# olofson/audiality2

Measured on AMD Instinct MI355X. Metric: voice-samples/sec + max realtime voices @48kHz, higher is better.
Workload: dtype int32; 1 GPU; 65536 voices 2xwtosc->panmix, 256 per group voice inline->fbdelay->fbdelay (benchmark/fmtest4.a2s delay settings; 256 groups, 512 fbdelays), 48 kHz, fragment=64, stereo (BASELINE configs[3]); voices_per_gpu=65536, chain=osc2-pan, groups=256

## Files before the change

### audiality2_amd/build.py

```python
import hashlib
import os
import shutil
import subprocess

HERE = os.path.dirname(os.path.abspath(__file__))
ROOT = os.path.dirname(HERE)
HIPCC = shutil.which("hipcc") or "/opt/rocm/bin/hipcc"


MARK = b"A2AMD_SRCHASH:"


def source_hash(sources, cmd=()):
    h = hashlib.sha256()
    for s in sources:
        h.update(os.path.basename(s).encode() + b"\0")
        with open(s, "rb") as f:
            h.update(f.read())
        h.update(b"\0")
    h.update(" ".join(cmd).encode())
    return h.hexdigest()[:32]


def stamped_hash(lib, mark=MARK):
    if not os.path.exists(lib):
        return None
    with open(lib, "rb") as f:
        blob = f.read()
    i = blob.find(mark)
    if i < 0:
        return None
    return blob[i + len(mark):i + len(mark) + 32].decode("ascii", "replace")


ENGMARK = b"A2AMD_ENGHASH:"


def engine_hash(engine):
    files = []
    for d in ("include", "src", os.path.join("src", "units"), os.path.join("src", "drivers")):
        p = os.path.join(engine, d)
        if os.path.isdir(p):
            files += [os.path.join(p, f) for f in sorted(os.listdir(p)) if f.endswith((".h", ".h.cmake", ".h.in"))]
    return source_hash(files, (stamped_hash(os.path.join(HERE, "liba2amd_units.so")) or "",))


def _stale(target, want):
    return stamped_hash(target) != want


def _define(h):
    return '-DA2AMD_SRCHASH="%s"' % h


def build_lib(force=False):
    csrc = os.path.join(HERE, "csrc")
    srcs = [os.path.join(csrc, f) for f in ("a2amd_host.cpp", "a2amd_sched.cpp", "a2amd_render.cpp", "a2amd_dist.cpp",
                                            "a2amd_vm.cpp", "a2amd_kernels.hip", "a2amd_fast.hip", "a2amd_vm.hip", "a2amd_wavecap.hip", "a2amd_wavepost.hip", "a2amd_win.hip", "a2amd_vmwin.hip", "a2amd_noise.hip", "a2amd_noisepan.hip", "a2amd_noisefiltpan.hip", "a2amd_cutsweep.hip", "a2amd_oscbare.hip", "a2amd_osc3filtpan.hip")]
    deps = srcs + [os.path.join(csrc, "a2amd_host.h"), os.path.join(csrc, "a2amd_switches.h"), os.path.join(csrc, "a2amd_device.h"), os.path.join(csrc, "a2amd_dsp.h"),
                   os.path.join(csrc, "a2amd_fm.h"), os.path.join(csrc, "a2amd_vmcore.h"), os.path.join(csrc, "a2amd_taps.h"), os.path.join(csrc, "a2amd_winctl.h"), os.path.join(csrc, "a2amd_vmdev.h"), os.path.join(csrc, "a2amd_noisemap.h"), os.path.join(csrc, "a2amd_noisevoice.h"), os.path.join(csrc, "a2amd_settled.h"), os.path.join(csrc, "a2amd_quiet.h"), os.path.join(csrc, "a2amd_cutsweep.h"), os.path.join(csrc, "a2amd_filt.h"), os.path.join(csrc, "a2amd_wavepads.h"), os.path.join(csrc, "a2amd_wavetame.h"), os.path.join(ROOT, "include", "a2amd.h"),
                   os.path.join(ROOT, "include", "a2amd_noise.h"), os.path.join(ROOT, "include", "a2amd_noisepan.h"), os.path.join(ROOT, "include", "a2amd_noisefilt.h"), os.path.join(ROOT, "include", "a2amd_sweep.h"), os.path.join(ROOT, "include", "a2amd_wavepost.h"),
                   os.path.join(ROOT, "include", "a2amd_bus.h"), os.path.join(ROOT, "include", "a2amd_oscbare.h"), os.path.join(ROOT, "include", "a2amd_osc3filt.h"), os.path.join(ROOT, "include", "a2amd_fbdpan.h"), os.path.join(ROOT, "include", "a2amd_buswin.h"), os.path.join(ROOT, "include", "a2amd_vmbatch.h"), os.path.join(ROOT, "include", "a2amd_osc2.h"), os.path.join(ROOT, "include", "a2amd_osc2lds.h"), os.path.join(ROOT, "include", "a2amd_osc2tame.h"), os.path.join(ROOT, "include", "a2amd_wavepool.h"), os.path.join(ROOT, "include", "a2amd_vm.h")]
    out = os.path.join(HERE, "liba2amd.so")
    flags = ["--offload-arch=gfx950", "-O3", "-std=c++17", "-fPIC", "-shared", "-Wno-unused-value"]
    want = source_hash(deps, flags)
    if force or _stale(out, want):
        subprocess.run([HIPCC] + flags + [_define(want), "-o", out] + srcs, check=True)
    return out


def build_units(force=False):
    src = os.path.join(HERE, "csrc", "a2amd_units.c")
    deps = [src, os.path.join(ROOT, "include", "a2amd.h"), os.path.join(ROOT, "include", "a2amd_noise.h"), os.path.join(ROOT, "include", "a2amd_noisepan.h"),
            os.path.join(ROOT, "include", "a2amd_noisefilt.h"), os.path.join(ROOT, "include", "a2amd_sweep.h"), os.path.join(ROOT, "include", "a2amd_bus.h"),
            os.path.join(ROOT, "include", "a2amd_wavepost.h"), os.path.join(ROOT, "include", "a2amd_oscbare.h"), os.path.join(ROOT, "include", "a2amd_osc3filt.h"), os.path.join(ROOT, "include", "a2amd_fbdpan.h"), os.path.join(ROOT, "include", "a2amd_buswin.h"), os.path.join(ROOT, "include", "a2amd_vmbatch.h"), os.path.join(ROOT, "include", "a2amd_osc2.h"), os.path.join(ROOT, "include", "a2amd_osc2lds.h"), os.path.join(ROOT, "include", "a2amd_osc2tame.h"), os.path.join(ROOT, "include", "a2amd_wavepool.h"), os.path.join(ROOT, "include", "a2amd_plugin.h"),
            os.path.join(ROOT, "include", "a2amd_walk.h"), os.path.join(ROOT, "include", "a2amd_vm.h")]
    out = os.path.join(HERE, "liba2amd_units.so")
    flags = ["-O2", "-Wall", "-fPIC", "-shared"]
    want = source_hash(deps, flags)
    if force or _stale(out, want):
        subprocess.run(["gcc"] + flags + [_define(want), "-o", out, src,
                        "-L" + HERE, "-la2amd", "-ldl", "-lpthread", "-lm", "-Wl,-rpath,$ORIGIN"], check=True)
    return out


def build_walk(force=False, engine=None):
    engine = engine or os.environ.get("A2_ENGINE_SRC", "/root/reference")
    out = os.path.join(HERE, "liba2amd_walk.so")
    src = os.path.join(HERE, "csrc", "a2amd_walk.c")
    own = [src, os.path.join(ROOT, "include", "a2amd_walk.h"), os.path.join(ROOT, "include", "a2amd_vm.h"),
           os.path.join(ROOT, "include", "a2amd_plugin.h")]
    flags = ["-O2", "-Wall", "-fPIC", "-shared"]
    want = source_hash(own, flags)
    kept = os.path.join(ROOT, "oracle", "_ref", "liba2amd_walk.so")
    if not (os.path.exists(os.path.join(engine, "src", "internals.h")) and shutil.which("cmake")):
        if (not os.path.exists(out) or _stale(out, want)) and not _stale(kept, want):
            shutil.copyfile(kept, out)
        if os.path.exists(out) and _stale(out, want):
            raise RuntimeError(f"{out} was not built from this tree's a2amd_walk.c (stamp {stamped_hash(out)}, "
                               f"sources {want}) and the engine's source tree ({engine}) is not here to rebuild it")
        return out if os.path.exists(out) else None
    inc = os.path.join(HERE, "_engine_include")
    weng = engine_hash(engine)
    if force or _stale(out, want) or stamped_hash(out, ENGMARK) != weng:
        subprocess.run(["cmake", f"-DENGINE={engine}", f"-DOUT={inc}", "-P", os.path.join(HERE, "csrc", "engine_header.cmake")],
                       check=True, stdout=subprocess.DEVNULL)
        subprocess.run(["gcc"] + flags + [_define(want), '-DA2AMD_ENGHASH="%s"' % weng, "-I" + inc] +
                       ["-I" + os.path.join(engine, d) for d in ("include", "src", "src/units", "src/drivers")] +
                       ["-o", out, src, "-L" + HERE, "-la2amd_units", "-la2amd", "-ldl", "-lpthread", "-Wl,-rpath,$ORIGIN"],
                       check=True)
    if stamped_hash(kept) != want or stamped_hash(kept, ENGMARK) != weng:
        os.makedirs(os.path.dirname(kept), exist_ok=True)
        shutil.copyfile(out, kept)
    return out


def build_oracle(force=False):
    odir = os.path.join(ROOT, "oracle")
    targets = ["restate"]
    if os.path.exists("/root/reference/src/core.c") and shutil.which("cmake"):
        targets += ["ref", "tools", "optionb"]
    subprocess.run(["make", "-s", "-C", odir] + (["-B"] if force else []) + targets, check=True)
    return os.path.join(odir, "liba2oracle.so")


def build_all(force=False):
    lib = build_lib(force)
    build_units(force)
    build_walk(force)
    return lib, build_oracle(force)
```

### audiality2_amd/csrc/a2amd_device.h

```cpp
#pragma once
#include <stdint.h>

#define A2D_MAXCHAIN   16
#define A2D_CHAIN_INLINE 8
#define A2D_MAXBATCH 256
#define FBW_MAXWIN (2 * A2D_MAXBATCH)
#define A2D_USTATE    24
#define A2D_MAXCH      8
#define A2D_FRAG      64
#define A2D_MIPS      10
#define A2D_FBD_BUFSIZE 131072
#define A2D_MAXPHINC  512
#define A2D_COEF_WORDS 3
#define A2D_WTOSC_MAXLENGTH (0x01000000 - 1 - 131)

enum { A2D_WTOSC = 0, A2D_PANMIX, A2D_FILTER12, A2D_FBDELAY, A2D_INLINE, A2D_XINSERT,
	A2D_FM1, A2D_FM2, A2D_FM3, A2D_FM4, A2D_FM3P, A2D_FM4P, A2D_FM2R, A2D_FM4R,
	A2D_DC, A2D_WAVESHAPER, A2D_DCBLOCK, A2D_LIMITER, A2D_XSINK, A2D_XSOURCE };
#define A2D_IS_FM(k) ((k) >= A2D_FM1 && (k) <= A2D_FM4R)

enum { A2D_OSC_OFF = 0, A2D_OSC_NOISE, A2D_OSC_WAVE, A2D_OSC_MIPWAVE };

#define A2D_DESC(kind, add, nin, nout, wired) \
	(((uint32_t)(kind) << 24) | ((uint32_t)(add) << 4) | ((uint32_t)(nin) << 8) | \
// ... 120 lines not shown
	A2DRun         *runs;
	A2DRun         *vmrun;
	A2DRec         *recs;
	uint32_t        rec_base, rec_cap;
	uint32_t       *total;
	uint32_t        now;
	uint32_t        msdur;
	int32_t         samplerate, basepitch;
	int32_t         nfrags;
	uint8_t         fragframes[A2D_MAXBATCH];
	uint8_t         fragbase[A2D_MAXBATCH];
};

enum { XW_SLOT = 0, XW_MODE = 1 };
#define A2D_XIO_HALF ((size_t)A2D_MAXBATCH * 8 * A2D_FRAG)
#define A2D_XIO_SLOT (2 * A2D_XIO_HALF)

#define A2D_FAST_FCH 8
#define A2D_OSC2_FCH 4
#define A2D_OSC2_SCH 16
#define A2D_OSC2_LDS_ENT 128
#define A2D_MAXVPW   32

struct A2DParams {
	const A2DVoice *voices;
	const A2DVoiceExt *vext;
	const uint32_t *udesc;
	int32_t        *ustate;
	int32_t        *vactive;
	const A2DRun   *runs;
	const A2DRec   *recs;
	const A2DWave  *waves;
	const int16_t  *wavepool;
	const int32_t  *wavecoef;
	int32_t        *busmem;
	int32_t        *fbdmem;
	const uint32_t *ptab;
	int32_t        *fmstate;
	const uint32_t *fmsine;
	int32_t *xio;
	const uint32_t *nseed;
	const int32_t  *nslot;
	int32_t         nnoise;
	const int32_t  *cutf;
	const int32_t  *cslot;
	int32_t         ncut;
	int32_t         nfrags;
	int32_t         samplerate;
	int32_t         debug;
	uint8_t         fragframes[A2D_MAXBATCH];
	uint16_t        fragstart[A2D_MAXBATCH];
	const int32_t  *wavecoef4;
};

#ifdef __HIPCC__
#define A2D_HD static inline __host__ __device__
#else
#define A2D_HD static inline
#endif
A2D_HD bool a2d_osc2_slice(int nfrags, int ysplit, int slice, int *c_lo, int *c_hi, int *nslices)
{
	const int nchunks = (nfrags + A2D_OSC2_FCH - 1) / A2D_OSC2_FCH;
	const int per = (nchunks + ysplit - 1) / ysplit;
	*c_lo = slice * per;
	*c_hi = *c_lo + per < nchunks ? *c_lo + per : nchunks;
	*nslices = (nchunks + per - 1) / per;
	return *c_lo < nchunks;
}
A2D_HD bool a2d_osc2_whole(unsigned start_first, unsigned start_last, unsigned frames_last, int n)
{
	return start_last + frames_last - start_first == (unsigned)n * A2D_FRAG;
}

A2D_HD unsigned a2d_osc2_stage(unsigned size0, unsigned periodic0, unsigned size1, unsigned periodic1)
{
	const bool c0 = periodic0 && size0 && !(size0 & (size0 - 1)) && size0 <= A2D_OSC2_LDS_ENT;
	const bool c1 = periodic1 && size1 && !(size1 & (size1 - 1)) && size1 <= A2D_OSC2_LDS_ENT;
	return (c0 ? 1u : 0u) | (c1 && (c0 ? size0 : 0u) + size1 <= A2D_OSC2_LDS_ENT ? 2u : 0u);
}

A2D_HD unsigned a2d_osc2_tame(unsigned tame0, unsigned tame1)
{
	return tame0 && tame1 ? 1u : 0u;
}

#ifdef __HIPCC__
static inline __host__ __device__ bool a2d_noise_seed(const A2DParams &p, int f, int ui, unsigned *seed)
{
	if(!p.nseed)
		return false;
	const int k = p.nslot[ui];
	if(k <= 0 || k > p.nnoise)
		return false;
	*seed = p.nseed[(size_t)f * (size_t)p.nnoise + (size_t)(k - 1)];
	return true;
}
#endif

#ifdef __HIPCC__
static inline __host__ __device__ bool a2d_cut_coeff(const A2DParams &p, int f, int ui, int *f1)
{
	if(p.ncut <= 0)
		return false;
#if defined(__HIP_DEVICE_COMPILE__)
	typedef const __attribute__((address_space(4))) A2DParams *CP;
	typedef const __attribute__((address_space(4))) int32_t *CI;
	uintptr_t qa = (uintptr_t)&p;
	asm volatile("" : "+s"(qa));
	const CP q = (CP)qa;
	const int ncut = q->ncut;
	const int k = *((CI)(uintptr_t)q->cslot + ui);
	if(k <= 0 || k > ncut)
		return false;
	const int v = *((CI)(uintptr_t)q->cutf + ((size_t)f * (size_t)ncut + (size_t)(k - 1)));
#else
	const int k = p.cslot[ui];
	if(k <= 0 || k > p.ncut)
		return false;
	const int v = p.cutf[(size_t)f * (size_t)p.ncut + (size_t)(k - 1)];
#endif
	if(v < 0)
		return false;
	*f1 = v;
	return true;
}
#endif

struct A2DCutSweep { int32_t ramper[4]; int32_t unit, slot, pad[2]; };
int a2d_launch_cut_sweep(const A2DCutSweep *list, int n, int f0, int count, unsigned frames, int32_t *cutf, int stride,
		size_t words, int32_t *cslot, int nunits, void *stream);
int a2d_launch_cut_resolve(int32_t *cutf, size_t words, const int32_t *f1tab, void *stream);

struct A2DNoiseOsc { uint32_t ph_lo, ph_hi, dphase; int32_t unit, slot, pad[3]; };
int a2d_launch_noise_seeds(const A2DNoiseOsc *osc, int n, uint32_t start, int f0, int count, unsigned frames,
		uint32_t *seed, int stride, size_t seed_words, int32_t *nslot, int nunits, void *stream);

int a2d_launch_leaf_noisepan(const A2DParams *dparams, const A2DParams &hp, const int *dlist, int nlist, int vpw, void *stream);
int a2d_launch_leaf_noisefiltpan(const A2DParams *dparams, const A2DParams &hp, const int *dlist, int nlist, int vpg, void *stream);
int a2d_launch_leaf_oscbare(const A2DParams *dparams, const A2DParams &hp, const int *dlist, int nlist, int vpw, void *stream);
int a2d_launch_leaf_osc3filtpan(const A2DParams *dparams, const A2DParams &hp, const int *dlist, int nlist, int vpg, void *stream);

int a2d_launch_vm(const A2DVmParams &vp, int emit, void *stream);
int a2d_launch_vm_pool(const A2DVmParams &vp, unsigned *out, void *stream);
#define A2D_WIN_STAGED 2
struct A2DVmwOut {
	A2DVmVoice *vmv;
	int        *ustate;
	int        *vactive;
	A2DRun     *runs;
	uint32_t   *total;
	uint32_t   *idle;
};
int a2d_launch_vm_commit(const A2DVmParams &vp, const A2DParams &hp, int nosc, int filt, const A2DVmwOut &from, void *stream);
int a2d_launch_vm_win(const A2DVmParams &vp, const A2DParams &hp, int nosc, int filt, int fa, int fb, uint32_t now_fa,
		uint32_t batch_end, int *wslot, int *wext, int *wscr, unsigned *widx, unsigned *wtop, unsigned wcap, void *stream,
		const A2DVmwOut *out = nullptr);
#define A2D_VMW_ROW (64 - 1 - 1)

int a2d_launch_voices(const A2DParams *dparams, const int *dlist, int nlist, int vpw, void *stream);
enum { A2D_STAGED_NONE = 0, A2D_STAGED_PHASES, A2D_STAGED_FULL };
struct A2DCommit { const int *list; int nlist, nosc; const int *ustage; const unsigned char *staged; };
struct A2DCommitSet { A2DCommit c[2]; int n; };
int a2d_launch_leaf_oscpan(const A2DParams *dparams, const A2DParams &hp, const int *dlist, int nlist,
		int vpw, int ysplit, int *ustage, unsigned char *staged, void *stream, void *event_after_main, A2DCommit *defer);
int a2d_launch_bus_driver(const A2DParams *dparams, const int *dlist, int nlist, int nfrags, int consume,
		const A2DCommitSet *commits, void *stream, int *master_host = nullptr, int ramping = 0);
int a2d_launch_commit(const A2DParams &hp, const A2DCommit &cm, void *stream);
int a2d_launch_bus_fbdchain(const A2DParams *dparams, const int *dlist, int nlist, int consume, void *stream);
int a2d_launch_bus_fbdpan(const A2DParams *dparams, const int *dlist, int nlist, int consume, void *stream, int windows = 0);
int a2d_launch_park(int32_t *stage, int32_t *bus, unsigned words, void *stream);
int a2d_launch_add_bus(int32_t *dst, int32_t *src, unsigned words, void *stream);
int a2d_launch_add_inject(const int32_t *inj, int32_t *bus, int nch, int n, int nfrags, void *stream);
int a2d_launch_build_coef(const int16_t *pool, int *coef, int *coef4, unsigned lo, unsigned hi, void *stream);
int a2d_launch_capture(const int32_t *bus, int32_t *dst, const uint32_t *fragpos, int nfrags, int nch, void *stream);
int a2d_launch_wave_from_pcm(const int32_t *pcm, int16_t *pool, const uint32_t *off, const uint32_t *size, int levels, int looped,
		int pre, int post, void *stream);
int a2d_launch_wave_level0(const int32_t *pcm, int16_t *d, unsigned size, void *stream);
int a2d_launch_wave_finish(int16_t *pool, const uint32_t *off, const uint32_t *size, int levels, int looped, int pre, int post,
		void *stream);
unsigned a2d_wavepost_scratch_words(unsigned size, unsigned flags, unsigned chunk);
int a2d_launch_wave_level0_post(const int32_t *pcm, int16_t *d, unsigned size, unsigned flags, unsigned chunk, uint32_t *scratch,
		void *stream);
int a2d_osc2filtpan_max_vpg(void);
int a2d_launch_leaf_osc2filtpan(const A2DParams *dparams, const A2DParams &hp, const int *dlist, int nlist,
		int vpg, void *stream);
int a2d_launch_leaf_oscfiltpan(const A2DParams *dparams, const A2DParams &hp, const int *dlist, int nlist,
		int vpw, void *stream);
int a2d_launch_scatter_runs(const int *didx, const A2DRun *dval, int n, A2DRun *druns, void *stream);
int a2d_launch_leaf_osc2pan(const A2DParams *dparams, const A2DParams &hp, const int *dlist, int nlist,
		int vpw, int ysplit, int *ustage, unsigned char *staged, void *stream, A2DCommit *defer, int voice_major, int lds_taps,
		int tame, unsigned long long *tame_count, int *ysplit_used);
struct A2Switches;
int a2d_launch_leaf_recs(const A2Switches &sw, const A2DParams *dparams, const A2DParams &hp, int nosc, int filt, const int *dlist,
		int nlist, int vpw, void *stream, int skip_empty = 0);
#define A2D_WIN_WORDS 24
#define A2D_WIN_SLOTWORDS(nosc, filt) ((filt) ? ((nosc) == 1 ? 20 : 24) : ((nosc) == 1 ? 12 : 20))
int a2d_launch_win_ctl(const A2DParams *dparams, const A2DParams &hp, int nosc, int filt, const int *dlist, int nlist,
		int skip_empty, int fa, int fb, int *wslot, int *wext, unsigned *widx, unsigned *wtop, unsigned wcap, int *wrc,
		void *stream);
int a2d_launch_win_render(const A2Switches &sw, const A2DParams &hp, int nosc, int filt, const int *dlist, int nlist, int fa, int fb,
		const int *wslot, const int *wext, const unsigned *widx, void *stream);
int a2d_launch_leaf_recs_all(const A2Switches &sw, const A2DParams *dparams, const A2DParams &hp, const int *const *lists, const int *counts,
		int vpw, void *stream, int skip_mask = 0);
int a2d_launch_leaf_fmpan(const A2DParams *dparams, const A2DParams &hp, int kind, const int *dlist, int nlist,
		int vpw, void *stream);
int a2d_launch_leaf_fmpan_all(const A2DParams *dparams, const A2DParams &hp, const int *dlist,
		const int *count8, int vpw, void *stream);
```

### audiality2_amd/csrc/a2amd_fast.hip

```cpp
#include <hip/hip_runtime.h>
#include <type_traits>
#include <algorithm>
#include <stdlib.h>
#include "a2amd_device.h"
#include "a2amd_switches.h"
#include "a2amd_dsp.h"
#include "a2amd_fm.h"
#include "a2amd_filt.h"

#include "a2amd_taps.h"

__global__ void k_build_coef(const int16_t *__restrict__ pool, int *__restrict__ coef, int *__restrict__ coef4, unsigned lo,
		unsigned hi)
{
	const unsigned j = lo + blockIdx.x * blockDim.x + threadIdx.x;
	if(j >= hi)
		return;
	const int dm = pool[j - 1], d0 = pool[j], d1 = pool[j + 1], d2 = pool[j + 2];
	const int c = (d1 - dm) >> 1;
	const int a = (3 * (d0 - d1) + d2 - dm) >> 1;
	const int b = dm - d0 + c - a;
	int *e = coef + A2D_COEF_WORDS * (size_t)j;
	e[0] = a;
	e[1] = b;
// ... 148 lines not shown
		ramp_prepare_s(o.a, nframes);
		const uint64_t phk = o.phase + (uint64_t)(unsigned)(in ? lane : 0) * o.dphase;
		const uint64_t nph = phk + o.dphase;
		const bool draw = in && ((o.dphase >= (1u << 23)) || ((nph ^ phk) >> 23));
		const unsigned long long m = __ballot(draw);
		const int me = (int)(threadIdx.x & 63);
		const unsigned long long below = (me >= 63) ? ~0ull : ((2ull << me) - 1ull);
		const int mine = __popcll(m & below), total = __popcll(m);
		int held = o.noise, myval = o.noise;
		unsigned st = o.seed;
		for(int j = 1; j <= total; ++j) {
			held = noise_next(st) - 32767;
			if(j == mine)
				myval = held;
		}
		o.seed = st;
		o.noise = held;
		if(in) {
			int ak = wadd(o.a.value, wmul(o.a.delta, lane));
			x = wmul(myval, ak >> 10) >> 6;
		}
		o.phase += (uint64_t)(unsigned)nframes * o.dphase;
		ramp_run(o.a, nframes);
	} else {
		ramp_prepare_s(o.p, nframes);
		ramp_prepare_s(o.a, nframes);
		ramp_run(o.p, nframes);
		ramp_run(o.a, nframes);
	}
	pd.x = x;
	return pd;
}

DEV int osc_fragment_s(const FastPtrs &g, OscS &o, int nframes, int lane)
{
	const OscPend pd = osc_fragment_begin(g, o, nframes, lane);
	return osc_fragment_end(pd);
}

DEV void pan_fragment_s(Ramp &vol, Ramp &pan, int x, int nframes, int lane, int &acc0, int &acc1)
{
	const bool clamp = a2s_pan_over(pan.target) || a2s_pan_over(pan.value);
	ramp_prepare_s(vol, nframes);
	ramp_prepare_s(pan, nframes);
	if((unsigned)lane < (unsigned)nframes) {
		int vk = wadd(vol.value, wmul(vol.delta, lane));
		int pk = wadd(pan.value, wmul(pan.delta, lane));
		int vp = mul64s(pk, vk, 24);
		int v0 = wsub(vk, vp), v1 = wadd(vk, vp);
		if(clamp) {
			int lim = wshl(vk, 1);
			if(v0 > lim) v0 = lim;
			if(v1 > lim) v1 = lim;
		}
		acc0 = wadd(acc0, mul64s(x, v0, 24));
		acc1 = wadd(acc1, mul64s(x, v1, 24));
	}
	ramp_run(vol, nframes);
	ramp_run(pan, nframes);
}

DEV void oscpan_fragment(const FastPtrs &g, OscS &o, Ramp &vol, Ramp &pan,
		int nframes, int lane, int &acc0, int &acc1)
{
	int x = osc_fragment_s(g, o, nframes, lane);
	pan_fragment_s(vol, pan, x, nframes, lane, acc0, acc1);
}

DEV int frames_of(const int (&ffr)[A2D_MAXBATCH / 64], int f)
{
	int r = 0;
#pragma unroll
	for(int k = 0; k < A2D_MAXBATCH / 64; ++k)
		if((f >> 6) == k)
			r = rdl(ffr[k], f & 63);
	return r;
}

enum { SV_MODE = 0, SV_WAVE, SV_DPHASE, SV_PHLO, SV_PHHI, SV_PRAMP, SV_P = 6, SV_A = 10,
	SV_VOL = 14, SV_PAN = 18, SV_NWORDS = 22 };

enum { DV_SETTLED = 0, DV_MM, DV_DPH, DV_SIZEM, DV_DOFF, DV_V0, DV_V1, DV_NWORDS };

DEV bool settled_wave(const A2DWave *w, unsigned dphase, int *d, bool settled = true, unsigned *periodic = nullptr,
		unsigned *tame = nullptr)
{
	unsigned dph;
	const unsigned mm = a2s_mip(dphase, w->period, &dph);
	d[0] = (int)mm;
	d[1] = (int)dph;
	d[2] = (int)w->size[mm];
	d[3] = (int)w->off[mm];
	if(periodic)
		*periodic = (w->periodic >> mm) & 1u;
	if(tame)
		*tame = (w->tame >> mm) & 1u;
	return settled && a2s_wave_ok(w->size[0], w->flags, dph);
}

DEV void osc_from_mem(OscS &o, const volatile int *w)
{
	o.mode = rfl(w[OW_MODE]);
	o.wave = rfl(w[OW_WAVE]);
	o.dphase = (unsigned)rfl(w[OW_DPHASE]);
	o.phase = (uint64_t)(unsigned)rfl(w[OW_PHASE_LO]) | ((uint64_t)(unsigned)rfl(w[OW_PHASE_HI]) << 32);
	o.p_ramping = rfl(w[OW_PRAMPING]);
	o.p.value = rfl(w[OW_P]); o.p.target = rfl(w[OW_P + 1]);
	o.p.delta = rfl(w[OW_P + 2]); o.p.timer = rfl(w[OW_P + 3]);
	o.a.value = rfl(w[OW_A]); o.a.target = rfl(w[OW_A + 1]);
	o.a.delta = rfl(w[OW_A + 2]); o.a.timer = rfl(w[OW_A + 3]);
	o.noise = 0;
	o.seed = 0;
}

DEV void osc_to_mem(int *w, const OscS &o)
{
	w[OW_MODE] = o.mode;
	w[OW_WAVE] = o.wave;
	w[OW_DPHASE] = (int)o.dphase;
	w[OW_PHASE_LO] = (int)(unsigned)o.phase;
	w[OW_PHASE_HI] = (int)(unsigned)(o.phase >> 32);
	w[OW_PRAMPING] = o.p_ramping;
	w[OW_P] = o.p.value; w[OW_P + 1] = o.p.target; w[OW_P + 2] = o.p.delta; w[OW_P + 3] = o.p.timer;
	w[OW_A] = o.a.value; w[OW_A + 1] = o.a.target; w[OW_A + 2] = o.a.delta; w[OW_A + 3] = o.a.timer;
}

DEV void stage_mark(unsigned char *m, bool mine, bool settled, bool last_slice, bool walker)
{
	if(mine && !settled) {
		if(walker)
			*m = A2D_STAGED_FULL;
	} else if(last_slice)
		*m = mine ? A2D_STAGED_PHASES : A2D_STAGED_NONE;
}

#define OSC1_WPE 4
__global__ __launch_bounds__(64 * FAST_WPB) __attribute__((amdgpu_waves_per_eu(OSC1_WPE, OSC1_WPE)))
void k_leaf_oscpan(const A2DParams *__restrict__ pp, const int *__restrict__ list, int nlist, int vpw,
		int ysplit, const A2DVoice *__restrict__ voices, const int *ustate,
		int *ustage, const int16_t *__restrict__ wavepool,
		const A2DWave *__restrict__ waves, const uint32_t *__restrict__ ptab, int *__restrict__ busmem,
		const int *__restrict__ wavecoef, unsigned char *__restrict__ staged)
{
	const A2DParams &p = *pp;
	const int wv = rfl((int)(threadIdx.x >> 6));
	const int lane = threadIdx.x & 63;
	const int first = (blockIdx.x * FAST_WPB + wv) * vpw;
	if(first >= nlist)
		return;
	const int nv = min(vpw, nlist - first);
	const int nfrags = p.nfrags;
	const int dbg = p.debug;
	FastPtrs g = { wavepool, waves, ptab, dbg };
	const CoefRsrc crs = coef_rsrc(wavecoef);

	const int nchunks = (nfrags + FAST_FCH - 1) / FAST_FCH;
	const int per = (nchunks + ysplit - 1) / ysplit;
	const int slice = blockIdx.y;
	const int c_lo = slice * per, c_hi = min(nchunks, c_lo + per);
	const bool last_slice = c_hi >= nchunks;
	if(c_lo >= nchunks)
		return;
	const int nslices = (nchunks + per - 1) / per;

	int ffr[A2D_MAXBATCH / 64], fst[A2D_MAXBATCH / 64];
#pragma unroll
	for(int k = 0; k < A2D_MAXBATCH / 64; ++k) {
		ffr[k] = (k * 64 + lane < nfrags) ? p.fragframes[k * 64 + lane] : 0;
		fst[k] = (k * 64 + lane < nfrags) ? p.fragstart[k * 64 + lane] : 0;
	}

	int dv[DV_NWORDS], amp_l = 0, phlo_l = 0, phhi_l = 0;
	int u0 = 0, u1 = 0, my_off = -1, my_nch = 2;
	bool mine = false;
#pragma unroll
	for(int k = 0; k < DV_NWORDS; ++k)
		dv[k] = 0;
	if(lane < nv)
		mine = p.runs[list[first + lane]].count == 0;
	if(mine) {
		const A2DVoice &vc = voices[list[first + lane]];
		u0 = vc.unit[0];
		u1 = vc.unit[1];
		my_off = vc.out_off;
		my_nch = vc.out_nch;
		const int *w0 = ustate + (size_t)u0 * A2D_USTATE;
		const int *w1 = ustate + (size_t)u1 * A2D_USTATE;
		int sv[SV_NWORDS];
		sv[SV_MODE] = w0[OW_MODE]; sv[SV_WAVE] = w0[OW_WAVE]; sv[SV_DPHASE] = w0[OW_DPHASE];
		sv[SV_PHLO] = w0[OW_PHASE_LO]; sv[SV_PHHI] = w0[OW_PHASE_HI]; sv[SV_PRAMP] = w0[OW_PRAMPING];
#pragma unroll
		for(int k = 0; k < 4; ++k) {
			sv[SV_P + k] = w0[OW_P + k];
			sv[SV_A + k] = w0[OW_A + k];
			sv[SV_VOL + k] = w1[PW_VOL + k];
			sv[SV_PAN + k] = w1[PW_PAN + k];
		}
		bool settled = a2s_osc_settled(sv[SV_MODE], (unsigned)sv[SV_DPHASE], sv[SV_PRAMP], sv + SV_P, sv + SV_A) &&
				a2s_arrived(sv + SV_VOL, sv + SV_PAN);
		if(settled) {
			settled = settled_wave(waves + sv[SV_WAVE], (unsigned)sv[SV_DPHASE], dv + DV_MM);
			a2s_pan_gains(sv[SV_VOL], sv[SV_PAN], a2s_pan_over(sv[SV_PAN]), &dv[DV_V0], &dv[DV_V1]);
		}
		dv[DV_SETTLED] = settled ? ((sv[SV_MODE] == A2D_OSC_MIPWAVE && (waves[sv[SV_WAVE]].flags & A2D_WF_RAWTAPS)) ? 3 : 1) : 0;
		amp_l = sv[SV_A];
		phlo_l = sv[SV_PHLO];
		phhi_l = sv[SV_PHHI];
	}
	const unsigned long long unsettled_mask = __ballot(mine && !dv[DV_SETTLED]);
	const unsigned long long settled_mask = __ballot(mine && dv[DV_SETTLED]);
	const unsigned long long raw_mask = __ballot(mine && dv[DV_SETTLED] == 3);

	for(int c = c_lo; c < c_hi; ++c) {
		const int f0 = c * FAST_FCH;
		const int nf = min((int)FAST_FCH, nfrags - f0);
		int acc0[FAST_FCH], acc1[FAST_FCH];
// ... 387 lines not shown
{
	CoefRsrc crs4 = crs;
	if(TAME)
		crs4 = coef4_rsrc(wavecoef4);
	int cur_off = rdl(my_off, 0), cur_nch = rdl(my_nch, 0);
	for(int v = 0; v < nv; ++v) {
		const int sl = rdl(settled_l, v);
		if(!sl)
			continue;
		const int voff = rdl(my_off, v);
		if(voff != cur_off) {
			flush_tile(busmem, cur_off, cur_nch, fa, nfs, nsc * OSC2_FCH, lane, dbg, tile);
			cur_off = voff;
			cur_nch = rdl(my_nch, v);
		}
		const int v0 = rdl(v0l, v), v1 = rdl(v1l, v);
		Osc2Voice s;
		unsigned ldph[2], mm[2];
		if(TAME && (sl & 8)) {
			osc2_voice_from_lanes(s, ldph, mm, od, amp_l, phlo_l, phhi_l, v, before, lane, true);
			Osc2Lds lv = { { level, level }, { 0, 0 } };
			const int st = (sl >> 1) & 3;
			if(st) {
				lds_wave_fence();
				if(st & 1) {
					lv.lg[0] = (s.sizem[0] - 1) << 4;
					stage_level4(level, wavecoef4, s.cb[0], s.sizem[0], lane);
				}
				if(st & 2) {
					LdsInt *const l1 = (st & 1) ? level + s.sizem[0] * 4 : level;
					lv.level[1] = l1;
					lv.lg[1] = (s.sizem[1] - 1) << 4;
					stage_level4(l1, wavecoef4, s.cb[1], s.sizem[1], lane);
				}
				lds_wave_fence();
			}
			switch(st) {
			case 0: osc2_voice_chunks<0, true>(crs4, s, ldph, mm, lv, nsc, nfs, last, v0, v1, v, lane, tile, phlo_l, phhi_l); break;
			case 1: osc2_voice_chunks<1, true>(crs4, s, ldph, mm, lv, nsc, nfs, last, v0, v1, v, lane, tile, phlo_l, phhi_l); break;
			case 2: osc2_voice_chunks<2, true>(crs4, s, ldph, mm, lv, nsc, nfs, last, v0, v1, v, lane, tile, phlo_l, phhi_l); break;
			default: osc2_voice_chunks<3, true>(crs4, s, ldph, mm, lv, nsc, nfs, last, v0, v1, v, lane, tile, phlo_l, phhi_l); break;
			}
			continue;
		}
		osc2_voice_from_lanes(s, ldph, mm, od, amp_l, phlo_l, phhi_l, v, before, lane);
		Osc2Lds lv = { { level, level }, { 0, 0 } };
		if(!STAGE) {
			osc2_voice_chunks<0>(crs, s, ldph, mm, lv, nsc, nfs, last, v0, v1, v, lane, tile, phlo_l, phhi_l);
			continue;
		}
		const int st = sl >> 1;
		if(st) {
			lds_wave_fence();
			if(st & 1) {
				lv.lg[0] = (unsigned)__builtin_ctz(s.sizem[0]);
				stage_level(level, wavecoef, s.cb[0], s.sizem[0], lane);
			}
			if(st & 2) {
				LdsInt *const l1 = (st & 1) ? level + s.sizem[0] * A2D_COEF_WORDS : level;
				lv.level[1] = l1;
				lv.lg[1] = (unsigned)__builtin_ctz(s.sizem[1]);
				stage_level(l1, wavecoef, s.cb[1], s.sizem[1], lane);
			}
			lds_wave_fence();
		}
		switch(st) {
		case 0: osc2_voice_chunks<0>(crs, s, ldph, mm, lv, nsc, nfs, last, v0, v1, v, lane, tile, phlo_l, phhi_l); break;
		case 1: osc2_voice_chunks<1>(crs, s, ldph, mm, lv, nsc, nfs, last, v0, v1, v, lane, tile, phlo_l, phhi_l); break;
		case 2: osc2_voice_chunks<2>(crs, s, ldph, mm, lv, nsc, nfs, last, v0, v1, v, lane, tile, phlo_l, phhi_l); break;
		default: osc2_voice_chunks<3>(crs, s, ldph, mm, lv, nsc, nfs, last, v0, v1, v, lane, tile, phlo_l, phhi_l); break;
		}
	}
	flush_tile(busmem, cur_off, cur_nch, fa, nfs, nsc * OSC2_FCH, lane, dbg, tile);
}

#define OSC2_WPE 4
template<bool TAME_K>
__global__ __launch_bounds__(64 * FAST_WPB) __attribute__((amdgpu_waves_per_eu(OSC2_WPE, OSC2_WPE)))
void k_leaf_osc2pan(const A2DParams *__restrict__ pp, const int *__restrict__ list, int nlist, int vpw,
		int ysplit, const A2DVoice *__restrict__ voices, const int *ustate, int *ustage,
		const int16_t *__restrict__ wavepool, const A2DWave *__restrict__ waves,
		const uint32_t *__restrict__ ptab, int *__restrict__ busmem, const int *__restrict__ wavecoef,
		unsigned char *__restrict__ staged, int vmajor, int lds_taps, const int *__restrict__ wavecoef4, int tame,
		unsigned long long *__restrict__ tame_count)
{
	const A2DParams &p = *pp;
	const int wv = rfl((int)(threadIdx.x >> 6));
	const int lane = threadIdx.x & 63;
	const int first = (blockIdx.x * FAST_WPB + wv) * vpw;
	if(first >= nlist)
		return;
	const int nv = min(vpw, nlist - first);
	const int nfrags = p.nfrags;
	const int dbg = p.debug;
	FastPtrs g = { wavepool, waves, ptab, dbg };
	const CoefRsrc crs = coef_rsrc(wavecoef);

	const int slice = blockIdx.y;
	int c_lo, c_hi, nslices;
	if(!a2d_osc2_slice(nfrags, ysplit, slice, &c_lo, &c_hi, &nslices))
		return;
	const bool last_slice = c_hi * OSC2_FCH >= nfrags;

	int ffr[A2D_MAXBATCH / 64], fst[A2D_MAXBATCH / 64];
#pragma unroll
	for(int k = 0; k < A2D_MAXBATCH / 64; ++k) {
		ffr[k] = (k * 64 + lane < nfrags) ? p.fragframes[k * 64 + lane] : 0;
		fst[k] = (k * 64 + lane < nfrags) ? p.fragstart[k * 64 + lane] : 0;
	}

	int od[2][OD_NWORDS], amp_l[2] = { 0, 0 }, phlo_l[2] = { 0, 0 }, phhi_l[2] = { 0, 0 };
	int v0l = 0, v1l = 0, settled_l = 0;
	int uu[3] = { 0, 0, 0 }, my_off = -1, my_nch = 2;
	bool mine = false;
#pragma unroll
	for(int o = 0; o < 2; ++o)
#pragma unroll
		for(int k = 0; k < OD_NWORDS; ++k)
			od[o][k] = 0;
	if(lane < nv)
		mine = p.runs[list[first + lane]].count == 0;
	if(mine) {
		const A2DVoice &vc = voices[list[first + lane]];
		my_off = vc.out_off;
		my_nch = vc.out_nch;
		bool settled = true;
		int wave_l[2], dphase_l[2];
		unsigned periodic[2] = { 0, 0 }, tame_lv[2] = { 0, 0 };
#pragma unroll
		for(int o = 0; o < 2; ++o) {
			uu[o] = vc.unit[o];
			const int *w = ustate + (size_t)uu[o] * A2D_USTATE;
			wave_l[o] = w[OW_WAVE];
			dphase_l[o] = w[OW_DPHASE];
			amp_l[o] = w[OW_A];
			phlo_l[o] = w[OW_PHASE_LO];
			phhi_l[o] = w[OW_PHASE_HI];
			settled = settled && a2s_osc_settled(w[OW_MODE], (unsigned)dphase_l[o], w[OW_PRAMPING], w + OW_P, w + OW_A);
		}
		uu[2] = vc.unit[2];
		const int *wp = ustate + (size_t)uu[2] * A2D_USTATE;
		int sp[8];
#pragma unroll
		for(int k = 0; k < 8; ++k)
			sp[k] = wp[k];
		settled = settled && a2s_arrived(sp + PW_VOL, sp + PW_PAN);
		if(settled) {
#pragma unroll
			for(int o = 0; o < 2; ++o)
				settled = settled_wave(waves + wave_l[o], (unsigned)dphase_l[o], od[o], settled, &periodic[o],
						TAME_K ? &tame_lv[o] : nullptr);
			a2s_pan_gains(sp[PW_VOL], sp[PW_PAN], a2s_pan_over(sp[PW_PAN]), &v0l, &v1l);
		}
		settled_l = settled ? 1 : 0;
		if(settled && lds_taps)
			settled_l |= (int)a2d_osc2_stage((unsigned)od[0][OD_SIZEM], periodic[0], (unsigned)od[1][OD_SIZEM], periodic[1]) << 1;
		if(TAME_K && settled && tame)
			settled_l |= (int)a2d_osc2_tame(tame_lv[0], tame_lv[1]) << 3;
	}
	const unsigned long long unsettled_mask = __ballot(mine && !settled_l);
	const bool any_staged = __ballot((settled_l & 6) != 0) != 0;
	const unsigned long long tame_mask = TAME_K ? __ballot((settled_l & 8) != 0) : 0ull;
	const bool any_tame = tame_mask != 0;
	if(TAME_K && any_tame && slice == 0 && lane == 0)
		atomicAdd(tame_count, (unsigned long long)__popcll(tame_mask));

	__shared__ int tiles[FAST_WPB][OSC2_SCH][2][A2D_FRAG];
	__shared__ __attribute__((aligned(16))) int levels[FAST_WPB][A2D_OSC2_LDS_ENT * (TAME_K ? 4 : A2D_COEF_WORDS)];
	int (*const tile)[2][A2D_FRAG] = tiles[wv];
	LdsInt *const level = (LdsInt *)levels[wv];
	if(vmajor)
#pragma unroll
		for(int r = 0; r < OSC2_SCH; ++r)
// ... 1932 lines not shown
						++r;
					wk = lane - ((fr[r][4] >> 8) & 0xff);
				}
				const int vk = wadd(fr[r][0], wmul(fr[r][1], wk));
				const int pk = wadd(fr[r][2], wmul(fr[r][3], wk));
				const int vp = mul64s(pk, vk, 24);
				v0 = wsub(vk, vp); v1 = wadd(vk, vp);
				if(WIN ? fr[r][4] & 1 : fr[r][4]) {
					const int lim = wshl(vk, 1);
					if(v0 > lim) v0 = lim;
					if(v1 > lim) v1 = lim;
				}
			}
			const int o0 = mul64s(x0, v0, 24), o1 = mul64s(x1, v1, 24);
			int *dst = out + (size_t)f * out_nch * A2D_FRAG;
			if(o0)
				atomicAdd(&dst[lane], o0);
			if(o1)
				atomicAdd(&dst[A2D_FRAG + lane], o1);
		}
		if(fend < nfrags)
			__syncthreads();
	}
	if(threadIdx.x == 0) {
		int total = 0;
		for(int f = 0; f < nfrags; ++f)
			total += p.fragframes[f];
#pragma unroll
		for(int k = 0; k < FBC_MAXD; ++k)
			if(k < nd)
				p.ustate[(size_t)vc.unit[k + 1] * A2D_USTATE + DW_BUFPOS] = wadd(d[k].pos, total);
	}
}

__global__ __launch_bounds__(FBC_THREADS)
void k_bus_fbdpan(const A2DParams *__restrict__ pp, const int *__restrict__ list, int nlist, int consume)
{
	bus_fbdpan<false>(pp, list, consume);
}

__global__ __launch_bounds__(FBC_THREADS)
void k_bus_fbdpan_win(const A2DParams *__restrict__ pp, const int *__restrict__ list, int nlist, int consume)
{
	bus_fbdpan<true>(pp, list, consume);
}

int a2d_launch_bus_fbdpan(const A2DParams *dparams, const int *dlist, int nlist, int consume, void *stream, int windows)
{
	if(nlist <= 0)
		return 0;
	hipLaunchKernelGGL(windows ? k_bus_fbdpan_win : k_bus_fbdpan, dim3(nlist), dim3(FBC_THREADS), 0, (hipStream_t)stream,
			dparams, dlist, nlist, consume);
	return (int)hipGetLastError();
}

int a2d_launch_leaf_oscpan(const A2DParams *dparams, const A2DParams &hp, const int *dlist, int nlist,
		int vpw, int ysplit, int *ustage, unsigned char *staged, void *stream, void *event_after_main, A2DCommit *defer)
{
	if(nlist <= 0)
		return 0;
	vpw = vpw < 1 ? 1 : (vpw > 64 ? 64 : vpw);
	if(ysplit < 1 || !ustage || !staged)
		ysplit = 1;
	int nwaves = (nlist + vpw - 1) / vpw;
	int nblocks = (nwaves + FAST_WPB - 1) / FAST_WPB;
	hipLaunchKernelGGL(k_leaf_oscpan, dim3(nblocks, ysplit), dim3(64 * FAST_WPB), 0, (hipStream_t)stream,
			dparams, dlist, nlist, vpw, ysplit, hp.voices, (const int *)hp.ustate,
			ysplit > 1 ? ustage : hp.ustate, hp.wavepool, hp.waves, hp.ptab, hp.busmem, hp.wavecoef, staged);
	if(event_after_main)
		hipEventRecord((hipEvent_t)event_after_main, (hipStream_t)stream);
	if(ysplit > 1) {
		A2DCommit cm = { dlist, nlist, 1, ustage, staged };
		if(defer)
			*defer = cm;
		else
			a2d_launch_commit(hp, cm, stream);
	} else if(defer)
		defer->nlist = 0;
	return (int)hipGetLastError();
}

int a2d_launch_leaf_osc2pan(const A2DParams *dparams, const A2DParams &hp, const int *dlist, int nlist,
		int vpw, int ysplit, int *ustage, unsigned char *staged, void *stream, A2DCommit *defer, int voice_major, int lds_taps,
		int tame, unsigned long long *tame_count, int *ysplit_used)
{
	if(nlist <= 0)
		return 0;
	vpw = vpw < 1 ? 1 : (vpw > 64 ? 64 : vpw);
	if(ysplit < 1 || !ustage || !staged)
		ysplit = 1;
	if(ysplit_used)
		*ysplit_used = ysplit;
	int nwaves = (nlist + vpw - 1) / vpw;
	int nblocks = (nwaves + FAST_WPB - 1) / FAST_WPB;
	if(tame && hp.wavecoef4 && tame_count)
		hipLaunchKernelGGL(k_leaf_osc2pan<true>, dim3(nblocks, ysplit), dim3(64 * FAST_WPB), 0, (hipStream_t)stream,
				dparams, dlist, nlist, vpw, ysplit, hp.voices, (const int *)hp.ustate,
				ysplit > 1 ? ustage : hp.ustate, hp.wavepool, hp.waves, hp.ptab, hp.busmem, hp.wavecoef, staged, voice_major, lds_taps,
				hp.wavecoef4, 1, tame_count);
	else
		hipLaunchKernelGGL(k_leaf_osc2pan<false>, dim3(nblocks, ysplit), dim3(64 * FAST_WPB), 0, (hipStream_t)stream,
				dparams, dlist, nlist, vpw, ysplit, hp.voices, (const int *)hp.ustate,
				ysplit > 1 ? ustage : hp.ustate, hp.wavepool, hp.waves, hp.ptab, hp.busmem, hp.wavecoef, staged, voice_major, lds_taps,
				(const int *)nullptr, 0, (unsigned long long *)nullptr);
	if(ysplit > 1) {
		A2DCommit cm = { dlist, nlist, 2, ustage, staged };
		if(defer)
			*defer = cm;
		else
			a2d_launch_commit(hp, cm, stream);
	} else if(defer)
		defer->nlist = 0;
	return (int)hipGetLastError();
}

__global__ void k_scatter_runs(const int *__restrict__ idx, const A2DRun *__restrict__ val, int n,
		A2DRun *__restrict__ runs)
{
	int i = blockIdx.x * blockDim.x + threadIdx.x;
	if(i < n)
		runs[idx[i]] = val[i];
}

int a2d_launch_scatter_runs(const int *didx, const A2DRun *dval, int n, A2DRun *druns, void *stream)
{
	if(n <= 0)
		return 0;
	hipLaunchKernelGGL(k_scatter_runs, dim3((n + 255) / 256), dim3(256), 0, (hipStream_t)stream,
			didx, dval, n, druns);
	return (int)hipGetLastError();
}

int a2d_launch_leaf_oscfiltpan(const A2DParams *dparams, const A2DParams &hp, const int *dlist, int nlist,
		int vpg, void *stream)
{
	if(nlist <= 0)
		return 0;
	vpg = vpg < 1 ? 1 : (vpg > FILT_MAXV ? FILT_MAXV : vpg);
	int nblocks = (nlist + vpg - 1) / vpg;
	size_t lds = (size_t)3 * vpg * FILT_PITCH * sizeof(int);
	hipLaunchKernelGGL(k_leaf_oscfiltpan, dim3(nblocks), dim3(64 * FILT_WAVES), lds, (hipStream_t)stream,
			dparams, dlist, nlist, vpg, hp.voices, hp.ustate, hp.wavepool, hp.waves, hp.ptab, hp.busmem, hp.wavecoef);
	return (int)hipGetLastError();
}

int a2d_osc2filtpan_max_vpg(void)
{
	const int nfull = FILT_WAVES - 1 - (FILT_WAVES / 4 - 1);
	const int v = nfull * (FILT2_LAUNCHV < FILT2_FASTV ? FILT2_LAUNCHV : FILT2_FASTV);
	return v > FILT_MAXV ? FILT_MAXV : v;
}

int a2d_launch_leaf_osc2filtpan(const A2DParams *dparams, const A2DParams &hp, const int *dlist, int nlist,
		int vpg, void *stream)
{
	if(nlist <= 0)
		return 0;
	vpg = vpg < 1 ? 1 : (vpg > FILT_MAXV ? FILT_MAXV : vpg);
	int nblocks = (nlist + vpg - 1) / vpg;
	size_t lds = (size_t)3 * vpg * FILT_PITCH * sizeof(int);
	hipLaunchKernelGGL(k_leaf_osc2filtpan, dim3(nblocks), dim3(64 * FILT_WAVES), lds, (hipStream_t)stream,
			dparams, dlist, nlist, vpg, hp.voices, hp.ustate, hp.wavepool, hp.waves, hp.ptab, hp.busmem, hp.wavecoef);
	return (int)hipGetLastError();
}

enum { PV_VOL = 0, PV_PAN = 4, PV_NWORDS = 8 };

DEV void pan_window_s(Ramp &vol, Ramp &pan, int x, int off, int len, int lane, int &acc0, int &acc1)
{
	const bool clamp = a2s_pan_over(pan.target) || a2s_pan_over(pan.value);
	ramp_prepare_s(vol, len);
	ramp_prepare_s(pan, len);
	const int k = lane - off;
	if(k >= 0 && k < len) {
		int vk = wadd(vol.value, wmul(vol.delta, k));
		int pk = wadd(pan.value, wmul(pan.delta, k));
		int vp = mul64s(pk, vk, 24);
		int v0 = wsub(vk, vp), v1 = wadd(vk, vp);
		if(clamp) {
			int lim = wshl(vk, 1);
			if(v0 > lim) v0 = lim;
			if(v1 > lim) v1 = lim;
		}
		acc0 = wadd(acc0, mul64s(x, v0, 24));
		acc1 = wadd(acc1, mul64s(x, v1, 24));
	}
	ramp_run(vol, len);
// ... 459 lines not shown
```

### audiality2_amd/csrc/a2amd_host.cpp

```cpp
#include "a2amd_host.h"
#include "a2amd_noisemap.h"
#include "a2amd_cutsweep.h"
#include "a2amd_settled.h"
#include "a2amd_wavepads.h"
#include "a2amd_wavetame.h"

namespace a2h { thread_local char g_err[256] = ""; }

extern "C" {

const char *a2amd_version(void) { return "a2amd 0.1 (gfx950)"; }
#ifndef A2AMD_SRCHASH
#define A2AMD_SRCHASH "unstamped"
#endif
const char *a2amd_source_stamp(void) { return "A2AMD_SRCHASH:" A2AMD_SRCHASH; }

const char *a2amd_last_error(const a2amd_ctx *c) { return c ? c->err : g_err; }

int a2amd_device_count(void)
{
	int n = 0;
	return hipGetDeviceCount(&n) == hipSuccess ? n : 0;
}


int a2amd_open(const a2amd_config *cfg, a2amd_ctx **out)
{
	if(!cfg || !out || cfg->channels < 1 || cfg->channels > A2D_MAXCH || cfg->samplerate <= 0) {
		snprintf(g_err, sizeof(g_err), "a2amd_open: bad configuration");
		return A2AMD_EINVAL;
	}
	int ndev = 0;
	hipError_t e = hipGetDeviceCount(&ndev);
	if(e != hipSuccess || ndev <= 0 || cfg->device >= ndev) {
		snprintf(g_err, sizeof(g_err), "a2amd_open: no usable HIP device (%s, %d devices, want #%d); "
				"this library has no CPU fallback", hipGetErrorString(e), ndev, cfg->device);
		return A2AMD_ENODEVICE;
	}
	a2amd_ctx *c = new a2amd_ctx();
	c->cfg = *cfg;
	c->err[0] = 0;
	if(!c->cfg.max_batch)
		c->cfg.max_batch = 1;
	if(c->cfg.max_batch > A2D_MAXBATCH)
		c->cfg.max_batch = A2D_MAXBATCH;
	memset(&c->stats, 0, sizeof(c->stats));
	build_pitch_table(c->ptab);
	a2amd_read_switches(&c->sw);
	c->bus_stride_frames = (size_t)c->cfg.max_batch * A2D_FRAG;
	c->bus_used = c->bus_stride_frames * (size_t)c->cfg.channels;
#define OPENCHK(call) do { hipError_t e_ = (call); if(e_ != hipSuccess) { \
	snprintf(g_err, sizeof(g_err), "a2amd_open: %s: %s", #call, hipGetErrorString(e_)); \
	delete c; return A2AMD_EHIP; } } while(0)
	OPENCHK(hipSetDevice(cfg->device));
	if(cfg->stream)
		c->stream = (hipStream_t)cfg->stream;
	else {
		OPENCHK(hipStreamCreateWithFlags(&c->stream, hipStreamNonBlocking));
		c->own_stream = true;
	}
	OPENCHK(hipEventCreate(&c->ev0));
	OPENCHK(hipEventCreate(&c->ev1));
	OPENCHK(hipEventCreate(&c->ev2));
	c->ev_pool.push_back(c->ev0);
	c->ev_pool.push_back(c->ev1);
	c->ev_pool.push_back(c->ev2);
	OPENCHK(hipMalloc((void **)&c->d_ptab, sizeof(c->ptab)));
	OPENCHK(hipMalloc((void **)&c->d_wavepool.d, (size_t)(8u << 20) * sizeof(int16_t)));
	c->d_wavepool.cap = 8u << 20;
	OPENCHK(hipMalloc((void **)&c->d_wavecoef.d, (size_t)(8u << 20) * A2D_COEF_WORDS * sizeof(int32_t)));
	c->d_wavecoef.cap = 8u << 20;
	if(coef4_wanted(c, 0)) {
		OPENCHK(hipMalloc((void **)&c->d_wavecoef4.d, (size_t)(8u << 20) * 4 * sizeof(int32_t)));
		c->d_wavecoef4.cap = 8u << 20;
	}
	OPENCHK(hipMalloc((void **)&c->d_tame_count, sizeof(unsigned long long)));
	OPENCHK(hipMemset(c->d_tame_count, 0, sizeof(unsigned long long)));
#undef OPENCHK
	*out = c;
	return A2AMD_OK;
}

void a2amd_close(a2amd_ctx *c)
{
	if(!c)
		return;
	use_device(c);
	hipStreamSynchronize(c->stream);
	if(c->vm.pred_stream)
		hipStreamSynchronize(c->vm.pred_stream);
	drop_graphs(c);
	if(c->comm && g_rccl.CommDestroy)
		g_rccl.CommDestroy(c->comm);
	if(c->grp_ev)
		hipEventDestroy(c->grp_ev);
	hipFree(c->d_voices.d); hipFree(c->d_vext.d); hipFree(c->d_udesc.d); hipFree(c->d_ustate.d); hipFree(c->d_ustage.d);
	hipFree(c->d_vactive.d); hipFree(c->d_runs.d); hipFree(c->d_recs.d);
	hipFree(c->d_nseed.d); hipFree(c->d_nslot.d);
	hipFree(c->d_cutf.d); hipFree(c->d_cslot.d);
	hipFree(c->d_win.d); hipFree(c->d_wext.d); hipFree(c->d_wscr.d); hipFree(c->d_wrc.d); hipFree(c->d_widx.d); hipFree(c->d_wtop);
	if(c->h_wtop)
		hipHostFree(c->h_wtop);
	if(c->wtop_ev)
		hipEventDestroy(c->wtop_ev);
	if(c->win_stream)
		hipStreamDestroy(c->win_stream);
	for(int k = 0; k < 7; ++k)
		if(c->win_fork[k])
			hipStreamDestroy(c->win_fork[k]);
	for(int k = 0; k < 8; ++k)
		if(c->win_fev[k])
			hipEventDestroy(c->win_fev[k]);
	for(int k = 0; k < 5; ++k)
		if(c->win_ev[k])
			hipEventDestroy(c->win_ev[k]);
	hipFree(c->d_waves.d); hipFree(c->d_wavepool.d); hipFree(c->d_wavecoef.d); hipFree(c->d_wavecoef4.d); hipFree(c->d_tame_count); hipFree(c->d_busmem.d);
	vm_close(c);
	hipFree(c->capture.d); hipFree(c->capture.d_fragpos); hipFree(c->d_wavepost.d);
	hipFree(c->d_fbdmem.d); hipFree(c->d_fmstate.d); hipFree(c->d_xio.d); hipFree(c->d_fmsine); hipFree(c->d_list.d); hipFree(c->d_staged.d); hipFree(c->d_scatter.d); hipFree(c->d_ptab); hipFree(c->d_blob.d);
	for(int k = 0; k < 2; ++k) { if(c->h_blob[k]) hipHostFree(c->h_blob[k]); if(c->blob_ev[k]) hipEventDestroy(c->blob_ev[k]); }
	if(c->h_master)
		hipHostFree(c->h_master);
	for(int k = 0; k < 2; ++k) { if(c->rb[k].h) hipHostFree(c->rb[k].h); if(c->rb[k].ev) hipEventDestroy(c->rb[k].ev); }
	for(hipEvent_t e : c->ev_pool)
		hipEventDestroy(e);
	if(c->own_stream)
		hipStreamDestroy(c->stream);
	delete c;
}

int a2amd_set_pitch_table(a2amd_ctx *c, const uint32_t *t)
{
	memcpy(c->ptab, t, sizeof(c->ptab));
	c->ptab_dirty = true;
	return A2AMD_OK;
}

int a2amd_get_pitch_table(const a2amd_ctx *c, uint32_t *t)
{
	memcpy(t, c->ptab, sizeof(c->ptab));
	return A2AMD_OK;
}

}
namespace a2h {
bool coef4_wanted(const a2amd_ctx *c, size_t pool_samples)
{
	return c->sw.raw <= 0 && pool_samples * (4 * A2D_COEF_WORDS) <= ((size_t)c->sw.coef_cache_mb << 20);
}

void coef4_drop(a2amd_ctx *c)
{
	if(!c->d_wavecoef4.d)
		return;
	hipStreamSynchronize(c->stream);
	if(c->vm.pred_stream)
		hipStreamSynchronize(c->vm.pred_stream);
	hipFree(c->d_wavecoef4.d);
	c->d_wavecoef4.d = nullptr;
	c->d_wavecoef4.cap = 0;
	c->waves_dirty = true;
	drop_graphs(c);
	c->blob_quiet = false;
}

void wave_tap_policy(a2amd_ctx *c)
{
	const int force = c->sw.raw;
	const size_t budget = (size_t)c->sw.coef_cache_mb << 20;
	const bool big = c->wavepool_used * (4 * A2D_COEF_WORDS) > budget;
	if(!coef4_wanted(c, c->wavepool_used))
		coef4_drop(c);
	for(size_t i = 0; i < c->waves.size(); ++i) {
		HWave &w = c->waves[i];
		if(!w.live || w.dw.type != A2AMD_WMIPWAVE)
			continue;
		const bool raw = force >= 0 ? force != 0 : (big && w.dw.size[0] >= 4096);
		const uint32_t f = (w.dw.flags & ~A2D_WF_RAWTAPS) | (raw ? A2D_WF_RAWTAPS : 0u);
		if(f != w.dw.flags) {
			w.dw.flags = f;
			c->mwaves[i].flags = f;
			c->waves_dirty = true;
		}
	}
}
}
extern "C" {
}

struct a2amd_capture {
	int32_t *d;
	size_t n;
	int device;
};

namespace a2h {
int capture_append(a2amd_ctx *c)
{
	a2amd_ctx::Capture &cp = c->capture;
// ... 1507 lines not shown
```

### audiality2_amd/csrc/a2amd_host.h

```cpp
#ifndef A2AMD_HOST_H
#define A2AMD_HOST_H
#include <hip/hip_runtime.h>
#include <rccl/rccl.h>
#include <dlfcn.h>
#include <math.h>
#include <stdarg.h>
#include <stdio.h>
#include <stdlib.h>
#include <string.h>
#include <algorithm>
#include <map>
#include <vector>
#include <future>

#include "../../include/a2amd.h"
#include "../../include/a2amd_vm.h"
#include "a2amd_device.h"
#include "a2amd_switches.h"

#ifndef M_PI
#define M_PI 3.14159265358979323846
#endif

namespace a2h {
// ... 304 lines not shown
	size_t ev_used = 0;
	uint32_t ptab[128];

	std::vector<HUnit> units;
	std::vector<int> free_units, deferred_free_units;
	std::vector<HVoice> voices;
	std::vector<int> free_voices, deferred_free_voices;
	std::vector<HWave> waves;
	int building = -1;
	std::vector<int> stack;
	std::vector<A2DRec> up_recs;
	std::vector<int> up_idx, up_now;
	std::vector<A2DRun> up_val;
	std::vector<int> with_recs, prev_with_recs;
	std::vector<int> dirty_voices;
	long long serial_base = 0;
	bool o2f_quiet = true;
	int n_started_live = 0;
	int walked_started = 0;
	int n_noise = 0, n_cutoff_ramps = 0;
	std::vector<int> noise_order;
	long long noise_order_serial = -1, walk_serial = -2;
	struct NoiseStretch { int f0, count; unsigned frames; uint32_t start; size_t first, n; };
	std::vector<NoiseStretch> noise_st;
	std::vector<A2DNoiseOsc> noise_osc;
	int noise_slots = 0;
	DevBuf<uint32_t> d_nseed;
	DevBuf<int32_t> d_nslot;
	std::vector<int> sweeping;
	struct CutStretch { int f0, count; unsigned frames; size_t first, n; };
	std::vector<CutStretch> cut_st;
	std::vector<A2DCutSweep> cut_list;
	int cut_slots = 0;
	DevBuf<int32_t> d_cutf;
	DevBuf<int32_t> d_cslot;
	a2amd_sweep_batch_info last_sweeps = {};
	uint32_t n_cut_standin = 0;
	uint32_t n_cut_windows = 0;
	bool owners_all_driver = false;
	bool consume_ok = false;
	bool others_clean = false;
	bool root_clean = false;
	bool capturing = false;
	int n_clients = 0;
	int sub_resume = -1;
	int paused_at = 0;
	std::vector<int32_t> snap_ustate, snap_vactive;
	bool snap_valid = false;
	std::vector<uint8_t> defmap;
	bool defmap_used = false;
	bool defmap_dirty = false;
	std::vector<uint8_t> held;
	size_t n_held = 0;
	uint64_t walk_time = 0;
	unsigned prev_frames = 0;

	bool frag_open = false;
	int cur_frag = 0, nfrags = 0;
	unsigned fragframes[A2D_MAXBATCH];
	uint8_t fragbase[A2D_MAXBATCH];
	bool uploaded = false;

	std::vector<A2DVoice> mvoices;
	std::vector<A2DVoiceExt> mvext;
	bool long_chains = false;
	std::vector<uint32_t> mudesc;
	std::vector<A2DWave> mwaves;
	bool voices_dirty = true, udesc_dirty = true, waves_dirty = true, lists_dirty = true, ptab_dirty = true;
	std::vector<int> list_all;
	ListRange leaf[LEAF_N];
	int fm_kind_count[8] = { 0 };
	std::vector<DepthRange> depth_ranges;
	ListRange dyn[DYN_N];
	A2Switches sw;
	a2amd_batch_info last_batch = {};
	a2amd_noise_batch_info last_noise = {};
	uint32_t n_noise_standin = 0, n_noise_quiet = 0;
	uint32_t n_noise_filt_quiet = 0;
	a2amd_noise_filter_batch_info last_noise_filter = {};
	uint32_t n_bare_quiet = 0, n_bare_gliding = 0, n_bare_records = 0, n_mono_drivers = 0;
	a2amd_bare_batch_info last_bare = {};
	uint32_t n_o3f_quiet = 0, n_o3f_gliding = 0, n_o3f_records = 0;
	a2amd_osc3filt_batch_info last_osc3filt = {};
	a2amd_osc2_batch_info last_osc2 = {};
	a2amd_fbdpan_batch_info last_fbdpan = {};
	a2amd_bus_windows_info last_buswin = {};
	a2amd_bus_info last_bus = {};
	uint32_t n_bus_windows_dropped = 0;

	size_t bus_stride_frames;
	size_t bus_used = 0;
	std::map<int, std::vector<int>> bus_free;
	std::vector<std::pair<int,int>> deferred_bus_free;

	int fbd_count = 0;
	std::vector<int> fbd_free, fbd_deferred_free, fbd_to_zero;
	int fm_count = 0;
	std::vector<int> fm_free, fm_deferred_free;

	std::vector<XioSlot> xio;
	std::vector<int> xio_free, xio_deferred_free;

	size_t wavepool_used = 0;
	std::vector<std::pair<size_t, size_t>> wavepool_free;
	std::vector<std::pair<size_t, size_t>> deferred_wavepool_free;
	std::vector<int> free_wave_slots, deferred_wave_slots;
	uint32_t wavepool_reallocs = 0, wavepool_reused = 0;

	DevBuf<A2DVoice> d_voices;
	DevBuf<A2DVoiceExt> d_vext;
	DevBuf<uint32_t> d_udesc;
	DevBuf<int32_t> d_ustate;
	DevBuf<int32_t> d_ustage;
	DevBuf<int32_t> d_vactive;
	DevBuf<A2DRun> d_runs;
	DevBuf<A2DRec> d_recs;
	DevBuf<A2DWave> d_waves;
	DevBuf<int16_t> d_wavepool;
	DevBuf<int32_t> d_wavecoef;
	DevBuf<int32_t> d_wavecoef4;
	unsigned long long *d_tame_count = nullptr;
	DevBuf<int32_t> d_busmem;
	DevBuf<int32_t> d_fbdmem;
	DevBuf<int32_t> d_fmstate;
	DevBuf<int32_t> d_xio;
	uint32_t *d_fmsine = nullptr;
	DevBuf<int> d_list;
	DevBuf<unsigned char> d_staged;
	DevBuf<int> d_scatter;
	uint32_t *d_ptab = nullptr;
	A2DParams *d_params = nullptr;
	DevBuf<char> d_blob;
	char *h_blob[2] = { nullptr, nullptr };
	size_t h_blob_cap[2] = { 0, 0 };
	hipEvent_t blob_ev[2] = { nullptr, nullptr };
	bool blob_busy[2] = { false, false };
	int blob_i = 0;
	const int *d_dyn = nullptr;
	A2DParams hparams;
	hipGraph_t graph[12] = {};
	hipGraphExec_t gexec[12] = {};
	const int32_t *gdst[12] = {};
	bool gdirect[12] = {};
	uint32_t gconsume[12] = {};
	struct Capture { int32_t *d = nullptr; size_t cap = 0, n = 0; bool on = false; uint32_t *d_fragpos = nullptr; } capture;
	DevBuf<uint32_t> d_wavepost;
	uint64_t wave_h2d_bytes = 0;
	uint32_t waves_uploaded = 0, waves_resident = 0;
	int32_t *master_dst = nullptr;
	bool master_direct = false;
	int32_t *h_master = nullptr;
	size_t h_master_cap = 0;
	bool blob_quiet = false;
	int blob_nfrags = 0;
	unsigned blob_frames[A2D_MAXBATCH];
	int quiet_streak = 0;
	struct Readback {
		int32_t *h = nullptr;
		size_t cap = 0;
		hipEvent_t ev = nullptr;
		int nfrags = 0;
		unsigned total = 0;
		uint8_t frames[A2D_MAXBATCH];
	} rb[2];
	int rb_head = 0, rb_count = 0;

	ncclComm_t comm = nullptr;
	int dist_rank = 0, dist_ranks = 1;
	bool dist_local = false;
	hipEvent_t grp_ev = nullptr;

	std::vector<int> moving;
	size_t n_moving_listed = 0;
	DevBuf<int> d_win, d_wext, d_wrc, d_wscr;
	DevBuf<unsigned> d_widx;
	unsigned *d_wtop = nullptr;
	unsigned *h_wtop = nullptr;
	hipEvent_t wtop_ev = nullptr;
	bool wtop_pending = false;
	hipStream_t win_fork[7] = { nullptr, nullptr, nullptr, nullptr, nullptr, nullptr, nullptr };
	hipEvent_t win_fev[8] = { nullptr, nullptr, nullptr, nullptr, nullptr, nullptr, nullptr, nullptr };
	hipStream_t win_stream = nullptr;
	hipEvent_t win_ev[5] = { nullptr, nullptr, nullptr, nullptr, nullptr };

	a2amd_stats stats;
	VmHost vm;

	int fail(int code, const char *fmt, ...)
	{
		va_list ap;
		va_start(ap, fmt);
		vsnprintf(err, sizeof(err), fmt, ap);
		va_end(ap);
		snprintf(g_err, sizeof(g_err), "%s", err);
		return code;
	}
};

static inline void use_device(const a2amd_ctx *c) { (void)hipSetDevice(c->cfg.device); }

namespace a2h {
template<class T>
int grow(a2amd_ctx *c, DevBuf<T> &b, size_t need, size_t elem_mult, bool keep)
{
	if(need <= b.cap)
		return 0;
	size_t ncap = std::max(need, b.cap ? b.cap * 2 : (elem_mult >= 65536 ? (size_t)2 : (size_t)1024));
	T *nd = nullptr;
	HIPCHK(c, hipMalloc((void **)&nd, ncap * elem_mult * sizeof(T)));
	if(keep && b.d && b.cap) {
// ... 97 lines not shown
```

### audiality2_amd/csrc/a2amd_render.cpp

```cpp
#include "a2amd_host.h"
#include "a2amd_wavepads.h"
#include "a2amd_wavetame.h"

extern "C" {
static double now_us()
{
	timespec ts;
	clock_gettime(CLOCK_MONOTONIC, &ts);
	return ts.tv_sec * 1e6 + ts.tv_nsec * 1e-3;
}
static double g_t[4], g_n;
static double g_why[13];
static double g_cnt[6];
struct TimingDump { ~TimingDump() {
	A2Switches sw; a2amd_read_switches(&sw); if(sw.hosttiming && g_n) fprintf(stderr,
	"a2amd host timing per render: upload %.1f us, issue %.1f us, readback %.1f us (%g renders; %g quiet uploads, "
	"%g graph launches, %g records, %g voices with records, %g walk scans, %g R_NOPs)\n",
	g_t[0] / g_n, g_t[1] / g_n, g_t[2] / g_n, g_n, g_cnt[0], g_cnt[5], g_cnt[1], g_cnt[4], g_cnt[2], g_cnt[3]);
	if(sw.hosttiming && g_n) { fprintf(stderr, "a2amd uploads by first reason against the quiet path "
	"(blob, recs, prev recs, voices, udesc, waves, lists, ptab, dirty voices, fbd, nfrags, bus, none):");
	for(int k = 0; k < 13; ++k) fprintf(stderr, " %g", g_why[k]); fprintf(stderr, "\n"); } } } g_timing_dump;

}
namespace a2h { double *dbg_counters() { return g_cnt; } double *dbg_why() { return g_why; } }
// ... 432 lines not shown
	return A2AMD_OK;
}

int a2amd_last_batch_bare(const a2amd_ctx *c, a2amd_bare_batch_info *out)
{
	if(!c || !out)
		return A2AMD_EINVAL;
	*out = c->last_bare;
	return A2AMD_OK;
}

int a2amd_last_batch_osc3filt(const a2amd_ctx *c, a2amd_osc3filt_batch_info *out)
{
	if(!c || !out)
		return A2AMD_EINVAL;
	*out = c->last_osc3filt;
	return A2AMD_OK;
}

int a2amd_last_batch_osc2(const a2amd_ctx *c, a2amd_osc2_batch_info *out)
{
	if(!c || !out)
		return A2AMD_EINVAL;
	*out = c->last_osc2;
	if(!out->launched || c->blob_nfrags < 1 || c->blob_nfrags > A2D_MAXBATCH)
		return A2AMD_OK;
	unsigned start[A2D_MAXBATCH];
	for(int f = 0, acc = 0; f < c->blob_nfrags; ++f) {
		start[f] = (unsigned)acc;
		acc += (int)c->blob_frames[f];
	}
	unsigned n = 0;
	for(int slice = 0; slice < (int)out->ysplit; ++slice) {
		int c_lo, c_hi, nslices;
		if(!a2d_osc2_slice(c->blob_nfrags, (int)out->ysplit, slice, &c_lo, &c_hi, &nslices))
			break;
		for(int s_lo = c_lo; s_lo < c_hi; s_lo += A2D_OSC2_SCH / A2D_OSC2_FCH, ++n) {
			const int s_hi = std::min(c_hi, s_lo + A2D_OSC2_SCH / A2D_OSC2_FCH);
			const int fa = s_lo * A2D_OSC2_FCH, fb = std::min(c->blob_nfrags, s_hi * A2D_OSC2_FCH);
			if(out->voice_major && a2d_osc2_whole(start[fa], start[fb - 1], c->blob_frames[fb - 1], fb - fa))
				++out->superchunks_voice_major;
			else {
				++out->superchunks_chunk_major;
				if(n < 64)
					out->chunk_major_mask |= 1ull << n;
			}
		}
	}
	return A2AMD_OK;
}

unsigned a2amd_osc2_stage_rule(unsigned size0, int periodic0, unsigned size1, int periodic1)
{
	return a2d_osc2_stage(size0, periodic0 != 0, size1, periodic1 != 0);
}

int a2amd_wave_level_periodic(const int16_t *level, unsigned size)
{
	return a2w_pads_periodic(level, size, A2AMD_WAVEPRE, A2AMD_WAVEPOST);
}

int a2amd_wave_level_tame(const int16_t *level, unsigned size)
{
	return a2w_level_tame(level, size, A2AMD_WAVEPRE, A2AMD_WAVEPOST);
}

unsigned a2amd_osc2_tame_rule(int tame0, int tame1)
{
	return a2d_osc2_tame(tame0 != 0, tame1 != 0);
}

int a2amd_osc2_tame_voices(a2amd_ctx *c, uint64_t *out)
{
	if(!c || !out)
		return A2AMD_EINVAL;
	use_device(c);
	unsigned long long n = 0;
	HIPCHK(c, hipStreamSynchronize(c->stream));
	HIPCHK(c, hipMemcpy(&n, c->d_tame_count, sizeof(n), hipMemcpyDeviceToHost));
	*out = n;
	return A2AMD_OK;
}

int a2amd_last_batch_fbdpan(const a2amd_ctx *c, a2amd_fbdpan_batch_info *out)
{
	if(!c || !out)
		return A2AMD_EINVAL;
	*out = c->last_fbdpan;
	return A2AMD_OK;
}

int a2amd_last_batch_bus_windows(const a2amd_ctx *c, a2amd_bus_windows_info *out)
{
	if(!c || !out)
		return A2AMD_EINVAL;
	*out = c->last_buswin;
	out->window_cap = FBW_MAXWIN;
	return A2AMD_OK;
}

int a2amd_set_profiling(a2amd_ctx *c, int on)
{
	if(int r = drain_events(c))
		return r;
	if(on) {
		c->stats.timed_leaf_ms = c->stats.timed_all_ms = 0;
		c->stats.timed_batches = 0;
	}
	c->profiling = on != 0;
	return A2AMD_OK;
}

}
```

### audiality2_amd/csrc/a2amd_sched.cpp

```cpp
#include "a2amd_host.h"
#include "a2amd_cutsweep.h"
#include <functional>

namespace a2h {




void touch(a2amd_ctx *c, int vi)
{
	HVoice &v = c->voices[vi];
	const long long serial = c->serial_base + rec_tag(c);
	if(v.touched != serial) {
		v.touched = serial;
		v.frag_mark = v.recs.size();
	}
}



void spell_out_pending(a2amd_ctx *c, int vi)
{
	HVoice &dv = c->voices[vi];
	const bool marked = c->frag_open && c->defmap_used && (size_t)vi < c->defmap.size() && c->defmap[vi];
// ... 258 lines not shown
			!xi.xio_mode;
}


static bool fbd_units_ok(const a2amd_ctx *c, const HVoice &v, int nd)
{
	if(nd < 1 || nd > 4 || v.own_nch != 2 || v.out_nch < 2 || v.own_off < 0 || v.inline_pos != 0)
		return false;
	const HUnit &il = c->units[v.unit[0]];
	if(il.kind != A2AMD_INLINE || (il.flags & A2AMD_PROCADD) || il.wired || il.nout != 2)
		return false;
	for(int k = 1; k <= nd; ++k) {
		const HUnit &d = c->units[v.unit[k]];
		if(d.kind != A2AMD_FBDELAY || d.nin != 2 || d.nout != 2)
			return false;
		for(int t = 0; t < 3; ++t)
			if(!fbd_tap_ok(d.fbd_taps[t]))
				return false;
	}
	return true;
}

bool is_fbdchain(const a2amd_ctx *c, const HVoice &v)
{
	const int nd = v.nunits - 1;
	if(!fbd_units_ok(c, v, nd))
		return false;
	for(int k = 1; k <= nd; ++k) {
		const HUnit &d = c->units[v.unit[k]];
		const bool last = k == nd;
		if((d.wired != 0) != last || (last && !(d.flags & A2AMD_PROCADD)))
			return false;
	}
	return true;
}

int seg_rows(const A2DRec *recs, size_t nrecs, const unsigned *fragframes, int nfrags)
{
	if(!nrecs)
		return 0;
	for(size_t i = 0; i < nrecs; ++i)
		if(A2D_ROP(recs[i].head) != R_SEG)
			return 0;
	int rows = nfrags, prev = -1;
	unsigned at = 0;
	for(size_t i = 0; i < nrecs; ++i) {
		const int f = (int)A2D_RFRAG(recs[i].head);
		const unsigned off = recs[i].dur & 0xffff, n = recs[i].dur >> 16;
		if(f >= nfrags || f < prev)
			return -1;
		if(f != prev) {
			if(prev >= 0 && at != fragframes[prev])
				return -1;
			prev = f;
			at = 0;
		} else
			++rows;
		if(off != at || !n || n > fragframes[f] - at)
			return -1;
		at += n;
	}
	return at == fragframes[prev] ? rows : -1;
}

bool is_fbdpan_chain(const a2amd_ctx *c, const HVoice &v)
{
	const int nd = v.nunits - 2;
	if(!fbd_units_ok(c, v, nd))
		return false;
	for(int k = 1; k <= nd; ++k)
		if(c->units[v.unit[k]].wired)
			return false;
	const HUnit &pm = c->units[v.unit[nd + 1]];
	return pm.kind == A2AMD_PANMIX && pm.nin == 2 && pm.nout == 2 && pm.wired && (pm.flags & A2AMD_PROCADD);
}

static ListRange append_range(std::vector<int> &to, const std::vector<int> &l)
{
	const ListRange r = { (int)to.size(), (int)l.size() };
	to.insert(to.end(), l.begin(), l.end());
	return r;
}

int upload(a2amd_ctx *c)
{
	if(!c->cut_st.empty())
		vm_build_f1tab(c);
	if(int r = vm_prepare_batch(c))
		return r;
	c->last_sweeps = a2amd_sweep_batch_info{};
	c->n_cut_standin = 0;
	c->n_noise_standin = c->n_noise_quiet = c->n_noise_filt_quiet = 0;
	c->n_bus_windows_dropped = 0;
	c->last_bus.driver_ramping = c->last_bus.driver_windows_dropped = 0;
	c->last_fbdpan.gliding_voices = 0;
	c->last_buswin = a2amd_bus_windows_info{};
	c->last_buswin.window_cap = FBW_MAXWIN;
	if(c->sw.hosttiming) {
		const int why = !c->blob_quiet ? 0 : !c->with_recs.empty() ? 1 : !c->prev_with_recs.empty() ? 2 :
				c->voices_dirty ? 3 : c->udesc_dirty ? 4 : c->waves_dirty ? 5 : c->lists_dirty ? 6 : c->ptab_dirty ? 7 :
				!c->dirty_voices.empty() ? 8 : !c->fbd_to_zero.empty() ? 9 : c->nfrags != c->blob_nfrags ? 10 :
				c->bus_used > c->d_busmem.cap ? 11 :
				memcmp(c->fragframes, c->blob_frames, (size_t)c->nfrags * sizeof(unsigned)) ? 10 : 12;
		dbg_why()[why] += 1;
	}
	if(c->blob_quiet && c->with_recs.empty() && c->prev_with_recs.empty() && c->moving.empty() && c->noise_st.empty() && c->cut_st.empty() && !c->voices_dirty &&
			!c->udesc_dirty && !c->waves_dirty && !c->lists_dirty && !c->ptab_dirty && !c->vm.list_dirty &&
			c->dirty_voices.empty() && c->fbd_to_zero.empty() && c->bus_used <= c->d_busmem.cap) {
		bool inject = false;
		for(const XioSlot &x : c->xio)
			if(x.unit >= 0 && (x.inj_used || (c->units[x.unit].xio_mode & A2AMD_XIO_INJECT)))
				inject = true;
		const bool same = c->nfrags == c->blob_nfrags &&
				!memcmp(c->fragframes, c->blob_frames, (size_t)c->nfrags * sizeof(unsigned));
		if(!inject && same) {
			if(c->sw.hosttiming)
				dbg_counters()[0] += 1;
			++c->quiet_streak;
			c->uploaded = true;
			return 0;
		}
		if(!inject && c->d_params && c->stream) {
			A2DParams p = c->hparams;
			p.nfrags = c->nfrags;
			p.nseed = nullptr;
			p.nnoise = 0;
			p.cutf = nullptr;
			p.ncut = 0;
			memset(p.fragframes, 0, sizeof(p.fragframes));
			memset(p.fragstart, 0, sizeof(p.fragstart));
			for(int f = 0, acc = 0; f < c->nfrags; ++f) {
				p.fragframes[f] = (uint8_t)c->fragframes[f];
				p.fragstart[f] = (uint16_t)acc;
				acc += (int)c->fragframes[f];
			}
			const int bi = c->blob_i;
			c->blob_i ^= 1;
			if(c->blob_busy[bi]) {
				HIPCHK(c, hipEventSynchronize(c->blob_ev[bi]));
				c->blob_busy[bi] = false;
			}
			if(c->h_blob[bi] && c->h_blob_cap[bi] >= sizeof(A2DParams) && c->blob_ev[bi]) {
				memcpy(c->h_blob[bi], &p, sizeof(p));
				HIPCHK(c, hipMemcpyAsync(c->d_blob.d, c->h_blob[bi], sizeof(p), hipMemcpyHostToDevice, c->stream));
				HIPCHK(c, hipEventRecord(c->blob_ev[bi], c->stream));
				c->blob_busy[bi] = true;
				c->hparams = p;
				if(c->nfrags != c->blob_nfrags) {
					drop_graphs(c);
					c->quiet_streak = 0;
				} else
					++c->quiet_streak;
				c->blob_nfrags = c->nfrags;
				memcpy(c->blob_frames, c->fragframes, (size_t)c->nfrags * sizeof(unsigned));
				if(c->sw.hosttiming)
					dbg_counters()[0] += 1;
				c->uploaded = true;
				return 0;
			}
		}
	}
	c->blob_quiet = false;
	c->quiet_streak = 0;
	drop_graphs(c);
	const size_t nv = c->voices.size(), nu = c->units.size();
	if(int r = grow(c, c->d_voices, nv, 1, true)) return r;
	if(int r = grow(c, c->d_udesc, nu, 1, false)) return r;
	if(int r = grow(c, c->d_ustate, nu, A2D_USTATE, true)) return r;
	if(int r = grow(c, c->d_ustage, c->d_ustate.cap, A2D_USTATE, false)) return r;
	if(int r = grow(c, c->d_vactive, nv, 1, true)) return r;
	if(int r = grow(c, c->d_runs, nv, 1, true)) return r;
	if(!c->noise_st.empty()) {
		if(int r = grow(c, c->d_nseed, (size_t)c->nfrags * (size_t)c->noise_slots, 1, false)) return r;
		if(int r = grow(c, c->d_nslot, c->d_ustate.cap, 1, false)) return r;
	}
	if(!c->cut_st.empty()) {
		if(int r = grow(c, c->d_cutf, (size_t)c->nfrags * (size_t)c->cut_slots, 1, false)) return r;
		if(int r = grow(c, c->d_cslot, c->d_ustate.cap, 1, false)) return r;
	}
	{
		const int32_t *before = c->d_busmem.d;
		if(int r = grow(c, c->d_busmem, c->bus_used, 1, false)) return r;
		if(c->d_busmem.d != before)
			c->others_clean = c->root_clean = false;
	}
	if(c->fbd_count)
		if(int r = grow(c, c->d_fbdmem, c->fbd_count, 2 * (size_t)A2D_FBD_BUFSIZE, true)) return r;
	if(!c->xio.empty()) {
		if(int r = grow(c, c->d_xio, c->xio.size(), A2D_XIO_SLOT, true)) return r;
		const size_t n = (size_t)c->nfrags * A2AMD_MAXCHANNELS * A2D_FRAG;
		for(size_t k = 0; k < c->xio.size(); ++k) {
			XioSlot &x = c->xio[k];
			if(x.unit < 0 || !(x.inj_used || (c->units[x.unit].xio_mode & A2AMD_XIO_INJECT)))
				continue;
			HIPCHK(c, hipMemcpyAsync(c->d_xio.d + k * A2D_XIO_SLOT + A2D_XIO_HALF, x.inj.data(),
					n * sizeof(int32_t), hipMemcpyHostToDevice, c->stream));
			HIPCHK(c, hipStreamSynchronize(c->stream));
			if(x.inj_used)
				std::fill(x.inj.begin(), x.inj.begin() + n, 0);
			x.inj_used = false;
		}
	}
	if(c->fm_count) {
		if(int r = grow(c, c->d_fmstate, c->fm_count, A2D_FMSTATE, true)) return r;
		if(!c->d_fmsine) {
			int16_t sine[2049];
			uint32_t pairs[2048];
			for(int k = 0; k < 2049; ++k)
				sine[k] = (int16_t)(sin(k * 2.0f * M_PI / 2048) * 32767.0f);
			for(int k = 0; k < 2048; ++k)
				pairs[k] = (uint32_t)(uint16_t)sine[k] | ((uint32_t)(sine[k + 1] - sine[k]) << 16);
			HIPCHK(c, hipMalloc((void **)&c->d_fmsine, sizeof(pairs)));
			HIPCHK(c, hipMemcpy(c->d_fmsine, pairs, sizeof(pairs), hipMemcpyHostToDevice));
		}
	}

	if(c->voices_dirty && nv) {
		if(c->mvoices.size() < nv)
			c->mvoices.resize(nv);
		int lo = (int)nv, hi = -1;
		for(int vi : c->dirty_voices)
			if(vi < (int)nv) {
				sync_voice_mirror(c, vi);
				lo = std::min(lo, vi);
				hi = std::max(hi, vi);
			}
		c->dirty_voices.clear();
		if(hi >= lo)
			HIPCHK(c, hipMemcpyAsync(c->d_voices.d + lo, c->mvoices.data() + lo,
					(size_t)(hi - lo + 1) * sizeof(A2DVoice), hipMemcpyHostToDevice, c->stream));
		if(c->long_chains) {
// ... 179 lines not shown
	sc_idx.resize(nsc_used);
	sc_val.resize(nsc_used);
	c->prev_with_recs.clear();
	c->stats.records += recs.size();
	if(c->sw.hosttiming) {
		dbg_counters()[1] += (double)recs.size();
		dbg_counters()[4] += (double)c->with_recs.size();
	}

	if(c->lists_dirty) {
		const bool cls_check = c->sw.cls_check;
		bool owners_ok = !c->sw.no_selfclean, root_driver = false;
		std::vector<int> leaf[LEAF_N];
		std::map<int, std::pair<std::vector<int>, std::vector<int>>> bydepth;
		std::map<int, std::vector<int>> fbd_bydepth, fbdpan_bydepth;
		int maxdepth = -1;
		for(size_t vi = 0; vi < nv; ++vi) {
			HVoice &v = c->voices[vi];
			if(!(v.live || v.dying) || !v.resolved) {
				v.cls = -1;
				continue;
			}
			const bool classify = v.cls_stale || v.cls < 0 || cls_check;
			const int was_cls = v.cls;
			if(v.inline_pos >= 0) {
				auto &d = bydepth[v.depth];
				if(classify)
					v.cls = !(c->sw.no_fast & 4) && is_driver_chain(c, v) ? CLS_BUSDRIVER :
							!(c->sw.no_fast & 32) && v.depth > 0 && is_fbdchain(c, v) ? CLS_FBDCHAIN :
							!(c->sw.no_fast & 512) && v.depth > 0 && is_fbdpan_chain(c, v) ? CLS_FBDPAN : CLS_BUSGENERIC;
				if(v.cls == CLS_BUSGENERIC || (v.out_off == 0) != (v.depth == 0))
					owners_ok = false;
				else if(v.depth == 0)
					root_driver = true;
				(v.cls == CLS_BUSDRIVER ? d.first : v.cls == CLS_FBDCHAIN ? fbd_bydepth[v.depth] :
						v.cls == CLS_FBDPAN ? fbdpan_bydepth[v.depth] : d.second).push_back((int)vi);
				maxdepth = std::max(maxdepth, v.depth);
			} else {
				if(classify)
					v.cls = !(c->sw.no_fast & 1) && is_oscpan_chain(c, v) ?
								(c->sw.noise_quiet && c->units[v.unit[0]].mode == A2D_OSC_NOISE ? CLS_NOISEPAN : CLS_OSCPAN) :
							!(c->sw.no_fast & 8) && is_osc2pan_chain(c, v) ? CLS_OSC2PAN :
							!(c->sw.no_fast & 2) && is_oscfiltpan_chain(c, v) ?
								(c->sw.noise_quiet && c->units[v.unit[0]].mode == A2D_OSC_NOISE ? CLS_NOISEFILTPAN : CLS_OSCFILTPAN) :
							!(c->sw.no_fast & 128) && !v.mode_mix && is_osc2filtpan_chain(c, v) ? CLS_OSC2FILTPAN :
							!(c->sw.no_fast & 16) && is_fmpan_chain(c, v) ? CLS_FMPAN :
							!(c->sw.no_fast & 256) && v.vm < 0 && is_oscbare_chain(c, v) ? CLS_OSCBARE :
							!(c->sw.no_fast & 1024) && v.vm < 0 && !v.mode_mix && is_osc3filtpan_chain(c, v) ? CLS_OSC3FILTPAN :
							CLS_GENERIC;
				if(v.out_off == 0)
					owners_ok = false;
				leaf[cls_lists[v.cls].leaf].push_back((int)vi);
			}
			if(cls_check && !v.cls_stale && was_cls >= 0 && was_cls != v.cls)
				return c->fail(A2AMD_ESTATE, "voice %zu: remembered launch class %d, classified %d (a change nobody reported)",
						vi, was_cls, v.cls);
			v.cls_stale = false;
		}
		auto by_bus = [&](int a, int b) { return c->voices[a].out_off < c->voices[b].out_off; };
		for(int k = 0; k < LEAF_N; ++k)
			if(k != LEAF_FMPAN && !std::is_sorted(leaf[k].begin(), leaf[k].end(), by_bus))
				std::stable_sort(leaf[k].begin(), leaf[k].end(), by_bus);
		std::stable_sort(leaf[LEAF_FMPAN].begin(), leaf[LEAF_FMPAN].end(), [&](int a, int b) {
			const int ka = c->units[c->voices[a].unit[0]].kind, kb = c->units[c->voices[b].unit[0]].kind;
			return ka != kb ? ka < kb : c->voices[a].out_off < c->voices[b].out_off;
		});
		for(int k = 0; k < 8; ++k)
			c->fm_kind_count[k] = 0;
		for(int vi : leaf[LEAF_FMPAN])
			++c->fm_kind_count[c->units[c->voices[vi].unit[0]].kind - A2AMD_FM1];
		c->list_all.clear();
		for(int k = 0; k < LEAF_N; ++k)
			c->leaf[k] = append_range(c->list_all, leaf[k]);
		c->depth_ranges.assign(maxdepth + 1, DepthRange());
		for(int d = 0; d <= maxdepth; ++d) {
			DepthRange &r = c->depth_ranges[d];
			r.driver = append_range(c->list_all, bydepth[d].first);
			r.fbd = append_range(c->list_all, fbd_bydepth[d]);
			r.fbdpan = append_range(c->list_all, fbdpan_bydepth[d]);
			r.generic = append_range(c->list_all, bydepth[d].second);
		}
		if(int r = grow(c, c->d_list, c->list_all.size() + 64, 1, false)) return r;
		if(int r = grow(c, c->d_staged, c->d_list.cap, 1, false)) return r;
		if(!c->list_all.empty())
			HIPCHK(c, hipMemcpyAsync(c->d_list.d, c->list_all.data(), c->list_all.size() * sizeof(int),
					hipMemcpyHostToDevice, c->stream));
		c->lists_dirty = false;
		c->owners_all_driver = owners_ok && root_driver;
		if(!c->vm.list.empty() || c->vm.stats.live)
			c->vm.list_dirty = true;
	}
	if(int r = vm_build_lists(c))
		return r;
	std::vector<int> dyn_all;
	{
		std::vector<int> dyn[DYN_N];
		std::vector<std::vector<int>> dyn_bus(c->depth_ranges.size()), fbdpan_win(c->depth_ranges.size());
		const bool no_recs_kernel = (c->sw.no_fast & 64) != 0;
		for(int vi : c->with_recs) {
			HVoice &v = c->voices[vi];
			if(c->sw.vm_dump)
				for(const A2DRec &r : v.recs)
					fprintf(stderr, "REC %lld v%d f%u op%u u%u r%u val %d dur %u start %u\n", c->serial_base, vi,
							A2D_RFRAG(r.head), A2D_ROP(r.head), A2D_RUNIT(r.head), A2D_RREG(r.head), r.value, r.dur, r.start);
			if(v.cls == CLS_OSCPAN || v.cls == CLS_NOISEPAN || v.cls == CLS_OSCFILTPAN || v.cls == CLS_NOISEFILTPAN || v.cls == CLS_OSC2PAN ||
					v.cls == CLS_OSC2FILTPAN) {
				const bool ok = !no_recs_kernel && !v.mode_mix && !v.fancy_recs;
				if(v.cls == CLS_OSC2FILTPAN)
					v.dynf2_run = c->serial_base;
				dyn[ok ? cls_lists[v.cls].dyn : DYN_REST].push_back(vi);
			} else if(v.cls == CLS_OSCBARE || v.cls == CLS_OSC3FILTPAN) {
				dyn[DYN_REST].push_back(vi);
			} else if((v.cls == CLS_BUSDRIVER || v.cls == CLS_FBDCHAIN || v.cls == CLS_FBDPAN) && v.depth < (int)dyn_bus.size()) {
				if(v.cls == CLS_FBDPAN && !c->sw.bus_windows && !(c->sw.no_fast & 512) && v.depth > 0 && v.vm < 0 && v.resolved) {
					const int rows = seg_rows(v.recs.data(), v.recs.size(), c->fragframes, c->nfrags);
					a2amd_bus_windows_info &bw = c->last_buswin;
					if(rows > 0 && rows <= FBW_MAXWIN) {
						fbdpan_win[v.depth].push_back(vi);
						++bw.fbdpan_voices;
						bw.fbdpan_gliding += v.moving_until > c->vm.batch_time;
						bw.fbdpan_windows += (uint32_t)rows;
						continue;
					}
					bw.refused_tiling += rows < 0;
					bw.refused_cap += rows > FBW_MAXWIN;
				}
				dyn_bus[v.depth].push_back(vi);
				if(c->sw.hosttiming_level >= 3 && !v.recs.empty())
					fprintf(stderr, "a2amd: bus voice %d (depth %d, class %d) carries %zu records, first: frag %u op %u unit %u reg %u value %d\n",
							vi, v.depth, v.cls, v.recs.size(), A2D_RFRAG(v.recs[0].head), A2D_ROP(v.recs[0].head),
							A2D_RUNIT(v.recs[0].head), A2D_RREG(v.recs[0].head), v.recs[0].value);
			}
		}
		for(int vi : c->vm.o2f_voices) {
			HVoice &v = c->voices[vi];
			if(v.dynf2_run == c->serial_base || v.cls != CLS_OSC2FILTPAN || !(v.live || v.dying) || v.vm < 0)
				continue;
			v.dynf2_run = c->serial_base;
			dyn[DYN_FILT2].push_back(vi);
		}
		const ListRange o2f = c->leaf[LEAF_OSC2FILTPAN];
		c->o2f_quiet = o2f.count >= c->sw.o2f_min;
		if(!c->o2f_quiet)
			for(int k = 0; k < o2f.count; ++k) {
				const int vi = c->list_all[o2f.first + k];
				HVoice &v = c->voices[vi];
				if(v.dynf2_run == c->serial_base || v.mode_mix)
					continue;
				v.dynf2_run = c->serial_base;
				dyn[DYN_FILT2].push_back(vi);
			}
		auto by_bus_dyn = [&](int a, int b) { return c->voices[a].out_off < c->voices[b].out_off; };
		for(int k = 0; k < DYN_N; ++k) {
			if(!std::is_sorted(dyn[k].begin(), dyn[k].end(), by_bus_dyn))
				std::stable_sort(dyn[k].begin(), dyn[k].end(), by_bus_dyn);
			c->dyn[k] = append_range(dyn_all, dyn[k]);
		}
		c->consume_ok = c->owners_all_driver;
		for(size_t d = 0; d < dyn_bus.size(); ++d) {
			c->depth_ranges[d].dyn = append_range(dyn_all, dyn_bus[d]);
			if(!dyn_bus[d].empty())
				c->consume_ok = false;
			c->depth_ranges[d].fbdpan_win = append_range(dyn_all, fbdpan_win[d]);
		}
		a2amd_bus_info &bi = c->last_bus;
		bi = a2amd_bus_info{};
// ... 649 lines not shown
			return false;
	return c->dyn[DYN_REST].first + c->dyn[DYN_REST].count == 0;
}

struct LeafPass {
	A2DCommitSet *pend;
	hipEvent_t e1;
	bool use_win;
	bool solo;
	bool done;
};

static int launch_leaves(a2amd_ctx *c, LeafPass &lp)
{
	if(lp.done)
		return 0;
	lp.done = true;
	A2DCommitSet &pend = *lp.pend;
	const int *const list = c->d_list.d;
	auto none_quiet = [&](int k, int nleaf) {
		return (c->sw.vmskip & (k == 2 ? 2 : 1)) && c->vm.spec_use && !c->vm.list.empty() && c->vm.n_cls[k] == nleaf && c->vm.spec_idle[k] == 0;
	};
	const ListRange oscpan = c->leaf[LEAF_OSCPAN];
	if(oscpan.count && none_quiet(0, oscpan.count)) {
		if(lp.solo && lp.e1)
			HIPCHK(c, hipEventRecord(lp.e1, c->stream));
		++c->vm.quiet_skipped;
	} else if(oscpan.count) {
		int vpw, ysplit;
		pick_fast_shape(c->sw, oscpan.count, c->nfrags, &vpw, &ysplit);
		if(a2d_launch_leaf_oscpan(c->d_params, c->hparams, list + oscpan.first, oscpan.count,
				vpw, ysplit, c->d_ustage.d, c->d_staged.d + oscpan.first, c->stream, lp.solo ? (void *)lp.e1 : nullptr,
				&pend.c[pend.n]))
			return c->fail(A2AMD_EHIP, "fast leaf launch failed: %s", hipGetErrorString(hipGetLastError()));
		if(pend.c[pend.n].nlist)
			++pend.n;
		++c->stats.launches;
		c->vm.last.quiet_launched[0] = 1;
	}
	const ListRange noisepan = c->leaf[LEAF_NOISEPAN];
	if(noisepan.count && !c->noise_st.empty() && c->n_noise_quiet) {
		const int vpw = c->sw.nzvpw_set ? c->sw.nzvpw : (noisepan.count + 1023) / 1024;
		if(a2d_launch_leaf_noisepan(c->d_params, c->hparams, list + noisepan.first, noisepan.count, vpw, c->stream))
			return c->fail(A2AMD_EHIP, "noise leaf launch failed: %s", hipGetErrorString(hipGetLastError()));
		++c->stats.launches;
		c->last_noise.quiet_launched = 1;
	}
	const ListRange noisefilt = c->leaf[LEAF_NOISEFILTPAN];
	if(noisefilt.count && !c->noise_st.empty() && c->n_noise_filt_quiet) {
		const int vpg = c->sw.nzfvpg_set ? c->sw.nzfvpg : (noisefilt.count + 255) / 256;
		if(a2d_launch_leaf_noisefiltpan(c->d_params, c->hparams, list + noisefilt.first, noisefilt.count, vpg, c->stream))
			return c->fail(A2AMD_EHIP, "noise filter leaf launch failed: %s", hipGetErrorString(hipGetLastError()));
		++c->stats.launches;
		c->last_noise_filter.quiet_launched = 1;
	}
	const ListRange bare = c->leaf[LEAF_OSCBARE];
	if(bare.count && c->n_bare_quiet) {
		const int vpw = std::min(std::max(c->sw.vpw_set ? c->sw.vpw : (bare.count + 1023) / 1024, 1), 64);
		if(a2d_launch_leaf_oscbare(c->d_params, c->hparams, list + bare.first, bare.count, vpw, c->stream))
			return c->fail(A2AMD_EHIP, "bare oscillator leaf launch failed: %s", hipGetErrorString(hipGetLastError()));
		++c->stats.launches;
		c->last_bare.launched = 1;
		c->last_bare.vpw = (uint32_t)vpw;
	}
	const ListRange o3f = c->leaf[LEAF_OSC3FILTPAN];
	if(o3f.count && c->n_o3f_quiet) {
		const int vpg = std::min(std::max(c->sw.f2vpw ? c->sw.f2vpw : (o3f.count + 255) / 256, 1), 64);
		if(a2d_launch_leaf_osc3filtpan(c->d_params, c->hparams, list + o3f.first, o3f.count, vpg, c->stream))
			return c->fail(A2AMD_EHIP, "3-osc filter leaf launch failed: %s", hipGetErrorString(hipGetLastError()));
		++c->stats.launches;
		c->last_osc3filt.launched = 1;
		c->last_osc3filt.vpg = (uint32_t)vpg;
		c->last_osc3filt.workgroups = (uint32_t)((o3f.count + vpg - 1) / vpg);
	}
	const ListRange osc2pan = c->leaf[LEAF_OSC2PAN];
	if(osc2pan.count && none_quiet(1, osc2pan.count))
		++c->vm.quiet_skipped;
	else if(osc2pan.count) {
		int vpw, ysplit;
		pick_fast_shape(c->sw, osc2pan.count, c->nfrags * A2D_FAST_FCH / A2D_OSC2_FCH, &vpw, &ysplit, 16);
		const int voice_major = !(c->sw.debug & 16);
		const int lds_taps = !(c->sw.debug & (1 << 17));
		const int tame = !(c->sw.debug & (1 << 18));
		if(a2d_launch_leaf_osc2pan(c->d_params, c->hparams, list + osc2pan.first, osc2pan.count,
				vpw, ysplit, c->d_ustage.d, c->d_staged.d + osc2pan.first, c->stream, &pend.c[pend.n], voice_major, lds_taps, tame, c->d_tame_count, &ysplit))
			return c->fail(A2AMD_EHIP, "2-osc leaf launch failed: %s", hipGetErrorString(hipGetLastError()));
		c->last_osc2.launched = 1;
		c->last_osc2.voices = (uint32_t)osc2pan.count;
		c->last_osc2.vpw = (uint32_t)std::min(std::max(vpw, 1), 64);
		c->last_osc2.ysplit = (uint32_t)ysplit;
		c->last_osc2.voice_major = (uint32_t)voice_major;
		if(pend.c[pend.n].nlist)
			++pend.n;
		++c->stats.launches;
		c->vm.last.quiet_launched[1] = 1;
	}
	const ListRange oscfilt = c->leaf[LEAF_OSCFILTPAN];
	if(oscfilt.count && none_quiet(2, oscfilt.count))
		++c->vm.quiet_skipped;
	else if(oscfilt.count) {
		const int nf = oscfilt.count;
		int vpw = c->sw.fvpw_set ? c->sw.fvpw : std::min(std::max((nf + 255) / 256, 1), 64);
		if(a2d_launch_leaf_oscfiltpan(c->d_params, c->hparams, list + oscfilt.first, nf, vpw, c->stream))
			return c->fail(A2AMD_EHIP, "filter leaf launch failed: %s", hipGetErrorString(hipGetLastError()));
		++c->stats.launches;
		c->vm.last.quiet_launched[2] = 1;
	}
	const ListRange o2f = c->leaf[LEAF_OSC2FILTPAN];
	if(o2f.count && c->o2f_quiet) {
		const int nf = o2f.count;
		const int maxv = a2d_osc2filtpan_max_vpg();
		const int rounds = std::max(1, (nf + 256 * maxv - 1) / (256 * maxv));
		const int vpg = c->sw.f2vpw ? c->sw.f2vpw : std::min(std::max((nf + 256 * rounds - 1) / (256 * rounds), 1), maxv);
		if(a2d_launch_leaf_osc2filtpan(c->d_params, c->hparams, list + o2f.first, nf, vpg, c->stream))
			return c->fail(A2AMD_EHIP, "2-osc filter leaf launch failed: %s", hipGetErrorString(hipGetLastError()));
		++c->stats.launches;
		c->last_batch.o2f_launched = 1;
		c->last_batch.o2f_voices = (uint32_t)nf;
		c->last_batch.o2f_max_vpg = (uint32_t)maxv;
		c->last_batch.o2f_vpg = (uint32_t)std::min(std::max(vpg, 1), 64);
	}
	const ListRange fm = c->leaf[LEAF_FMPAN];
	int fm_kinds = 0;
	for(int k = 0; k < 8; ++k)
		fm_kinds += c->fm_kind_count[k] != 0;
	if(fm_kinds > 1 && fm.count <= 16384 && !c->sw.fmvpw_set) {
		if(a2d_launch_leaf_fmpan_all(c->d_params, c->hparams, list + fm.first, c->fm_kind_count, (fm.count + 1023) / 1024, c->stream))
			return c->fail(A2AMD_EHIP, "fm leaf launch failed: %s", hipGetErrorString(hipGetLastError()));
		++c->stats.launches;
	} else {
		for(int k = 0, at = fm.first; k < 8; at += c->fm_kind_count[k++]) {
			const int n = c->fm_kind_count[k];
			if(!n)
				continue;
			int vpw = c->sw.fmvpw_set ? c->sw.fmvpw : (n + 1023) / 1024;
			vpw = std::min(std::max(vpw, 1), 64);
			if(a2d_launch_leaf_fmpan(c->d_params, c->hparams, A2AMD_FM1 + k, list + at, n, vpw, c->stream))
				return c->fail(A2AMD_EHIP, "fm leaf launch failed: %s", hipGetErrorString(hipGetLastError()));
			++c->stats.launches;
		}
	}
	const ListRange gen = c->leaf[LEAF_GENERIC];
	if(gen.count) {
		if(a2d_launch_voices(c->d_params, list + gen.first, gen.count, pick_vpw(gen.count), c->stream))
			return c->fail(A2AMD_EHIP, "leaf launch failed: %s", hipGetErrorString(hipGetLastError()));
		++c->stats.launches;
	}
	if(!lp.use_win) {
		static const int nosc[4] = { 1, 2, 1, 2 }, filt[4] = { 0, 0, 1, 1 };
		const int *lists[4];
		int counts[4], total = 0, kinds = 0;
		for(int k = 0; k < 4; ++k) {
			lists[k] = c->d_dyn + c->dyn[k].first;
			counts[k] = c->dyn[k].count;
			total += counts[k];
			kinds += counts[k] != 0;
		}
		c->last_batch.recs_voices = (uint32_t)total;
		if(!c->vm.list.empty())
			c->last_batch.recs_voices += (uint32_t)(c->vm.n_cls[0] + c->vm.n_cls[1] + c->vm.n_cls[2]);
		if(kinds > 1 && total <= 4096 && !c->sw.rvpw_set) {
			if(a2d_launch_leaf_recs_all(c->sw, c->d_params, c->hparams, lists, counts, 1, c->stream, c->o2f_quiet ? 8 : 0))
				return c->fail(A2AMD_EHIP, "leaf records launch failed: %s", hipGetErrorString(hipGetLastError()));
			++c->stats.launches;
		} else {
			for(int k = 0; k < 4; ++k)
				if(int r = launch_recs(c, nosc[k], filt[k], lists[k], counts[k], k == DYN_FILT2 && c->o2f_quiet))
					return r;
		}
		if(!c->vm.list.empty()) {
			const int *l = c->vm.d_list.d + c->vm.list.size();
			for(int k = 0; k < 3; l += c->vm.n_cls[k++])
				if(int r = launch_recs(c, nosc[k], filt[k], l, c->vm.n_cls[k], 1))
					return r;
		}
	}
	const ListRange rest = c->dyn[DYN_REST];
	if(rest.count > 0) {
		if(a2d_launch_voices(c->d_params, c->d_dyn + rest.first, rest.count, pick_vpw(rest.count), c->stream))
			return c->fail(A2AMD_EHIP, "leaf launch failed: %s", hipGetErrorString(hipGetLastError()));
		++c->stats.launches;
	}
	return 0;
}

static int issue_leaf_phase(a2amd_ctx *c, bool consume, bool consume_sub, hipEvent_t e0, hipEvent_t e1, A2DCommitSet *pend)
{
	const bool selfclean = consume || consume_sub;
	if(c->capturing ? !selfclean : !(selfclean && c->others_clean && c->root_clean))
		HIPCHK(c, hipMemsetAsync(c->d_busmem.d, 0, c->bus_used * sizeof(int32_t), c->stream));
	c->others_clean = selfclean;
	c->root_clean = consume;
	if(e0)
		HIPCHK(c, hipEventRecord(e0, c->stream));
	bool use_win;
	{
		int nwinv = 0;
		for(int k = DYN_OSC1; k <= DYN_FILT2; ++k)
			nwinv += c->dyn[k].count;
		for(int k = 0; k < 3; ++k)
			nwinv += c->vm.list.empty() ? 0 : c->vm.n_cls[k];
		use_win = c->sw.win >= 0 ? c->sw.win != 0 : nwinv >= c->sw.win_min;
	}
	const bool vmwin_ok = c->sw.vmwin;
	if(int r = vm_issue(c, use_win && vmwin_ok && !c->vm.fused_off))
		return r;
	c->last_batch = a2amd_batch_info{};
	c->last_batch.o2f_class = (uint32_t)c->leaf[LEAF_OSC2FILTPAN].count;
	c->last_batch.o2f_listed = (uint32_t)c->dyn[DYN_FILT2].count;
	c->last_batch.n_moving_listed = (uint32_t)c->n_moving_listed;
	c->last_batch.general_voices = (uint32_t)c->dyn[DYN_REST].count;
	c->last_noise = a2amd_noise_batch_info{};
	c->last_noise.class_voices = (uint32_t)c->leaf[LEAF_NOISEPAN].count;
	c->last_noise.standin_voices = c->n_noise_standin;
	c->last_noise.quiet_voices = c->n_noise_quiet;
	c->last_noise_filter = a2amd_noise_filter_batch_info{};
	c->last_noise_filter.class_voices = (uint32_t)c->leaf[LEAF_NOISEFILTPAN].count;
	c->last_noise_filter.quiet_voices = c->n_noise_filt_quiet;
	c->last_noise_filter.min_voices = (uint32_t)c->sw.nzf_min;
	c->last_bare = a2amd_bare_batch_info{};
	c->last_bare.class_voices = (uint32_t)c->leaf[LEAF_OSCBARE].count;
	c->last_bare.quiet_voices = c->n_bare_quiet;
	c->last_bare.gliding_voices = c->n_bare_gliding;
	c->last_bare.record_voices = c->n_bare_records;
	c->last_bare.mono_drivers = c->n_mono_drivers;
	c->last_osc3filt = a2amd_osc3filt_batch_info{};
	c->last_osc3filt.class_voices = (uint32_t)c->leaf[LEAF_OSC3FILTPAN].count;
	c->last_osc3filt.quiet_voices = c->n_o3f_quiet;
	c->last_osc3filt.gliding_voices = c->n_o3f_gliding;
	c->last_osc3filt.record_voices = c->n_o3f_records;
	c->last_osc2 = a2amd_osc2_batch_info{};
	LeafPass lp = { pend, e1, use_win, oscpan_alone(c), false };
	const std::function<int()> mid = [&]() -> int {
		if(!c->sw.vmspec_early || !vmwin_ok || !vm_spec_wanted(c))
			return 0;
		if(int r = launch_leaves(c, lp))
			return r;
		flush_commits(c, pend);
		return vm_speculate(c);
	};
	if(use_win) {
		if(int r = issue_windows(c, c->d_dyn, c->dyn, mid))
			return r;
		if(vmwin_ok)
			if(int r = vm_predict(c))
				return r;
	}
	if(int r = launch_leaves(c, lp))
		return r;
	if(e1 && !lp.solo)
		HIPCHK(c, hipEventRecord(e1, c->stream));
	if(use_win && vmwin_ok && !c->vm.spec_launched_now && vm_spec_wanted(c)) {
		flush_commits(c, pend);
		if(int r = vm_speculate(c))
			return r;
	}
	vm_note_batch(c, use_win && vmwin_ok);
	return 0;
}

int issue_kernels(a2amd_ctx *c, unsigned phases, hipEvent_t e0, hipEvent_t e1, hipEvent_t e2)
{
	const bool has_sub = (phases & A2AMD_RENDER_SUBTREES) != 0, has_root = (phases & A2AMD_RENDER_ROOT) != 0;
	const bool consume = c->consume_ok && has_sub && has_root;
	const bool consume_sub = c->consume_ok && has_sub && !has_root;
	A2DCommitSet pend;
	pend.n = 0;
	pend.c[0].nlist = pend.c[1].nlist = 0;
	if(phases & A2AMD_RENDER_SUBTREES) {
		if(c->sub_resume < 0)
			if(int r = issue_leaf_phase(c, consume, consume_sub, e0, e1, &pend))
				return r;
		const int dstart = c->sub_resume >= 0 ? c->sub_resume : (int)c->depth_ranges.size() - 1;
		c->sub_resume = -1;
		c->paused_at = 0;
		for(int d = dstart; d >= 1; --d) {
			if(int r = launch_depth(c, d, consume ? 3 : consume_sub ? 1 : 0, &pend))
				return r;
			if((phases & A2AMD_RENDER_TAPS) && depth_has_mutes(c, d)) {
				c->paused_at = d;
				c->sub_resume = d > 1 ? d - 1 : -1;
				break;
			}
		}
		if(!(phases & A2AMD_RENDER_ROOT))
			flush_commits(c, &pend);
	}
	if(phases & A2AMD_RENDER_ROOT) {
		const bool root_stores = consume || c->consume_ok;
		if(!has_sub && !root_stores)
			HIPCHK(c, hipMemsetAsync(c->d_busmem.d, 0,
					(size_t)c->nfrags * c->cfg.channels * A2D_FRAG * sizeof(int32_t), c->stream));
		if(!c->depth_ranges.empty())
			if(int r = launch_depth(c, 0, root_stores ? 3 : 0, &pend))
				return r;
		if(!has_sub && root_stores)
			c->root_clean = true;
		flush_commits(c, &pend);
		if(e2)
			HIPCHK(c, hipEventRecord(e2, c->stream));
		c->stats.fragments += c->nfrags;
		c->stats.voice_fragments += (uint64_t)c->nfrags * (uint64_t)c->list_all.size();
	}
	return 0;
}

void drop_graphs(a2amd_ctx *c)
{
	for(int i = 0; i < 12; ++i) {
		if(c->gexec[i]) {
			hipGraphExecDestroy(c->gexec[i]);
			c->gexec[i] = nullptr;
		}
		if(c->graph[i]) {
// ... 53 lines not shown
```

### audiality2_amd/csrc/a2amd_taps.h

```cpp
#pragma once
#include <hip/hip_runtime.h>
#include <stdint.h>
#include "a2amd_device.h"
#include "a2amd_dsp.h"
#include "a2amd_fm.h"

#define FAST_WPB   4
#define FAST_FCH   A2D_FAST_FCH

#define WRL(reg, val) reg = me ? (val) : reg

DEV int hermite_step(int v, unsigned ph)
{
	int p;
	asm("v_mul_i32_i24_sdwa %0, %1, %2 dst_sel:DWORD dst_unused:UNUSED_PAD src0_sel:DWORD src1_sel:BYTE_0"
			: "=v"(p) : "v"(v), "v"(ph));
	return __builtin_amdgcn_sbfe(p, 8, 17);
}

DEV int hermite4(int dm, int d0, int d1, int d2, unsigned ph)
{
	int c = (d1 - dm) >> 1;
	int a = (3 * (d0 - d1) + d2 - dm) >> 1;
	int b = dm - d0 + c - a;
	a = hermite_step(a, ph);
	a = hermite_step(a + b, ph);
	return d0 + hermite_step(a + c, ph);
}

struct __attribute__((packed, aligned(2))) Quad16 { uint32_t lo, hi; };

DEV int inter_quads(const Quad16 qa, const Quad16 qb, unsigned ph, unsigned ph2)
{
	int h0 = hermite4((int16_t)(qa.lo & 0xffff), (int)qa.lo >> 16, (int16_t)(qa.hi & 0xffff), (int)qa.hi >> 16, ph);
	int h1 = hermite4((int16_t)(qb.lo & 0xffff), (int)qb.lo >> 16, (int16_t)(qb.hi & 0xffff), (int)qb.hi >> 16, ph2);
	return h0 + h1;
}

DEV int inter_dwords(const int16_t *d, unsigned ph, unsigned dph16)
{
	const unsigned ph2 = ph + (dph16 >> 1);
	const Quad16 qa = *(const Quad16 *)(d + (int)(ph >> 8) - 1);
	const Quad16 qb = *(const Quad16 *)(d + (int)(ph2 >> 8) - 1);
	return inter_quads(qa, qb, ph, ph2);
}

typedef int Coef4 __attribute__((ext_vector_type(3)));
#define A2D_COEF_LOAD "llvm.amdgcn.struct.buffer.load.v3i32"
typedef int CoefRsrc __attribute__((ext_vector_type(4)));
extern "C" __device__ Coef4 a2d_coef_load(CoefRsrc rsrc, int vindex, int voffset, int soffset, int aux)
		__asm(A2D_COEF_LOAD);

DEV CoefRsrc coef_rsrc(const int *wavecoef)
{
	const uint64_t b = (uint64_t)wavecoef;
	CoefRsrc r;
	r.x = rfl((int)(unsigned)b);
	r.y = rfl((int)(((unsigned)(b >> 32) & 0xffffu) | ((4u * A2D_COEF_WORDS) << 16)));
	r.z = -1;
	r.w = 0x00020000;
	return r;
}

DEV int coef_base(unsigned doff) { return (int)(doff * (4u * A2D_COEF_WORDS)); }

DEV int hermite_ct(const Coef4 k, unsigned ph)
{
	int t = hermite_step(k.x, ph);
	t = hermite_step(wadd(t, k.y), ph);
	return hermite_step(wadd(t, k.z >> 16), ph);
}

DEV int inter_coefs(const Coef4 ka, unsigned pa, const Coef4 kb, unsigned pb)
{
	int d;
	asm("v_add_u32_sdwa %0, sext(%1), sext(%2) dst_sel:DWORD dst_unused:UNUSED_PAD src0_sel:WORD_0 src1_sel:WORD_0"
			: "=v"(d) : "v"(ka.z), "v"(kb.z));
	return wadd(wadd(d, hermite_ct(ka, pa)), hermite_ct(kb, pb));
}

DEV int frac_x(unsigned ph)
{
	int x;
	const int seven = 7;
	asm("v_lshlrev_b32_sdwa %0, %1, %2 dst_sel:DWORD dst_unused:UNUSED_PAD src0_sel:DWORD src1_sel:BYTE_0"
			: "=v"(x) : "v"(seven), "v"(ph));
	return x;
}
// ... 84 lines not shown

DEV void stage_level4(LdsInt *level, const int *wavecoef4, int cb, unsigned size, int lane)
{
	const Coef4x *src = (const Coef4x *)(wavecoef4 + ((unsigned)cb >> 2));
	LdsCoef4x *dst = (LdsCoef4x *)level;
#pragma unroll
	for(int r = 0; r < A2D_OSC2_LDS_ENT / 64; ++r) {
		const unsigned i = (unsigned)(r * 64 + lane);
		if(i < size)
			dst[i] = src[i];
	}
}

DEV void lds_wave_fence()
{
	__builtin_amdgcn_fence(__ATOMIC_ACQ_REL, "wavefront");
	__builtin_amdgcn_wave_barrier();
}

DEV unsigned tap_phase(uint64_t ph, unsigned ldph)
{
	const unsigned lo = (unsigned)ph & 0xffffu, hi = (unsigned)(ph >> 16);
	return hi + ((lo + ldph) >> 16);
}

DEV unsigned lane_dph(int lane, unsigned dph)
{
	unsigned t = (unsigned)lane * dph;
	asm("" : "+v"(t));
	return t;
}

DEV int64_t div_trunc_exact(int64_t n, int d)
{
	int64_t q = (int64_t)((double)n / (double)d);
	const int64_t r = n - q * d;
	if(n >= 0) {
		if(r < 0) --q; else if(r >= d) ++q;
	} else {
		if(r > 0) ++q; else if(r <= -(int64_t)d) --q;
	}
	return q;
}


template<int N>
DEV void flush_acc(int *busmem, int off, int nch, int f0, int nf, int lane, int dbg,
		int (&acc0)[N], int (&acc1)[N])
{
#pragma unroll
	for(int j = 0; j < N; ++j) {
		if(j < nf && off >= 0 && !(dbg & 1)) {
			int *dst = busmem + off + (size_t)(f0 + j) * nch * A2D_FRAG;
			if(acc0[j])
				atomicAdd(&dst[lane], acc0[j]);
			if(acc1[j])
				atomicAdd(&dst[A2D_FRAG + lane], acc1[j]);
		}
		acc0[j] = 0;
		acc1[j] = 0;
	}
}

DEV void tile_add(int *w, int x)
{
	(void)__hip_atomic_fetch_add(w, x, __ATOMIC_RELAXED, __HIP_MEMORY_SCOPE_WAVEFRONT);
}

DEV void flush_tile(int *busmem, int off, int nch, int f0, int nf, int nrows, int lane, int dbg, int (*tile)[2][A2D_FRAG])
{
	for(int r = 0; r < nrows; ++r) {
		const int a0 = tile[r][0][lane], a1 = tile[r][1][lane];
		tile[r][0][lane] = 0;
		tile[r][1][lane] = 0;
		if(r < nf && off >= 0 && !(dbg & 1)) {
			int *dst = busmem + off + (size_t)(f0 + r) * nch * A2D_FRAG;
			if(a0)
				atomicAdd(&dst[lane], a0);
			if(a1)
				atomicAdd(&dst[A2D_FRAG + lane], a1);
		}
	}
}
```

### audiality2_amd/replay.py

```python
import ctypes as C
import gzip
import lzma

import numpy as np

T_FRAGMENT, T_INIT, T_DEINIT, T_WRITE, T_PROCESS, T_INLINE_END, T_WAVE, T_CONFIG, T_WAVEDROP = range(1, 10)
MIPLEVELS = 10
WAVEPRE = 1
WAVEPOST = 131


class Trace:

    def __init__(self, path):
        opener = gzip.open if str(path).endswith(".gz") else lzma.open if str(path).endswith(".xz") else open
        with opener(path, "rb") as f:
            raw = f.read()
        words = np.frombuffer(raw[: len(raw) // 4 * 4], dtype="<i4")
        self.records = []
        self.waves = {}
        self.config = None
        i = 0
        n = len(words)
        while i + 8 <= n:
# ... 15 lines not shown
                                       sizes=[int(s) for s in sizes], data=data)
                self.records.append((T_WAVE, wid, 0, 0, 0, 0, 0, 0))
            elif op == T_CONFIG:
                self.config = dict(samplerate=r[1], basepitch=r[2], channels=r[3],
                                   buffer=r[4], noiseseed=r[5] & 0xFFFFFFFF)
            else:
                self.records.append(r)
        if self.config is None:
            raise ValueError("trace without CONFIG record")
        self.kinds = {r[1]: r[3] for r in self.records if r[0] == T_INIT}

    @property
    def total_frames(self):
        return sum(r[1] for r in self.records if r[0] == T_FRAGMENT)


class a2amd_config(C.Structure):
    _fields_ = [("struct_size", C.c_uint32), ("samplerate", C.c_int32),
                ("basepitch", C.c_int32), ("channels", C.c_int32),
                ("device", C.c_int32), ("max_batch", C.c_uint32),
                ("stream", C.c_void_p)]


class a2amd_wavedesc(C.Structure):
    _fields_ = [("type", C.c_int32), ("flags", C.c_uint32), ("period", C.c_uint32),
                ("size", C.c_uint32 * MIPLEVELS),
                ("data", C.POINTER(C.c_int16) * MIPLEVELS)]


class a2amd_noise_batch_info(C.Structure):
    _fields_ = [("quiet_launched", C.c_uint32), ("quiet_voices", C.c_uint32),
                ("class_voices", C.c_uint32), ("standin_voices", C.c_uint32)]

    def __repr__(self):
        return "noise_batch_info(" + ", ".join(f"{n}={getattr(self, n)}" for n, _ in self._fields_) + ")"


class a2amd_noise_filter_batch_info(C.Structure):
    _fields_ = [("quiet_launched", C.c_uint32), ("quiet_voices", C.c_uint32),
                ("class_voices", C.c_uint32), ("min_voices", C.c_uint32)]

    def __repr__(self):
        return "noise_filter_batch_info(" + ", ".join(f"{n}={getattr(self, n)}" for n, _ in self._fields_) + ")"


class a2amd_sweep_batch_info(C.Structure):
    _fields_ = [("pass_launched", C.c_uint32), ("filters", C.c_uint32),
                ("ramp_windows", C.c_uint32), ("standin_voices", C.c_uint32)]

    def __repr__(self):
        return "sweep_batch_info(" + ", ".join(f"{n}={getattr(self, n)}" for n, _ in self._fields_) + ")"


class a2amd_bus_info(C.Structure):
    _fields_ = [(n, C.c_uint32) for n in ("driver_voices", "driver_ramping", "driver_windows_dropped", "fbd_voices",
                                          "generic_voices", "consume", "master_direct")]

    def __repr__(self):
        return "bus_info(" + ", ".join(f"{n}={getattr(self, n)}" for n, _ in self._fields_) + ")"


class a2amd_bare_batch_info(C.Structure):
    _fields_ = [(n, C.c_uint32) for n in ("launched", "class_voices", "quiet_voices", "gliding_voices", "record_voices",
                                          "vpw", "mono_drivers", "reserved")]

    def __repr__(self):
        return "bare_batch_info(" + ", ".join(f"{n}={getattr(self, n)}" for n, _ in self._fields_) + ")"


class a2amd_osc3filt_batch_info(C.Structure):
    _fields_ = [(n, C.c_uint32) for n in ("launched", "class_voices", "quiet_voices", "gliding_voices", "record_voices",
                                          "vpg", "workgroups", "reserved")]

    def __repr__(self):
        return "osc3filt_batch_info(" + ", ".join(f"{n}={getattr(self, n)}" for n, _ in self._fields_) + ")"


class a2amd_osc2_batch_info(C.Structure):
    _fields_ = [(n, C.c_uint32) for n in ("launched", "voices", "vpw", "ysplit", "voice_major", "superchunks_voice_major",
                                          "superchunks_chunk_major", "reserved")] + [("chunk_major_mask", C.c_uint64)]

    def __repr__(self):
        return "osc2_batch_info(" + ", ".join(f"{n}={getattr(self, n)}" for n, _ in self._fields_) + ")"


class a2amd_fbdpan_batch_info(C.Structure):
    _fields_ = [(n, C.c_uint32) for n in ("launched", "class_voices", "quiet_voices", "gliding_voices", "record_voices",
                                          "max_delays")] + [("reserved", C.c_uint32 * 2)]

    def __repr__(self):
        return "fbdpan_batch_info(" + ", ".join(f"{n}={getattr(self, n)}" for n, _ in self._fields_[:-1]) + ")"


class a2amd_bus_windows_info(C.Structure):
    _fields_ = [(n, C.c_uint32) for n in ("fbd_dropped", "fbdpan_voices", "fbdpan_gliding", "fbdpan_windows", "refused_tiling",
                                          "refused_cap", "window_cap", "launched")]

    def __repr__(self):
        return "bus_windows_info(" + ", ".join(f"{n}={getattr(self, n)}" for n, _ in self._fields_) + ")"


class a2amd_vm_batch_info(C.Structure):
    _fields_ = [("listed", C.c_uint32), ("class_voices", C.c_uint32 * 3), ("other_voices", C.c_uint32),
                ("pending", C.c_uint32), ("fused", C.c_uint32), ("not_fused", C.c_uint32),
                ("spec_valid", C.c_uint32), ("spec_taken", C.c_uint32), ("spec_miss", C.c_uint32),
                ("spec_next", C.c_uint32), ("spec_why_not", C.c_uint32), ("records", C.c_uint32),
                ("idle_known", C.c_uint32), ("idle", C.c_uint32 * 3), ("quiet_launched", C.c_uint32 * 3)]

    def __repr__(self):
        return ("vm_batch_info(" + ", ".join(f"{n}={list(getattr(self, n)) if n in ('class_voices', 'idle', 'quiet_launched') else getattr(self, n)}"
                                             for n, _ in self._fields_) + ")")


class a2amd_wave_pool_info(C.Structure):
    _fields_ = [(n, C.c_uint64) for n in ("used", "capacity", "free_samples")] + \
               [(n, C.c_uint32) for n in ("coef4", "raw_waves", "reallocations", "regions_reused")]

    def __repr__(self):
        return "wave_pool_info(" + ", ".join(f"{n}={getattr(self, n)}" for n, _ in self._fields_) + ")"


class a2amd_vm_state(C.Structure):
    _fields_ = [("waketime", C.c_uint32), ("state", C.c_uint8), ("func", C.c_uint8), ("pc", C.c_uint16),
                ("r", C.c_int32 * 64)]


class Backend:

    def __init__(self, lib, prefix, samplerate, basepitch, channels=2, device=0,
                 max_batch=64, stream=None):
        self.lib, self.prefix, self.channels = lib, prefix, channels

        def fn(name, restype, *argtypes):
            f = getattr(lib, prefix + name)
            f.restype, f.argtypes = restype, list(argtypes)
            return f

        vp, i32, u32, u64 = C.c_void_p, C.c_int, C.c_uint, C.c_uint64
        self._open = fn("open", i32, C.POINTER(a2amd_config), C.POINTER(vp))
        self._close = fn("close", None, vp)
        self._err = fn("last_error", C.c_char_p, vp)
        self._wave_upload = fn("wave_upload", i32, vp, u64, C.POINTER(a2amd_wavedesc))
        self._wave_drop = fn("wave_drop", i32, vp, u64)
        self._fragment = fn("fragment", i32, vp, u32)
        self._unit_init = fn("unit_init", i32, vp, u64, i32, u32, i32, i32, i32, i32, u32)
        self._unit_deinit = fn("unit_deinit", i32, vp, i32)
        self._unit_write = fn("unit_write", i32, vp, i32, i32, i32, u32, u32, i32)
        self._unit_process = fn("unit_process", i32, vp, i32, u32, u32, C.POINTER(C.c_uint32))
        self._inline_end = fn("inline_end", i32, vp, i32)
        self._unit_clients = fn("unit_clients", i32, vp, i32, u32)
        self._unit_inject = fn("unit_inject", i32, vp, i32, u32, u32, C.POINTER(C.POINTER(C.c_int32)))
        self._unit_tapped = fn("unit_tapped", i32, vp, i32, u32, C.POINTER(C.POINTER(C.c_int32)))
        self._render = fn("render", i32, vp, u32, C.POINTER(C.POINTER(C.c_int32)), u32)
        self._set_pt = fn("set_pitch_table", i32, vp, C.POINTER(C.c_uint32))
        self._get_pt = fn("get_pitch_table", i32, vp, C.POINTER(C.c_uint32))
        self.has_walk = hasattr(lib, prefix + "voice_process")
        if self.has_walk:
            self._voice_process = fn("voice_process", i32, vp, i32, u32, u32, C.POINTER(C.c_uint32))
            self._voice_slot = fn("voice_slot", i32, vp, i32)
            self._default_map = fn("default_map", C.POINTER(C.c_uint8), vp, C.POINTER(u32))
        self._fragment_repeat_noise = None
        if hasattr(lib, prefix + "fragment_repeat_noise"):
            self._fragment_repeat_noise = fn("fragment_repeat_noise", i32, vp, u32, u32, C.POINTER(C.c_uint32))
        self._last_batch_noise = None
        if hasattr(lib, prefix + "last_batch_noise"):
            self._last_batch_noise = fn("last_batch_noise", i32, vp, C.POINTER(a2amd_noise_batch_info))
        self._last_batch_noise_filter = None
        if hasattr(lib, prefix + "last_batch_noise_filter"):
            self._last_batch_noise_filter = fn("last_batch_noise_filter", i32, vp, C.POINTER(a2amd_noise_filter_batch_info))
        self._fragment_repeat = None
        if hasattr(lib, prefix + "fragment_repeat"):
            self._fragment_repeat = fn("fragment_repeat", i32, vp, u32, u32)
        self._last_batch_sweeps = None
        if hasattr(lib, prefix + "last_batch_sweeps"):
            self._last_batch_sweeps = fn("last_batch_sweeps", i32, vp, C.POINTER(a2amd_sweep_batch_info))
        self._last_batch_buses = None
        if hasattr(lib, prefix + "last_batch_buses"):
            self._last_batch_buses = fn("last_batch_buses", i32, vp, C.POINTER(a2amd_bus_info))
        self._last_batch_bare = None
        if hasattr(lib, prefix + "last_batch_bare"):
            self._last_batch_bare = fn("last_batch_bare", i32, vp, C.POINTER(a2amd_bare_batch_info))
        self._last_batch_osc3filt = None
        if hasattr(lib, prefix + "last_batch_osc3filt"):
            self._last_batch_osc3filt = fn("last_batch_osc3filt", i32, vp, C.POINTER(a2amd_osc3filt_batch_info))
        self._last_batch_osc2 = None
        if hasattr(lib, prefix + "last_batch_osc2"):
            self._last_batch_osc2 = fn("last_batch_osc2", i32, vp, C.POINTER(a2amd_osc2_batch_info))
        self._osc2_stage_rule = self._wave_level_periodic = None
        if hasattr(lib, prefix + "osc2_stage_rule"):
            self._osc2_stage_rule = fn("osc2_stage_rule", u32, u32, i32, u32, i32)
            self._wave_level_periodic = fn("wave_level_periodic", i32, C.POINTER(C.c_int16), u32)
        self._osc2_tame_rule = self._wave_level_tame = None
        if hasattr(lib, prefix + "osc2_tame_rule"):
            self._osc2_tame_rule = fn("osc2_tame_rule", u32, i32, i32)
            self._wave_level_tame = fn("wave_level_tame", i32, C.POINTER(C.c_int16), u32)
            self._osc2_tame_voices = fn("osc2_tame_voices", i32, vp, C.POINTER(C.c_uint64))
        if hasattr(lib, prefix + "wave_pool_info"):
            self._wave_pool_info = fn("wave_pool_info", i32, vp, C.POINTER(a2amd_wave_pool_info))

            def wave_pool_info():
                pi = a2amd_wave_pool_info()
                self._chk(self._wave_pool_info(self.ctx, C.byref(pi)), "wave_pool_info")
                return pi
            self.wave_pool_info = wave_pool_info
        self._last_batch_fbdpan = None
        if hasattr(lib, prefix + "last_batch_fbdpan"):
            self._last_batch_fbdpan = fn("last_batch_fbdpan", i32, vp, C.POINTER(a2amd_fbdpan_batch_info))
        self._last_batch_bus_windows = None
        if hasattr(lib, prefix + "last_batch_bus_windows"):
            self._last_batch_bus_windows = fn("last_batch_bus_windows", i32, vp, C.POINTER(a2amd_bus_windows_info))
        self.has_vm = hasattr(lib, prefix + "vm_adopt")
        if self.has_vm:
            self._fragment_offset = fn("fragment_offset", i32, vp, u32)
            self._vm_program = fn("vm_program", i32, vp, u64, C.POINTER(C.c_uint32), u32)
            self._vm_adopt = fn("vm_adopt", i32, vp, i32, i32, C.POINTER(a2amd_vm_state), C.POINTER(C.c_int32),
                                C.POINTER(C.c_uint8), C.c_uint32, C.c_uint32, vp, i32)
            self._vm_expect_cuts = fn("vm_expect_cuts", i32, vp, C.POINTER(C.c_uint32), i32)
            self._vm_recall = fn("vm_recall", i32, vp, C.POINTER(C.c_int32), u32, C.POINTER(a2amd_vm_state), vp)
        self._last_batch_vm = None
        if hasattr(lib, prefix + "last_batch_vm"):
            self._last_batch_vm = fn("last_batch_vm", i32, vp, C.POINTER(a2amd_vm_batch_info))
        self.has_capture = hasattr(lib, prefix + "wave_upload_captured_post")
        if self.has_capture:
            self._capture_begin = fn("capture_begin", i32, vp)
            self._capture_end = fn("capture_end", i32, vp, C.POINTER(vp))
            self._capture_frames = fn("capture_frames", u32, vp)
            self._capture_free = fn("capture_free", None, vp)
            self._wave_upload_captured = fn("wave_upload_captured", i32, vp, u64, C.POINTER(a2amd_wavedesc), vp)
            self._wave_upload_captured_post = fn("wave_upload_captured_post", i32, vp, u64, C.POINTER(a2amd_wavedesc), vp, u32)
            self._wave_stats = fn("wave_stats", i32, vp, C.POINTER(u64), C.POINTER(u32), C.POINTER(u32))
        cfg = a2amd_config(C.sizeof(a2amd_config), samplerate, basepitch, channels,
                           device, max_batch, stream)
        self.ctx = vp()
        rc = self._open(C.byref(cfg), C.byref(self.ctx))
        if rc != 0:
            raise RuntimeError(f"{prefix}open failed: {rc} "
                               f"{self._err(None).decode(errors='replace')}")
        self.noise = C.c_uint32(0)
        self._keep = []

    def close(self):
        if self.ctx:
            self._close(self.ctx)
            self.ctx = None

    def _chk(self, rc, what):
        if rc < 0:
            msg = self._err(self.ctx)
            raise RuntimeError(f"{self.prefix}{what}: {rc} {msg.decode(errors='replace') if msg else ''}")
        return rc

    def wave_upload(self, key, wtype, flags, period, sizes, data):
        d = a2amd_wavedesc()
        d.type, d.flags, d.period = wtype, flags, period
        for lv, arr in enumerate(data):
            arr = np.ascontiguousarray(arr, dtype=np.int16)
            self._keep.append(arr)
            d.size[lv] = sizes[lv]
            d.data[lv] = arr.ctypes.data_as(C.POINTER(C.c_int16))
        return self._chk(self._wave_upload(self.ctx, key, C.byref(d)), "wave_upload")

    def capture_begin(self):
        return self._chk(self._capture_begin(self.ctx), "capture_begin")

    def capture_end(self):
        cap = C.c_void_p()
        self._chk(self._capture_end(self.ctx, C.byref(cap)), "capture_end")
        return cap if cap.value else None

    def capture_frames(self, cap):
# ... 3 lines not shown
        self._capture_free(cap)

    def wave_upload_captured(self, key, wtype, flags, period, sizes, cap, chunk=None, check=True):
        d = a2amd_wavedesc()
        d.type, d.flags, d.period = wtype, flags, period
        for lv, n in enumerate(sizes):
            d.size[lv] = n
        if chunk is None:
            rc = self._wave_upload_captured(self.ctx, key, C.byref(d), cap)
        else:
            rc = self._wave_upload_captured_post(self.ctx, key, C.byref(d), cap, chunk)
        return self._chk(rc, "wave_upload_captured") if check else rc

    def wave_stats(self):
        h2d, up, res = C.c_uint64(), C.c_uint32(), C.c_uint32()
        self._chk(self._wave_stats(self.ctx, C.byref(h2d), C.byref(up), C.byref(res)), "wave_stats")
        return h2d.value, up.value, res.value

    def wave_drop(self, key):
        return self._chk(self._wave_drop(self.ctx, key), "wave_drop")

    def fragment(self, frames):
        return self._chk(self._fragment(self.ctx, frames), "fragment")

    def fragment_repeat(self, frames, count):
        if self._fragment_repeat is None:
            raise RuntimeError(f"this library has no {self.prefix}fragment_repeat")
        return self._chk(self._fragment_repeat(self.ctx, frames, count), "fragment_repeat")

    def last_batch_sweeps(self):
        if self._last_batch_sweeps is None:
            raise RuntimeError(f"this library has no {self.prefix}last_batch_sweeps")
        bi = a2amd_sweep_batch_info()
        self._chk(self._last_batch_sweeps(self.ctx, C.byref(bi)), "last_batch_sweeps")
        return bi

    def fragment_repeat_noise(self, frames, count):
        if self._fragment_repeat_noise is None:
            raise RuntimeError(f"this library has no {self.prefix}fragment_repeat_noise")
        return self._chk(self._fragment_repeat_noise(self.ctx, frames, count, C.byref(self.noise)),
                         "fragment_repeat_noise")

    def last_batch_noise(self):
        if self._last_batch_noise is None:
            raise RuntimeError(f"this library has no {self.prefix}last_batch_noise")
        bi = a2amd_noise_batch_info()
        self._chk(self._last_batch_noise(self.ctx, C.byref(bi)), "last_batch_noise")
        return bi

    def last_batch_noise_filter(self):
        if self._last_batch_noise_filter is None:
            raise RuntimeError(f"this library has no {self.prefix}last_batch_noise_filter")
        bi = a2amd_noise_filter_batch_info()
        self._chk(self._last_batch_noise_filter(self.ctx, C.byref(bi)), "last_batch_noise_filter")
        return bi

    def last_batch_buses(self):
        if self._last_batch_buses is None:
            raise RuntimeError(f"this library has no {self.prefix}last_batch_buses")
        bi = a2amd_bus_info()
        self._chk(self._last_batch_buses(self.ctx, C.byref(bi)), "last_batch_buses")
        return bi

    def last_batch_bare(self):
        if self._last_batch_bare is None:
            raise RuntimeError(f"this library has no {self.prefix}last_batch_bare")
        bi = a2amd_bare_batch_info()
        self._chk(self._last_batch_bare(self.ctx, C.byref(bi)), "last_batch_bare")
        return bi

    def last_batch_osc3filt(self):
        if self._last_batch_osc3filt is None:
            raise RuntimeError(f"this library has no {self.prefix}last_batch_osc3filt")
        bi = a2amd_osc3filt_batch_info()
        self._chk(self._last_batch_osc3filt(self.ctx, C.byref(bi)), "last_batch_osc3filt")
        return bi

    def last_batch_osc2(self):
        if self._last_batch_osc2 is None:
            raise RuntimeError(f"this library has no {self.prefix}last_batch_osc2")
        bi = a2amd_osc2_batch_info()
        self._chk(self._last_batch_osc2(self.ctx, C.byref(bi)), "last_batch_osc2")
        return bi

    def osc2_stage_rule(self, size0, periodic0, size1, periodic1):
        if self._osc2_stage_rule is None:
            raise RuntimeError(f"this library has no {self.prefix}osc2_stage_rule")
        return int(self._osc2_stage_rule(size0, int(bool(periodic0)), size1, int(bool(periodic1))))

    def osc2_tame_rule(self, tame0, tame1):
        if self._osc2_tame_rule is None:
            raise RuntimeError(f"this library has no {self.prefix}osc2_tame_rule")
        return int(self._osc2_tame_rule(int(bool(tame0)), int(bool(tame1))))

    def osc2_tame_voices(self):
        if self._osc2_tame_rule is None:
            raise RuntimeError(f"this library has no {self.prefix}osc2_tame_voices")
        n = C.c_uint64(0)
        self._chk(self._osc2_tame_voices(self.ctx, C.byref(n)), "osc2_tame_voices")
        return int(n.value)

    def wave_level_tame(self, level, size=None):
        if self._wave_level_tame is None:
            raise RuntimeError(f"this library has no {self.prefix}wave_level_tame")
        arr = np.ascontiguousarray(level, dtype=np.int16)
        n = len(arr) - WAVEPRE - WAVEPOST if size is None else size
        return bool(self._wave_level_tame(arr.ctypes.data_as(C.POINTER(C.c_int16)), n))

    def wave_level_periodic(self, level):
        if self._wave_level_periodic is None:
            raise RuntimeError(f"this library has no {self.prefix}wave_level_periodic")
        arr = np.ascontiguousarray(level, dtype=np.int16)
        return bool(self._wave_level_periodic(arr.ctypes.data_as(C.POINTER(C.c_int16)), len(arr) - WAVEPRE - WAVEPOST))

    def last_batch_fbdpan(self):
        if self._last_batch_fbdpan is None:
            raise RuntimeError(f"this library has no {self.prefix}last_batch_fbdpan")
        bi = a2amd_fbdpan_batch_info()
        self._chk(self._last_batch_fbdpan(self.ctx, C.byref(bi)), "last_batch_fbdpan")
        return bi

    def last_batch_bus_windows(self):
        if self._last_batch_bus_windows is None:
            raise RuntimeError(f"this library has no {self.prefix}last_batch_bus_windows")
        bi = a2amd_bus_windows_info()
        self._chk(self._last_batch_bus_windows(self.ctx, C.byref(bi)), "last_batch_bus_windows")
        return bi

    def last_batch_vm(self):
        if self._last_batch_vm is None:
            raise RuntimeError(f"this library has no {self.prefix}last_batch_vm")
        bi = a2amd_vm_batch_info()
        self._chk(self._last_batch_vm(self.ctx, C.byref(bi)), "last_batch_vm")
        return bi

    def fragment_offset(self, offset):
        return self._chk(self._fragment_offset(self.ctx, offset), "fragment_offset")

    def vm_program(self, key, words):
        code = (C.c_uint32 * len(words))(*[w & 0xffffffff for w in words])
        return self._chk(self._vm_program(self.ctx, key, code, len(words)), "vm_program")

    def vm_adopt(self, head_unit, prog, state, wires, now, msdur, check=True):
        wu = (C.c_int32 * 64)(*([-1] * 64))
        wr = (C.c_uint8 * 64)()
        for r, (u, ureg) in wires.items():
            wu[r], wr[r] = u, ureg
        rc = self._vm_adopt(self.ctx, head_unit, prog, C.byref(state), wu, wr, now & 0xffffffff, msdur, None, 0)
        return self._chk(rc, "vm_adopt") if check else rc

    def vm_expect_cuts(self, when):
        arr = (C.c_uint32 * max(len(when), 1))(*[w & 0xffffffff for w in when])
        return self._chk(self._vm_expect_cuts(self.ctx, arr, len(when)), "vm_expect_cuts")

    def vm_recall(self, head_units):
        n = len(head_units)
        out = (a2amd_vm_state * n)()
        self._chk(self._vm_recall(self.ctx, (C.c_int32 * n)(*head_units), n, out, None), "vm_recall")
        return list(out)

    def last_error(self):
        msg = self._err(self.ctx)
        return msg.decode(errors="replace") if msg else ""

    def unit_init(self, voice_key, kind, flags, nin, nout, wired, transpose=0, wakefrac=0):
        return self._chk(self._unit_init(self.ctx, voice_key, kind, flags, nin, nout, wired,
# ... 130 lines not shown
```

### include/a2amd.h

```cpp
#ifndef A2AMD_H
#define A2AMD_H

#include <stdint.h>

#ifdef __cplusplus
extern "C" {
#endif

#define A2AMD_MAXFRAG      64
#define A2AMD_MAXCHANNELS   8
#define A2AMD_MIPLEVELS    10
#define A2AMD_WAVEPRE       1
#define A2AMD_WAVEPOST    131
#define A2AMD_MAXCHAIN     16

typedef struct a2amd_ctx a2amd_ctx;

typedef enum a2amd_errors {
	A2AMD_OK = 0,
	A2AMD_ENODEVICE   = -1,
	A2AMD_EINVAL      = -2,
	A2AMD_ENOMEM      = -3,
	A2AMD_EUNSUPPORTED= -4,
	A2AMD_ESTATE      = -5,
// ... 97 lines not shown
#define A2AMD_XIO_MUTE    4u
int  a2amd_unit_clients(a2amd_ctx *ctx, int unit, unsigned mode);
int  a2amd_unit_insertable(a2amd_ctx *ctx, int unit);
int  a2amd_render_paused(a2amd_ctx *ctx);
int  a2amd_unit_insert(a2amd_ctx *ctx, int unit, unsigned fragment, unsigned offset, unsigned frames,
		const int32_t *const *bufs);
int  a2amd_unit_inject(a2amd_ctx *ctx, int unit, unsigned offset, unsigned frames,
		const int32_t *const *bufs);
int  a2amd_unit_tapped(a2amd_ctx *ctx, int unit, unsigned fragment, const int32_t **bufs);

int  a2amd_inline_end(a2amd_ctx *ctx, int unit);

#define A2AMD_RENDER_SUBTREES 1u
#define A2AMD_RENDER_ROOT     2u
#define A2AMD_RENDER_UPLOAD   4u
#define A2AMD_RENDER_READBACK 8u
#define A2AMD_RENDER_TAPS     64u
#define A2AMD_RENDER_KEEP    16u
#define A2AMD_RENDER_ASYNC   32u
#define A2AMD_RENDER_EXCHANGE 128u
#define A2AMD_RENDER_ALL     15u
int  a2amd_render(a2amd_ctx *ctx, unsigned phases, int32_t *const *out,
		unsigned out_capacity_frames);
int  a2amd_collect(a2amd_ctx *ctx, int32_t *const *out, unsigned out_capacity_frames);
int  a2amd_replay(a2amd_ctx *ctx, unsigned steps);
int  a2amd_rootbus(a2amd_ctx *ctx, void **devptr, uint64_t *bytes);
int  a2amd_rootbus_copy(a2amd_ctx *ctx, void *stage, int to_stage);

int  a2amd_dist_unique_id(void *id128);
int  a2amd_dist_init(a2amd_ctx *ctx, const void *id128, int rank, int nranks);
int  a2amd_dist_init_local(a2amd_ctx *const *ctxs, int n);
int  a2amd_render_group(a2amd_ctx *const *ctxs, int n, unsigned phases, int32_t *const *out,
		unsigned out_capacity_frames);

int  a2amd_fragment_repeat(a2amd_ctx *ctx, unsigned frames, unsigned count);


typedef struct a2amd_stats {
	uint64_t fragments;
	uint64_t voice_fragments;
	uint64_t records;
	uint64_t launches;
	double   last_kernel_ms;
	double   last_leaf_ms;
	uint32_t live_units, live_voices, live_waves, reserved;
	double   timed_leaf_ms;
	double   timed_all_ms;
	uint64_t timed_batches;
} a2amd_stats;
int  a2amd_get_stats(a2amd_ctx *ctx, a2amd_stats *st);
int  a2amd_set_profiling(a2amd_ctx *ctx, int on);
typedef struct a2amd_batch_info {
	uint32_t o2f_launched;
	uint32_t o2f_voices;
	uint32_t o2f_vpg;
	uint32_t o2f_max_vpg;
	uint32_t o2f_class;
	uint32_t o2f_listed;
	uint32_t recs_voices;
	uint32_t win_voices;
	uint32_t win_slabs;
	uint32_t n_moving_listed;
	uint32_t general_voices;
} a2amd_batch_info;
int  a2amd_last_batch(const a2amd_ctx *ctx, a2amd_batch_info *bi);

#ifdef __cplusplus
}
#endif

#include "a2amd_noise.h"
#include "a2amd_noisepan.h"
#include "a2amd_noisefilt.h"
#include "a2amd_sweep.h"
#include "a2amd_bus.h"
#include "a2amd_wavepost.h"
#include "a2amd_oscbare.h"
#include "a2amd_fbdpan.h"
#include "a2amd_buswin.h"
#include "a2amd_vmbatch.h"
#include "a2amd_osc2.h"
#include "a2amd_osc2lds.h"
#include "a2amd_osc2tame.h"
#include "a2amd_osc3filt.h"
#include "a2amd_wavepool.h"

#endif
```

Before: 571.7 billion voice-samples/s.

## Add specialized tame 2-osc leaf kernel that claims simple wavefronts before general kernel

```diff
diff --git a/audiality2_amd/build.py b/audiality2_amd/build.py
--- a/audiality2_amd/build.py
+++ b/audiality2_amd/build.py
@@ -56,11 +56,11 @@
 def build_lib(force=False):
     csrc = os.path.join(HERE, "csrc")
     srcs = [os.path.join(csrc, f) for f in ("a2amd_host.cpp", "a2amd_sched.cpp", "a2amd_render.cpp", "a2amd_dist.cpp",
-                                            "a2amd_vm.cpp", "a2amd_kernels.hip", "a2amd_fast.hip", "a2amd_vm.hip", "a2amd_wavecap.hip", "a2amd_wavepost.hip", "a2amd_win.hip", "a2amd_vmwin.hip", "a2amd_noise.hip", "a2amd_noisepan.hip", "a2amd_noisefiltpan.hip", "a2amd_cutsweep.hip", "a2amd_oscbare.hip", "a2amd_osc3filtpan.hip")]
+                                            "a2amd_vm.cpp", "a2amd_kernels.hip", "a2amd_fast.hip", "a2amd_vm.hip", "a2amd_wavecap.hip", "a2amd_wavepost.hip", "a2amd_win.hip", "a2amd_vmwin.hip", "a2amd_noise.hip", "a2amd_noisepan.hip", "a2amd_noisefiltpan.hip", "a2amd_cutsweep.hip", "a2amd_oscbare.hip", "a2amd_osc3filtpan.hip", "a2amd_osc2tame.hip")]
     deps = srcs + [os.path.join(csrc, "a2amd_host.h"), os.path.join(csrc, "a2amd_switches.h"), os.path.join(csrc, "a2amd_device.h"), os.path.join(csrc, "a2amd_dsp.h"),
                    os.path.join(csrc, "a2amd_fm.h"), os.path.join(csrc, "a2amd_vmcore.h"), os.path.join(csrc, "a2amd_taps.h"), os.path.join(csrc, "a2amd_winctl.h"), os.path.join(csrc, "a2amd_vmdev.h"), os.path.join(csrc, "a2amd_noisemap.h"), os.path.join(csrc, "a2amd_noisevoice.h"), os.path.join(csrc, "a2amd_settled.h"), os.path.join(csrc, "a2amd_quiet.h"), os.path.join(csrc, "a2amd_cutsweep.h"), os.path.join(csrc, "a2amd_filt.h"), os.path.join(csrc, "a2amd_wavepads.h"), os.path.join(csrc, "a2amd_wavetame.h"), os.path.join(ROOT, "include", "a2amd.h"),
                    os.path.join(ROOT, "include", "a2amd_noise.h"), os.path.join(ROOT, "include", "a2amd_noisepan.h"), os.path.join(ROOT, "include", "a2amd_noisefilt.h"), os.path.join(ROOT, "include", "a2amd_sweep.h"), os.path.join(ROOT, "include", "a2amd_wavepost.h"),
-                   os.path.join(ROOT, "include", "a2amd_bus.h"), os.path.join(ROOT, "include", "a2amd_oscbare.h"), os.path.join(ROOT, "include", "a2amd_osc3filt.h"), os.path.join(ROOT, "include", "a2amd_fbdpan.h"), os.path.join(ROOT, "include", "a2amd_buswin.h"), os.path.join(ROOT, "include", "a2amd_vmbatch.h"), os.path.join(ROOT, "include", "a2amd_osc2.h"), os.path.join(ROOT, "include", "a2amd_osc2lds.h"), os.path.join(ROOT, "include", "a2amd_osc2tame.h"), os.path.join(ROOT, "include", "a2amd_wavepool.h"), os.path.join(ROOT, "include", "a2amd_vm.h")]
+                   os.path.join(ROOT, "include", "a2amd_bus.h"), os.path.join(ROOT, "include", "a2amd_oscbare.h"), os.path.join(ROOT, "include", "a2amd_osc3filt.h"), os.path.join(ROOT, "include", "a2amd_fbdpan.h"), os.path.join(ROOT, "include", "a2amd_buswin.h"), os.path.join(ROOT, "include", "a2amd_vmbatch.h"), os.path.join(ROOT, "include", "a2amd_osc2.h"), os.path.join(ROOT, "include", "a2amd_osc2lds.h"), os.path.join(ROOT, "include", "a2amd_osc2tame.h"), os.path.join(ROOT, "include", "a2amd_osc2tame_kernel.h"), os.path.join(ROOT, "include", "a2amd_wavepool.h"), os.path.join(ROOT, "include", "a2amd_vm.h")]
     out = os.path.join(HERE, "liba2amd.so")
     flags = ["--offload-arch=gfx950", "-O3", "-std=c++17", "-fPIC", "-shared", "-Wno-unused-value"]
     want = source_hash(deps, flags)
@@ -73,7 +73,7 @@
     src = os.path.join(HERE, "csrc", "a2amd_units.c")
     deps = [src, os.path.join(ROOT, "include", "a2amd.h"), os.path.join(ROOT, "include", "a2amd_noise.h"), os.path.join(ROOT, "include", "a2amd_noisepan.h"),
             os.path.join(ROOT, "include", "a2amd_noisefilt.h"), os.path.join(ROOT, "include", "a2amd_sweep.h"), os.path.join(ROOT, "include", "a2amd_bus.h"),
-            os.path.join(ROOT, "include", "a2amd_wavepost.h"), os.path.join(ROOT, "include", "a2amd_oscbare.h"), os.path.join(ROOT, "include", "a2amd_osc3filt.h"), os.path.join(ROOT, "include", "a2amd_fbdpan.h"), os.path.join(ROOT, "include", "a2amd_buswin.h"), os.path.join(ROOT, "include", "a2amd_vmbatch.h"), os.path.join(ROOT, "include", "a2amd_osc2.h"), os.path.join(ROOT, "include", "a2amd_osc2lds.h"), os.path.join(ROOT, "include", "a2amd_osc2tame.h"), os.path.join(ROOT, "include", "a2amd_wavepool.h"), os.path.join(ROOT, "include", "a2amd_plugin.h"),
+            os.path.join(ROOT, "include", "a2amd_wavepost.h"), os.path.join(ROOT, "include", "a2amd_oscbare.h"), os.path.join(ROOT, "include", "a2amd_osc3filt.h"), os.path.join(ROOT, "include", "a2amd_fbdpan.h"), os.path.join(ROOT, "include", "a2amd_buswin.h"), os.path.join(ROOT, "include", "a2amd_vmbatch.h"), os.path.join(ROOT, "include", "a2amd_osc2.h"), os.path.join(ROOT, "include", "a2amd_osc2lds.h"), os.path.join(ROOT, "include", "a2amd_osc2tame.h"), os.path.join(ROOT, "include", "a2amd_osc2tame_kernel.h"), os.path.join(ROOT, "include", "a2amd_wavepool.h"), os.path.join(ROOT, "include", "a2amd_plugin.h"),
             os.path.join(ROOT, "include", "a2amd_walk.h"), os.path.join(ROOT, "include", "a2amd_vm.h")]
     out = os.path.join(HERE, "liba2amd_units.so")
     flags = ["-O2", "-Wall", "-fPIC", "-shared"]
diff --git a/audiality2_amd/csrc/a2amd_device.h b/audiality2_amd/csrc/a2amd_device.h
--- a/audiality2_amd/csrc/a2amd_device.h
+++ b/audiality2_amd/csrc/a2amd_device.h
@@ -226,6 +226,52 @@
 A2D_HD unsigned a2d_osc2_tame(unsigned tame0, unsigned tame1)
 {
 	return tame0 && tame1 ? 1u : 0u;
+}
+
+A2D_HD void a2d_osc2_shape(int *vpw, int *ysplit, bool can_stage)
+{
+	*vpw = *vpw < 1 ? 1 : (*vpw > 64 ? 64 : *vpw);
+	if(*ysplit < 1 || !can_stage)
+		*ysplit = 1;
+}
+
+#define A2D_OSC2TAME_MIN 1024
+A2D_HD bool a2d_osc2_all_whole(const unsigned *frames, int nfrags, int ysplit)
+{
+	if(nfrags <= 0 || ysplit < 1)
+		return false;
+	for(int slice = 0; slice < ysplit; ++slice) {
+		int c_lo, c_hi, nslices;
+		if(!a2d_osc2_slice(nfrags, ysplit, slice, &c_lo, &c_hi, &nslices))
+			break;
+		for(int s_lo = c_lo; s_lo < c_hi; s_lo += A2D_OSC2_SCH / A2D_OSC2_FCH) {
+			const int s_hi = s_lo + A2D_OSC2_SCH / A2D_OSC2_FCH < c_hi ? s_lo + A2D_OSC2_SCH / A2D_OSC2_FCH : c_hi;
+			const int fa = s_lo * A2D_OSC2_FCH, fb = s_hi * A2D_OSC2_FCH < nfrags ? s_hi * A2D_OSC2_FCH : nfrags;
+			unsigned n = 0;
+			for(int f = fa; f < fb; ++f)
+				n += frames[f];
+			if(!a2d_osc2_whole(0, n - frames[fb - 1], frames[fb - 1], fb - fa))
+				return false;
+		}
+	}
+	return true;
+}
+A2D_HD bool a2d_osc2tame_voice(unsigned records, bool osc0, bool osc1, bool pan, bool waves, unsigned tame0, unsigned tame1,
+		unsigned size0, unsigned size1, unsigned dph0, unsigned dph1, uint64_t ph0, uint64_t ph1, unsigned frames)
+{
+	if(records || !(osc0 && osc1 && pan && waves) || !a2d_osc2_tame(tame0, tame1))
+		return false;
+	if(!size0 || (size0 & (size0 - 1)) || !size1 || (size1 & (size1 - 1)))
+		return false;
+	if((ph0 >> 48) || (ph1 >> 48))
+		return false;
+	if(((ph0 + (uint64_t)frames * dph0) >> 48) || ((ph1 + (uint64_t)frames * dph1) >> 48))
+		return false;
+	return !((((uint64_t)size0 << 24) + (uint64_t)A2D_FRAG * dph0) >> 48) && !((((uint64_t)size1 << 24) + (uint64_t)A2D_FRAG * dph1) >> 48);
+}
+A2D_HD bool a2d_osc2tame_wave(unsigned long long ok, int nv)
+{
+	return nv >= 1 && nv <= 64 && ok == (nv == 64 ? ~0ull : (1ull << nv) - 1);
 }
 
 #ifdef __HIPCC__
@@ -333,7 +379,10 @@
 int a2d_launch_scatter_runs(const int *didx, const A2DRun *dval, int n, A2DRun *druns, void *stream);
 int a2d_launch_leaf_osc2pan(const A2DParams *dparams, const A2DParams &hp, const int *dlist, int nlist,
 		int vpw, int ysplit, int *ustage, unsigned char *staged, void *stream, A2DCommit *defer, int voice_major, int lds_taps,
-		int tame, unsigned long long *tame_count, int *ysplit_used);
+		int tame, unsigned long long *tame_count, int *ysplit_used, const unsigned char *taken = nullptr);
+int a2d_launch_leaf_osc2tame(const A2DParams *dparams, const A2DParams &hp, const int *dlist, int nlist, int vpw, int ysplit,
+		int *ustage, unsigned char *staged, void *stream, int lds_taps, unsigned long long *tame_count, unsigned char *taken,
+		unsigned long long *taken_count);
 struct A2Switches;
 int a2d_launch_leaf_recs(const A2Switches &sw, const A2DParams *dparams, const A2DParams &hp, int nosc, int filt, const int *dlist,
 		int nlist, int vpw, void *stream, int skip_empty = 0);
diff --git a/audiality2_amd/csrc/a2amd_fast.hip b/audiality2_amd/csrc/a2amd_fast.hip
--- a/audiality2_amd/csrc/a2amd_fast.hip
+++ b/audiality2_amd/csrc/a2amd_fast.hip
@@ -254,22 +254,6 @@
 
 enum { DV_SETTLED = 0, DV_MM, DV_DPH, DV_SIZEM, DV_DOFF, DV_V0, DV_V1, DV_NWORDS };
 
-DEV bool settled_wave(const A2DWave *w, unsigned dphase, int *d, bool settled = true, unsigned *periodic = nullptr,
-		unsigned *tame = nullptr)
-{
-	unsigned dph;
-	const unsigned mm = a2s_mip(dphase, w->period, &dph);
-	d[0] = (int)mm;
-	d[1] = (int)dph;
-	d[2] = (int)w->size[mm];
-	d[3] = (int)w->off[mm];
-	if(periodic)
-		*periodic = (w->periodic >> mm) & 1u;
-	if(tame)
-		*tame = (w->tame >> mm) & 1u;
-	return settled && a2s_wave_ok(w->size[0], w->flags, dph);
-}
-
 DEV void osc_from_mem(OscS &o, const volatile int *w)
 {
 	o.mode = rfl(w[OW_MODE]);
@@ -295,15 +279,6 @@
 	w[OW_PRAMPING] = o.p_ramping;
 	w[OW_P] = o.p.value; w[OW_P + 1] = o.p.target; w[OW_P + 2] = o.p.delta; w[OW_P + 3] = o.p.timer;
 	w[OW_A] = o.a.value; w[OW_A + 1] = o.a.target; w[OW_A + 2] = o.a.delta; w[OW_A + 3] = o.a.timer;
-}
-
-DEV void stage_mark(unsigned char *m, bool mine, bool settled, bool last_slice, bool walker)
-{
-	if(mine && !settled) {
-		if(walker)
-			*m = A2D_STAGED_FULL;
-	} else if(last_slice)
-		*m = mine ? A2D_STAGED_PHASES : A2D_STAGED_NONE;
 }
 
 #define OSC1_WPE 4
@@ -857,13 +832,15 @@
 		const int16_t *__restrict__ wavepool, const A2DWave *__restrict__ waves,
 		const uint32_t *__restrict__ ptab, int *__restrict__ busmem, const int *__restrict__ wavecoef,
 		unsigned char *__restrict__ staged, int vmajor, int lds_taps, const int *__restrict__ wavecoef4, int tame,
-		unsigned long long *__restrict__ tame_count)
+		unsigned long long *__restrict__ tame_count, const unsigned char *__restrict__ taken)
 {
 	const A2DParams &p = *pp;
 	const int wv = rfl((int)(threadIdx.x >> 6));
 	const int lane = threadIdx.x & 63;
 	const int first = (blockIdx.x * FAST_WPB + wv) * vpw;
 	if(first >= nlist)
+		return;
+	if(taken && taken[blockIdx.x * FAST_WPB + wv])
 		return;
 	const int nv = min(vpw, nlist - first);
 	const int nfrags = p.nfrags;
@@ -2962,13 +2939,11 @@
 
 int a2d_launch_leaf_osc2pan(const A2DParams *dparams, const A2DParams &hp, const int *dlist, int nlist,
 		int vpw, int ysplit, int *ustage, unsigned char *staged, void *stream, A2DCommit *defer, int voice_major, int lds_taps,
-		int tame, unsigned long long *tame_count, int *ysplit_used)
+		int tame, unsigned long long *tame_count, int *ysplit_used, const unsigned char *taken)
 {
 	if(nlist <= 0)
 		return 0;
-	vpw = vpw < 1 ? 1 : (vpw > 64 ? 64 : vpw);
-	if(ysplit < 1 || !ustage || !staged)
-		ysplit = 1;
+	a2d_osc2_shape(&vpw, &ysplit, ustage && staged);
 	if(ysplit_used)
 		*ysplit_used = ysplit;
 	int nwaves = (nlist + vpw - 1) / vpw;
@@ -2977,12 +2952,12 @@
 		hipLaunchKernelGGL(k_leaf_osc2pan<true>, dim3(nblocks, ysplit), dim3(64 * FAST_WPB), 0, (hipStream_t)stream,
 				dparams, dlist, nlist, vpw, ysplit, hp.voices, (const int *)hp.ustate,
 				ysplit > 1 ? ustage : hp.ustate, hp.wavepool, hp.waves, hp.ptab, hp.busmem, hp.wavecoef, staged, voice_major, lds_taps,
-				hp.wavecoef4, 1, tame_count);
+				hp.wavecoef4, 1, tame_count, taken);
 	else
 		hipLaunchKernelGGL(k_leaf_osc2pan<false>, dim3(nblocks, ysplit), dim3(64 * FAST_WPB), 0, (hipStream_t)stream,
 				dparams, dlist, nlist, vpw, ysplit, hp.voices, (const int *)hp.ustate,
 				ysplit > 1 ? ustage : hp.ustate, hp.wavepool, hp.waves, hp.ptab, hp.busmem, hp.wavecoef, staged, voice_major, lds_taps,
-				(const int *)nullptr, 0, (unsigned long long *)nullptr);
+				(const int *)nullptr, 0, (unsigned long long *)nullptr, taken);
 	if(ysplit > 1) {
 		A2DCommit cm = { dlist, nlist, 2, ustage, staged };
 		if(defer)
diff --git a/audiality2_amd/csrc/a2amd_host.cpp b/audiality2_amd/csrc/a2amd_host.cpp
--- a/audiality2_amd/csrc/a2amd_host.cpp
+++ b/audiality2_amd/csrc/a2amd_host.cpp
@@ -76,6 +76,8 @@
 	}
 	OPENCHK(hipMalloc((void **)&c->d_tame_count, sizeof(unsigned long long)));
 	OPENCHK(hipMemset(c->d_tame_count, 0, sizeof(unsigned long long)));
+	OPENCHK(hipMalloc((void **)&c->d_taken_count, sizeof(unsigned long long)));
+	OPENCHK(hipMemset(c->d_taken_count, 0, sizeof(unsigned long long)));
 #undef OPENCHK
 	*out = c;
 	return A2AMD_OK;
@@ -114,7 +116,7 @@
 	for(int k = 0; k < 5; ++k)
 		if(c->win_ev[k])
 			hipEventDestroy(c->win_ev[k]);
-	hipFree(c->d_waves.d); hipFree(c->d_wavepool.d); hipFree(c->d_wavecoef.d); hipFree(c->d_wavecoef4.d); hipFree(c->d_tame_count); hipFree(c->d_busmem.d);
+	hipFree(c->d_waves.d); hipFree(c->d_wavepool.d); hipFree(c->d_wavecoef.d); hipFree(c->d_wavecoef4.d); hipFree(c->d_tame_count); hipFree(c->d_taken_count); hipFree(c->d_osc2_taken.d); hipFree(c->d_busmem.d);
 	vm_close(c);
 	hipFree(c->capture.d); hipFree(c->capture.d_fragpos); hipFree(c->d_wavepost.d);
 	hipFree(c->d_fbdmem.d); hipFree(c->d_fmstate.d); hipFree(c->d_xio.d); hipFree(c->d_fmsine); hipFree(c->d_list.d); hipFree(c->d_staged.d); hipFree(c->d_scatter.d); hipFree(c->d_ptab); hipFree(c->d_blob.d);
diff --git a/audiality2_amd/csrc/a2amd_host.h b/audiality2_amd/csrc/a2amd_host.h
--- a/audiality2_amd/csrc/a2amd_host.h
+++ b/audiality2_amd/csrc/a2amd_host.h
@@ -410,6 +410,8 @@
 	a2amd_bare_batch_info last_bare = {};
 	uint32_t n_o3f_quiet = 0, n_o3f_gliding = 0, n_o3f_records = 0;
 	a2amd_osc3filt_batch_info last_osc3filt = {};
+	bool osc2quiet_hold = false;
+	a2amd_osc2quiet_batch_info last_osc2quiet = {};
 	a2amd_osc2_batch_info last_osc2 = {};
 	a2amd_fbdpan_batch_info last_fbdpan = {};
 	a2amd_bus_windows_info last_buswin = {};
@@ -447,6 +449,7 @@
 	DevBuf<int16_t> d_wavepool;
 	DevBuf<int32_t> d_wavecoef;
 	DevBuf<int32_t> d_wavecoef4;
+	unsigned long long *d_taken_count = nullptr;
 	unsigned long long *d_tame_count = nullptr;
 	DevBuf<int32_t> d_busmem;
 	DevBuf<int32_t> d_fbdmem;
@@ -454,6 +457,7 @@
 	DevBuf<int32_t> d_xio;
 	uint32_t *d_fmsine = nullptr;
 	DevBuf<int> d_list;
+	DevBuf<unsigned char> d_osc2_taken;
 	DevBuf<unsigned char> d_staged;
 	DevBuf<int> d_scatter;
 	uint32_t *d_ptab = nullptr;
diff --git a/audiality2_amd/csrc/a2amd_osc2tame.hip b/audiality2_amd/csrc/a2amd_osc2tame.hip
--- /dev/null
+++ b/audiality2_amd/csrc/a2amd_osc2tame.hip
@@ -0,0 +1,278 @@
+#include <hip/hip_runtime.h>
+#include "a2amd_device.h"
+#include "a2amd_dsp.h"
+#include "a2amd_settled.h"
+#include "a2amd_taps.h"
+
+#define O2T_FCH A2D_OSC2_FCH
+#define O2T_SCH A2D_OSC2_SCH
+#define O2T_WPE 4
+
+struct O2tVoice {
+	unsigned dph[2];
+	uint64_t mask[2];
+	int cb[2], amp[2];
+	uint64_t ph[2];
+};
+struct O2tLds {
+	const LdsInt *level[2];
+	unsigned m16[2];
+};
+
+template<int ST>
+DEV void o2t_chunk(const CoefRsrc &crs, O2tVoice &s, const unsigned (&ldph)[2], const O2tLds &lv, int (&xs)[O2T_FCH])
+{
+	constexpr int H = O2T_FCH / 2;
+	Coef4x ka[2][H], kb[2][H];
+	unsigned pa[2][O2T_FCH], pb[2][O2T_FCH];
+#pragma unroll
+	for(int o = 0; o < 2; ++o) {
+		const unsigned dph = s.dph[o];
+		uint64_t phs[O2T_FCH];
+#pragma unroll
+		for(int j = 0; j < O2T_FCH; ++j)
+			phs[j] = (s.ph[o] + (uint64_t)dph * (unsigned)(j * A2D_FRAG)) & s.mask[o];
+		s.ph[o] = phs[O2T_FCH - 1] + (uint64_t)dph * (unsigned)A2D_FRAG;
+#pragma unroll
+		for(int j = 0; j < O2T_FCH; ++j) {
+			pa[o][j] = tap_phase(phs[j], ldph[o]);
+			asm("" : "+v"(pa[o][j]));
+			pb[o][j] = pa[o][j] + (dph >> 17);
+		}
+	}
+	auto fetch = [&](int o, int h, int slot) {
+#pragma unroll
+		for(int j = 0; j < H; ++j) {
+			if((ST >> o) & 1) {
+				ka[slot][j] = coef4_lds(lv.level[o], pa[o][h * H + j], lv.m16[o]);
+				kb[slot][j] = coef4_lds(lv.level[o], pb[o][h * H + j], lv.m16[o]);
+			} else {
+				ka[slot][j] = coef4_at(crs, s.cb[o], pa[o][h * H + j]);
+				kb[slot][j] = coef4_at(crs, s.cb[o], pb[o][h * H + j]);
+			}
+		}
+	};
+	auto use = [&](int o, int h, int slot) {
+#pragma unroll
+		for(int j = 0; j < H; ++j) {
+			const int x = wadd(hermite_fused(ka[slot][j], pa[o][h * H + j]), hermite_fused(kb[slot][j], pb[o][h * H + j]));
+			const int y = mul64s(x, s.amp[o], 17);
+			xs[h * H + j] = o ? wadd(xs[h * H + j], y) : y;
+		}
+	};
+	fetch(0, 0, 0);
+	fetch(0, 1, 1);
+	__builtin_amdgcn_sched_barrier(0);
+	use(0, 0, 0);
+	__builtin_amdgcn_sched_barrier(0);
+	fetch(1, 0, 0);
+	__builtin_amdgcn_sched_barrier(0);
+	use(0, 1, 1);
+	__builtin_amdgcn_sched_barrier(0);
+	fetch(1, 1, 1);
+	__builtin_amdgcn_sched_barrier(0);
+	use(1, 0, 0);
+	use(1, 1, 1);
+}
+
+template<int ST>
+DEV void o2t_voice_chunks(const CoefRsrc &crs, O2tVoice &s, const unsigned (&ldph)[2], const O2tLds &lv, int nsc, int v0, int v1,
+		int lane, int (*tile)[2][A2D_FRAG])
+{
+	for(int k = 0; k < nsc; ++k) {
+		int xs[O2T_FCH];
+		o2t_chunk<ST>(crs, s, ldph, lv, xs);
+#pragma unroll
+		for(int j = 0; j < O2T_FCH; ++j) {
+			tile_add(&tile[k * O2T_FCH + j][0][lane], mul64s(xs[j], v0, 24));
+			tile_add(&tile[k * O2T_FCH + j][1][lane], mul64s(xs[j], v1, 24));
+		}
+	}
+}
+
+__global__ __launch_bounds__(64 * FAST_WPB) __attribute__((amdgpu_waves_per_eu(O2T_WPE, O2T_WPE)))
+void k_leaf_osc2tame(const A2DParams *__restrict__ pp, const int *__restrict__ list, int nlist, int vpw, int per,
+		const A2DVoice *__restrict__ voices, const int *ustate, int *ustage, const A2DWave *__restrict__ waves,
+		int *__restrict__ busmem, unsigned char *__restrict__ staged, int lds_taps, const int *__restrict__ wavecoef4,
+		unsigned long long *__restrict__ tame_count, unsigned char *__restrict__ taken,
+		unsigned long long *__restrict__ taken_count)
+{
+	const A2DParams &p = *pp;
+	const int wv = rfl((int)(threadIdx.x >> 6));
+	const int lane = threadIdx.x & 63;
+	const int w = blockIdx.x * FAST_WPB + wv;
+	const int first = w * vpw;
+	if(first >= nlist)
+		return;
+	const int nv = min(vpw, nlist - first);
+	const int nfrags = p.nfrags;
+	const int slice = blockIdx.y;
+	const int nchunks = (nfrags + O2T_FCH - 1) / O2T_FCH;
+	const int c_lo = slice * per, c_hi = min(c_lo + per, nchunks);
+	if(c_lo >= nchunks)
+		return;
+	const bool last_slice = c_hi * O2T_FCH >= nfrags;
+
+	int mm_l[2] = { 0, 0 }, dph_l[2] = { 0, 0 }, size_l[2] = { 0, 0 }, cb_l[2] = { 0, 0 }, amp_l[2] = { 0, 0 };
+	int phlo_l[2] = { 0, 0 }, phhi_l[2] = { 0, 0 };
+	int v0l = 0, v1l = 0, stage_l = 0, my_off = -1, my_nch = 2, uu[2] = { 0, 0 };
+	bool ok = false;
+	if(lane < nv) {
+		const int slot = list[first + lane];
+		const A2DVoice &vc = voices[slot];
+		my_off = vc.out_off;
+		my_nch = vc.out_nch;
+		bool osc[2];
+		int wave_l[2];
+		unsigned periodic[2] = { 0, 0 }, tame_lv[2] = { 0, 0 };
+		uint64_t phl[2] = { 0, 0 };
+#pragma unroll
+		for(int o = 0; o < 2; ++o) {
+			uu[o] = vc.unit[o];
+			const int *ws = ustate + (size_t)uu[o] * A2D_USTATE;
+			wave_l[o] = ws[OW_WAVE];
+			dph_l[o] = ws[OW_DPHASE];
+			amp_l[o] = ws[OW_A];
+			phlo_l[o] = ws[OW_PHASE_LO];
+			phhi_l[o] = ws[OW_PHASE_HI];
+			osc[o] = a2s_osc_settled(ws[OW_MODE], (unsigned)dph_l[o], ws[OW_PRAMPING], ws + OW_P, ws + OW_A);
+		}
+		const int *wp = ustate + (size_t)vc.unit[2] * A2D_USTATE;
+		int sp[8];
+#pragma unroll
+		for(int k = 0; k < 8; ++k)
+			sp[k] = wp[k];
+		const bool pan = a2s_arrived(sp + PW_VOL, sp + PW_PAN);
+		bool wok = false;
+		if(osc[0] && osc[1] && pan) {
+			wok = true;
+#pragma unroll
+			for(int o = 0; o < 2; ++o) {
+				int od[4];
+				wok = settled_wave(waves + wave_l[o], (unsigned)dph_l[o], od, wok, &periodic[o], &tame_lv[o]);
+				mm_l[o] = od[0];
+				dph_l[o] = od[1];
+				size_l[o] = od[2];
+				cb_l[o] = coef4_base((unsigned)od[3]);
+				phl[o] = ((uint64_t)(unsigned)phlo_l[o] | ((uint64_t)(unsigned)phhi_l[o] << 32)) >> mm_l[o];
+			}
+			a2s_pan_gains(sp[PW_VOL], sp[PW_PAN], a2s_pan_over(sp[PW_PAN]), &v0l, &v1l);
+		}
+		ok = wok && a2d_osc2tame_voice((unsigned)p.runs[slot].count, osc[0], osc[1], pan, wok, tame_lv[0], tame_lv[1],
+				(unsigned)size_l[0], (unsigned)size_l[1], (unsigned)dph_l[0], (unsigned)dph_l[1], phl[0], phl[1],
+				(unsigned)nfrags * A2D_FRAG);
+		if(ok) {
+			if(lds_taps)
+				stage_l = (int)a2d_osc2_stage((unsigned)size_l[0], periodic[0], (unsigned)size_l[1], periodic[1]);
+#pragma unroll
+			for(int o = 0; o < 2; ++o) {
+				phlo_l[o] = (int)(unsigned)phl[o];
+				phhi_l[o] = (int)(unsigned)(phl[o] >> 32);
+			}
+		}
+	}
+	const bool eligible = a2d_osc2tame_wave(__ballot(ok), nv);
+	if(slice == 0 && lane == 0) {
+		taken[w] = eligible ? 1 : 0;
+		if(eligible) {
+			atomicAdd(tame_count, (unsigned long long)nv);
+			atomicAdd(taken_count, 1ull);
+		}
+	}
+	if(!eligible)
+		return;
+
+	__shared__ int tiles[FAST_WPB][O2T_SCH][2][A2D_FRAG];
+	__shared__ __attribute__((aligned(16))) int levels[FAST_WPB][A2D_OSC2_LDS_ENT * 4];
+	int (*const tile)[2][A2D_FRAG] = tiles[wv];
+	LdsInt *const level = (LdsInt *)levels[wv];
+#pragma unroll
+	for(int r = 0; r < O2T_SCH; ++r)
+		tile[r][0][lane] = tile[r][1][lane] = 0;
+	const CoefRsrc crs = coef4_rsrc(wavecoef4);
+	const int dbg = p.debug;
+	for(int s_lo = c_lo; s_lo < c_hi; s_lo += O2T_SCH / O2T_FCH) {
+		const int s_hi = min(c_hi, s_lo + O2T_SCH / O2T_FCH);
+		const int fa = s_lo * O2T_FCH, nfs = min(nfrags, s_hi * O2T_FCH) - fa, nsc = s_hi - s_lo;
+		const unsigned before = (unsigned)fa * A2D_FRAG;
+		int cur_off = rdl(my_off, 0), cur_nch = rdl(my_nch, 0);
+		for(int v = 0; v < nv; ++v) {
+			const int voff = rdl(my_off, v);
+			if(voff != cur_off) {
+				flush_tile(busmem, cur_off, cur_nch, fa, nfs, nsc * O2T_FCH, lane, dbg, tile);
+				cur_off = voff;
+				cur_nch = rdl(my_nch, v);
+			}
+			const int v0 = rdl(v0l, v), v1 = rdl(v1l, v);
+			O2tVoice s;
+			unsigned ldph[2], size[2];
+#pragma unroll
+			for(int o = 0; o < 2; ++o) {
+				s.dph[o] = (unsigned)rdl(dph_l[o], v);
+				size[o] = (unsigned)rdl(size_l[o], v);
+				s.mask[o] = ((uint64_t)size[o] << 24) - 1;
+				s.cb[o] = rdl(cb_l[o], v);
+				s.amp[o] = rdl(amp_l[o], v);
+				s.ph[o] = ((uint64_t)(unsigned)rdl(phlo_l[o], v) | ((uint64_t)(unsigned)rdl(phhi_l[o], v) << 32)) +
+						(uint64_t)before * s.dph[o];
+				ldph[o] = lane_dph(lane, s.dph[o]);
+			}
+			O2tLds lv = { { level, level }, { 0, 0 } };
+			const int st = rdl(stage_l, v);
+			if(st) {
+				lds_wave_fence();
+				if(st & 1) {
+					lv.m16[0] = (size[0] - 1) << 4;
+					stage_level4(level, wavecoef4, s.cb[0], size[0], lane);
+				}
+				if(st & 2) {
+					LdsInt *const l1 = (st & 1) ? level + size[0] * 4 : level;
+					lv.level[1] = l1;
+					lv.m16[1] = (size[1] - 1) << 4;
+					stage_level4(l1, wavecoef4, s.cb[1], size[1], lane);
+				}
+				lds_wave_fence();
+			}
+			switch(st) {
+			case 0: o2t_voice_chunks<0>(crs, s, ldph, lv, nsc, v0, v1, lane, tile); break;
+			case 1: o2t_voice_chunks<1>(crs, s, ldph, lv, nsc, v0, v1, lane, tile); break;
+			case 2: o2t_voice_chunks<2>(crs, s, ldph, lv, nsc, v0, v1, lane, tile); break;
+			default: o2t_voice_chunks<3>(crs, s, ldph, lv, nsc, v0, v1, lane, tile); break;
+			}
+		}
+		flush_tile(busmem, cur_off, cur_nch, fa, nfs, nsc * O2T_FCH, lane, dbg, tile);
+	}
+
+	if(lane < nv && last_slice) {
+#pragma unroll
+		for(int o = 0; o < 2; ++o) {
+			const uint64_t dph = (unsigned)dph_l[o];
+			const uint64_t mask = ((uint64_t)(unsigned)size_l[o] << 24) - 1;
+			const uint64_t phl = (uint64_t)(unsigned)phlo_l[o] | ((uint64_t)(unsigned)phhi_l[o] << 32);
+			const uint64_t start = (phl + dph * ((uint64_t)(unsigned)(nfrags - 1) * A2D_FRAG)) & mask;
+			const uint64_t endph = (start + dph * A2D_FRAG) << mm_l[o];
+			int *ws = ustage + (size_t)uu[o] * A2D_USTATE;
+			ws[OW_PHASE_LO] = (int)(unsigned)endph;
+			ws[OW_PHASE_HI] = (int)(unsigned)(endph >> 32);
+		}
+	}
+	if(ustage != ustate && lane < nv)
+		stage_mark(staged + first + lane, true, true, last_slice, false);
+}
+
+int a2d_launch_leaf_osc2tame(const A2DParams *dparams, const A2DParams &hp, const int *dlist, int nlist, int vpw, int ysplit,
+		int *ustage, unsigned char *staged, void *stream, int lds_taps, unsigned long long *tame_count, unsigned char *taken,
+		unsigned long long *taken_count)
+{
+	if(nlist <= 0 || hp.nfrags <= 0)
+		return 0;
+	a2d_osc2_shape(&vpw, &ysplit, ustage && staged);
+	const int nwaves = (nlist + vpw - 1) / vpw;
+	const int nblocks = (nwaves + FAST_WPB - 1) / FAST_WPB;
+	int c_lo, c_hi, nslices;
+	a2d_osc2_slice(hp.nfrags, ysplit, 0, &c_lo, &c_hi, &nslices);
+	hipLaunchKernelGGL(k_leaf_osc2tame, dim3(nblocks, ysplit), dim3(64 * FAST_WPB), 0, (hipStream_t)stream,
+			dparams, dlist, nlist, vpw, c_hi - c_lo, hp.voices, (const int *)hp.ustate, ysplit > 1 ? ustage : hp.ustate, hp.waves,
+			hp.busmem, staged, lds_taps, hp.wavecoef4, tame_count, taken, taken_count);
+	return (int)hipGetLastError();
+}
diff --git a/audiality2_amd/csrc/a2amd_render.cpp b/audiality2_amd/csrc/a2amd_render.cpp
--- a/audiality2_amd/csrc/a2amd_render.cpp
+++ b/audiality2_amd/csrc/a2amd_render.cpp
@@ -538,6 +538,29 @@
 	return A2AMD_OK;
 }
 
+int a2amd_last_batch_osc2quiet(a2amd_ctx *c, a2amd_osc2quiet_batch_info *out)
+{
+	if(!c || !out)
+		return A2AMD_EINVAL;
+	use_device(c);
+	unsigned long long n = 0;
+	HIPCHK(c, hipStreamSynchronize(c->stream));
+	HIPCHK(c, hipMemcpy(&n, c->d_taken_count, sizeof(n), hipMemcpyDeviceToHost));
+	*out = c->last_osc2quiet;
+	out->taken_total = n;
+	return A2AMD_OK;
+}
+
+int a2amd_osc2quiet_hold(a2amd_ctx *c, int hold)
+{
+	if(!c)
+		return A2AMD_EINVAL;
+	if(c->osc2quiet_hold != (hold != 0))
+		drop_graphs(c);
+	c->osc2quiet_hold = hold != 0;
+	return A2AMD_OK;
+}
+
 int a2amd_last_batch_fbdpan(const a2amd_ctx *c, a2amd_fbdpan_batch_info *out)
 {
 	if(!c || !out)
diff --git a/audiality2_amd/csrc/a2amd_sched.cpp b/audiality2_amd/csrc/a2amd_sched.cpp
--- a/audiality2_amd/csrc/a2amd_sched.cpp
+++ b/audiality2_amd/csrc/a2amd_sched.cpp
@@ -364,6 +364,13 @@
 	return r;
 }
 
+static bool osc2_pair_wanted(const a2amd_ctx *c, const unsigned *frames, int nfrags)
+{
+	const int n = c->leaf[LEAF_OSC2PAN].count;
+	return n && !(c->sw.debug & ((1 << 18) | 16 | (1 << 19))) && c->hparams.wavecoef4 && !c->osc2quiet_hold &&
+			(n >= A2D_OSC2TAME_MIN || (c->sw.debug & (1 << 20))) && a2d_osc2_all_whole(frames, nfrags, 1);
+}
+
 int upload(a2amd_ctx *c)
 {
 	if(!c->cut_st.empty())
@@ -428,7 +435,8 @@
 				HIPCHK(c, hipEventRecord(c->blob_ev[bi], c->stream));
 				c->blob_busy[bi] = true;
 				c->hparams = p;
-				if(c->nfrags != c->blob_nfrags) {
+				if(c->nfrags != c->blob_nfrags ||
+						osc2_pair_wanted(c, c->fragframes, c->nfrags) != osc2_pair_wanted(c, c->blob_frames, c->nfrags)) {
 					drop_graphs(c);
 					c->quiet_streak = 0;
 				} else
@@ -774,6 +782,7 @@
 		}
 		if(int r = grow(c, c->d_list, c->list_all.size() + 64, 1, false)) return r;
 		if(int r = grow(c, c->d_staged, c->d_list.cap, 1, false)) return r;
+		if(int r = grow(c, c->d_osc2_taken, c->d_list.cap, 1, false)) return r;
 		if(!c->list_all.empty())
 			HIPCHK(c, hipMemcpyAsync(c->d_list.d, c->list_all.data(), c->list_all.size() * sizeof(int),
 					hipMemcpyHostToDevice, c->stream));
@@ -1589,12 +1598,23 @@
 		const int voice_major = !(c->sw.debug & 16);
 		const int lds_taps = !(c->sw.debug & (1 << 17));
 		const int tame = !(c->sw.debug & (1 << 18));
+		a2d_osc2_shape(&vpw, &ysplit, c->d_ustage.d && c->d_staged.d);
+		const bool pair = osc2_pair_wanted(c, c->fragframes, c->nfrags);
+		if(pair) {
+			if(a2d_launch_leaf_osc2tame(c->d_params, c->hparams, list + osc2pan.first, osc2pan.count, vpw, ysplit, c->d_ustage.d,
+					c->d_staged.d + osc2pan.first, c->stream, lds_taps, c->d_tame_count, c->d_osc2_taken.d, c->d_taken_count))
+				return c->fail(A2AMD_EHIP, "2-osc tame leaf launch failed: %s", hipGetErrorString(hipGetLastError()));
+			++c->stats.launches;
+			c->last_osc2quiet.launched = 1;
+			c->last_osc2quiet.wavefronts = (uint32_t)((osc2pan.count + vpw - 1) / vpw);
+		}
 		if(a2d_launch_leaf_osc2pan(c->d_params, c->hparams, list + osc2pan.first, osc2pan.count,
-				vpw, ysplit, c->d_ustage.d, c->d_staged.d + osc2pan.first, c->stream, &pend.c[pend.n], voice_major, lds_taps, tame, c->d_tame_count, &ysplit))
+				vpw, ysplit, c->d_ustage.d, c->d_staged.d + osc2pan.first, c->stream, &pend.c[pend.n], voice_major, lds_taps, tame, c->d_tame_count, &ysplit,
+				pair ? c->d_osc2_taken.d : nullptr))
 			return c->fail(A2AMD_EHIP, "2-osc leaf launch failed: %s", hipGetErrorString(hipGetLastError()));
 		c->last_osc2.launched = 1;
 		c->last_osc2.voices = (uint32_t)osc2pan.count;
-		c->last_osc2.vpw = (uint32_t)std::min(std::max(vpw, 1), 64);
+		c->last_osc2.vpw = (uint32_t)vpw;
 		c->last_osc2.ysplit = (uint32_t)ysplit;
 		c->last_osc2.voice_major = (uint32_t)voice_major;
 		if(pend.c[pend.n].nlist)
@@ -1737,6 +1757,7 @@
 	c->last_osc3filt.gliding_voices = c->n_o3f_gliding;
 	c->last_osc3filt.record_voices = c->n_o3f_records;
 	c->last_osc2 = a2amd_osc2_batch_info{};
+	c->last_osc2quiet = a2amd_osc2quiet_batch_info{};
 	LeafPass lp = { pend, e1, use_win, oscpan_alone(c), false };
 	const std::function<int()> mid = [&]() -> int {
 		if(!c->sw.vmspec_early || !vmwin_ok || !vm_spec_wanted(c))
diff --git a/audiality2_amd/csrc/a2amd_taps.h b/audiality2_amd/csrc/a2amd_taps.h
--- a/audiality2_amd/csrc/a2amd_taps.h
+++ b/audiality2_amd/csrc/a2amd_taps.h
@@ -4,6 +4,7 @@
 #include "a2amd_device.h"
 #include "a2amd_dsp.h"
 #include "a2amd_fm.h"
+#include "a2amd_settled.h"
 
 #define FAST_WPB   4
 #define FAST_FCH   A2D_FAST_FCH
@@ -254,3 +255,28 @@
 		}
 	}
 }
+
+DEV bool settled_wave(const A2DWave *w, unsigned dphase, int *d, bool settled = true, unsigned *periodic = nullptr,
+		unsigned *tame = nullptr)
+{
+	unsigned dph;
+	const unsigned mm = a2s_mip(dphase, w->period, &dph);
+	d[0] = (int)mm;
+	d[1] = (int)dph;
+	d[2] = (int)w->size[mm];
+	d[3] = (int)w->off[mm];
+	if(periodic)
+		*periodic = (w->periodic >> mm) & 1u;
+	if(tame)
+		*tame = (w->tame >> mm) & 1u;
+	return settled && a2s_wave_ok(w->size[0], w->flags, dph);
+}
+
+DEV void stage_mark(unsigned char *m, bool mine, bool settled, bool last_slice, bool walker)
+{
+	if(mine && !settled) {
+		if(walker)
+			*m = A2D_STAGED_FULL;
+	} else if(last_slice)
+		*m = mine ? A2D_STAGED_PHASES : A2D_STAGED_NONE;
+}
diff --git a/audiality2_amd/replay.py b/audiality2_amd/replay.py
--- a/audiality2_amd/replay.py
+++ b/audiality2_amd/replay.py
@@ -121,6 +121,13 @@
 
     def __repr__(self):
         return "osc2_batch_info(" + ", ".join(f"{n}={getattr(self, n)}" for n, _ in self._fields_) + ")"
+
+
+class a2amd_osc2quiet_batch_info(C.Structure):
+    _fields_ = [("launched", C.c_uint32), ("wavefronts", C.c_uint32), ("taken_total", C.c_uint64)]
+
+    def __repr__(self):
+        return "osc2quiet_batch_info(" + ", ".join(f"{n}={getattr(self, n)}" for n, _ in self._fields_) + ")"
 
 
 class a2amd_fbdpan_batch_info(C.Structure):
@@ -225,6 +232,10 @@
         self._last_batch_osc2 = None
         if hasattr(lib, prefix + "last_batch_osc2"):
             self._last_batch_osc2 = fn("last_batch_osc2", i32, vp, C.POINTER(a2amd_osc2_batch_info))
+        self._last_batch_osc2quiet = None
+        if hasattr(lib, prefix + "last_batch_osc2quiet"):
+            self._last_batch_osc2quiet = fn("last_batch_osc2quiet", i32, vp, C.POINTER(a2amd_osc2quiet_batch_info))
+            self._osc2quiet_hold = fn("osc2quiet_hold", i32, vp, i32)
         self._osc2_stage_rule = self._wave_level_periodic = None
         if hasattr(lib, prefix + "osc2_stage_rule"):
             self._osc2_stage_rule = fn("osc2_stage_rule", u32, u32, i32, u32, i32)
@@ -394,6 +405,18 @@
         bi = a2amd_osc2_batch_info()
         self._chk(self._last_batch_osc2(self.ctx, C.byref(bi)), "last_batch_osc2")
         return bi
+
+    def last_batch_osc2quiet(self):
+        if self._last_batch_osc2quiet is None:
+            raise RuntimeError(f"this library has no {self.prefix}last_batch_osc2quiet")
+        bi = a2amd_osc2quiet_batch_info()
+        self._chk(self._last_batch_osc2quiet(self.ctx, C.byref(bi)), "last_batch_osc2quiet")
+        return bi
+
+    def osc2quiet_hold(self, hold):
+        if self._last_batch_osc2quiet is None:
+            raise RuntimeError(f"this library has no {self.prefix}osc2quiet_hold")
+        self._chk(self._osc2quiet_hold(self.ctx, int(bool(hold))), "osc2quiet_hold")
 
     def osc2_stage_rule(self, size0, periodic0, size1, periodic1):
         if self._osc2_stage_rule is None:
diff --git a/include/a2amd.h b/include/a2amd.h
--- a/include/a2amd.h
+++ b/include/a2amd.h
@@ -203,6 +203,7 @@
 #include "a2amd_osc2.h"
 #include "a2amd_osc2lds.h"
 #include "a2amd_osc2tame.h"
+#include "a2amd_osc2tame_kernel.h"
 #include "a2amd_osc3filt.h"
 #include "a2amd_wavepool.h"
 
diff --git a/include/a2amd_osc2tame_kernel.h b/include/a2amd_osc2tame_kernel.h
--- /dev/null
+++ b/include/a2amd_osc2tame_kernel.h
@@ -0,0 +1,23 @@
+#ifndef A2AMD_OSC2TAME_KERNEL_H
+#define A2AMD_OSC2TAME_KERNEL_H
+#include <stdint.h>
+
+#ifdef __cplusplus
+extern "C" {
+#endif
+
+struct a2amd_ctx;
+
+typedef struct a2amd_osc2quiet_batch_info {
+	uint32_t launched;
+	uint32_t wavefronts;
+	uint64_t taken_total;
+} a2amd_osc2quiet_batch_info;
+int a2amd_last_batch_osc2quiet(struct a2amd_ctx *ctx, a2amd_osc2quiet_batch_info *out);
+
+int a2amd_osc2quiet_hold(struct a2amd_ctx *ctx, int hold);
+
+#ifdef __cplusplus
+}
+#endif
+#endif
```

Result: faster. 627.5 billion voice-samples/s (median of 6 runs) (+9.8%).
